# RohanVKashyap/resolution-pde

Hardware: AMD Instinct MI355X
Metric: training samples/sec, FFNO2D NS 256^2 (higher is better)
Workload: dtype f32; 1 GPU; FFNO2D(1,1,width=64,n_layers=4,n_modes=20,factor=4,ff_weight_norm,n_ff_layers=3,layer_norm,dropout=0.1) train step on [B,1,256,256] Gaussian random fields (BASELINE configs[2]); batch_per_gpu=32, global_batch=32, optimizer=AdamW lr=1e-3 (rpde.optim.FlatAdamW: torch.optim.AdamW's rule, one kernel), parallelism=single, grad_bucket_bytes=6828576, target=input advanced by a fixed spectral filter (utils/synthetic.py:advance)

## Files before the change

include/rpde.h:

```cpp
#ifndef RPDE_H
#define RPDE_H

#include <stddef.h>
#include <stdint.h>

#ifdef __cplusplus
extern "C" {
#endif

typedef enum {
  RPDE_OK = 0,
  RPDE_ERR_ARG = -1,
  RPDE_ERR_HIP = -2,
  RPDE_ERR_WORKSPACE = -3,
  RPDE_ERR_MODES = -4
} rpde_status;

enum { RPDE_NORM_BACKWARD = 0, RPDE_NORM_ORTHO = 1, RPDE_NORM_FORWARD = 2 };
enum { RPDE_MODE_FULL = 0, RPDE_MODE_LOWPASS = 1 };
enum { RPDE_ACT_IDENTITY = 0, RPDE_ACT_GELU = 1, RPDE_ACT_RELU = 2 };
enum { RPDE_EPI_MULAUX = 100 };

const char* rpde_last_error(void);
int rpde_version(void);

typedef struct rpde_plan rpde_plan;
int rpde_plan_create(rpde_plan** plan, int n, int modes, int norm, void* stream);
int rpde_plan_destroy(rpde_plan* plan);
int rpde_plan_info(const rpde_plan* plan, int* n, int* modes, int* kp, int* ldn);
int rpde_plan_cache_count(void);
int rpde_plan_tables(const rpde_plan* plan, float* analysis_host, float* synthesis_host);

typedef struct {
  const float* A; const float* B; float* C;
  int M, N, K;
  int a_kmajor;
  int b_kmajor;
  int64_t lda, ldb, ldc;
  int batch, zdiv;
  int64_t sA1, sA2, sB1, sB2, sC1, sC2;
  int ksplit;
  int64_t sCk;
  float alpha;
  int accumulate;
  const float* bias; int bias_mode;
  int act_a, act_b;
  int epi_dact;
  const float* aux; int64_t ldaux;
  float drop_p; uint64_t drop_seed; int64_t drop_ld;
  int write_act;
  int drop_where;
  float* colsum;
  float* aux_out;
  const void* b_split;
  const void* a_split;
  const float* acc_src;
  const uint64_t* drop_epoch;
} rpde_gemm_desc;
int rpde_gemm_f32(const rpde_gemm_desc* d, void* stream);

size_t rpde_split_weights_bytes(int N, int K);
int rpde_split_weights(const float* w, int kmajor, int64_t ld, int N, int K, void* out, void* stream);

size_t rpde_fspectral1d_ws_bytes(int B, int n, int C, int K);
size_t rpde_fspectral1d_spec_elems(int B, int n, int C, int K);
int rpde_fspectral1d_fwd(const float* x, const float* w, float* out, float* spec_in,
                         int B, int n, int C, int K, int mode, int norm,
                         void* ws, size_t ws_bytes, void* stream);
int rpde_fspectral1d_bwd(const float* grad_out, const float* spec_in, const float* w,
                         float* grad_x, float* grad_w, const float* grad_skip,
                         int B, int n, int C, int K, int mode, int norm,
                         void* ws, size_t ws_bytes, void* stream);

size_t rpde_fspectral2d_ws_bytes(int B, int M, int N, int C, int K);
size_t rpde_fspectral2d_spec_elems(int B, int M, int N, int C, int K, int axis );
int rpde_fspectral2d_fwd(const float* x, const float* w_y, const float* w_x, float* out,
                         float* spec_y, float* spec_x,
                         int B, int M, int N, int C, int K, int mode,
                         void* ws, size_t ws_bytes, void* stream);
int rpde_fspectral2d_bwd(const float* grad_out, const float* spec_y, const float* spec_x,
                         const float* w_y, const float* w_x,
                         float* grad_x, float* grad_wy, float* grad_wx, const float* grad_skip,
                         int B, int M, int N, int C, int K, int mode,
                         void* ws, size_t ws_bytes, void* stream);
size_t rpde_fspectral2d_prep_bytes(int M, int N, int C, int K);
size_t rpde_fspectral2d_eval_ws_bytes(int B, int M, int N, int C, int K);
int rpde_fspectral2d_prepare(const float* w_y, const float* w_x, int M, int N, int C, int K,
                             void* prep, size_t prep_bytes, void* stream);
int rpde_fspectral2d_fwd_prepared(const float* x, const void* prep, float* out, int B, int M, int N, int C, int K,
                                  void* ws, size_t ws_bytes, void* stream);

size_t rpde_spectral1d_ws_bytes(int B, int Cin, int Cout, int n, int K);
int rpde_spectral1d_fwd(const float* x, const float* w, float* out, float* spec_in,
                        int B, int Cin, int Cout, int n, int K, int act_in,
                        void* ws, size_t ws_bytes, void* stream);
int rpde_spectral1d_bwd(const float* grad_out, const float* spec_in, const float* w,
                        const float* x, float* grad_x, float* grad_w,
                        int B, int Cin, int Cout, int n, int K, int act_in,
                        void* ws, size_t ws_bytes, void* stream);

size_t rpde_spectral2d_ws_bytes(int B, int Cin, int Cout, int M, int N, int m1, int m2);
size_t rpde_spectral2d_spec_elems(int B, int Cin, int M, int N, int m1, int m2);
int rpde_spectral2d_fwd(const float* x, const float* w1, const float* w2, float* out, float* spec_in,
                        int B, int Cin, int Cout, int M, int N, int m1, int m2, int act_in,
                        void* ws, size_t ws_bytes, void* stream);
int rpde_spectral2d_bwd(const float* grad_out, const float* spec_in, const float* w1, const float* w2,
                        const float* x, float* grad_x, float* grad_w1, float* grad_w2,
                        int B, int Cin, int Cout, int M, int N, int m1, int m2, int act_in,
                        void* ws, size_t ws_bytes, void* stream);

typedef struct {
  int n_layers; int dim; int factor;
  int layer_norm; float ln_eps;
  float dropout_p; uint64_t seed;
  int post_act;
  const float* const* weights;
  const float* const* biases;
  const float* ln_gamma; const float* ln_beta;
  const uint64_t* seed_epoch;
} rpde_ff_params;
size_t rpde_feedforward_ws_bytes(int64_t P, int dim, int factor, int n_layers);
size_t rpde_feedforward_fwd_ws_bytes(int dim, int factor, int n_layers);
int rpde_feedforward_is_fused(int dim, int factor, int n_layers, int64_t P);
int rpde_feedforward_fwd(const rpde_ff_params* p, const float* x, const float* residual,
                         float* const* hs, float* const* ds, float* z_last, float* out, int64_t P,
                         void* ws, size_t ws_bytes, void* stream);
int rpde_feedforward_bwd(const rpde_ff_params* p, const float* x, const float* const* hs,
                         const float* const* ds, const float* z_last,
                         const float* grad_out, float* grad_x,
                         float* const* grad_weights, float* const* grad_biases,
                         float* grad_gamma, float* grad_beta, int64_t P,
                         void* ws, size_t ws_bytes, void* stream);
int rpde_feedforward_prepare(const rpde_ff_params* p, void* prep, size_t prep_bytes, void* stream);
int rpde_feedforward_fwd_prepared(const rpde_ff_params* p, const float* x, const float* residual, float* out, int64_t P,
                                  const void* prep, size_t prep_bytes, void* stream);

size_t rpde_linear_ws_bytes(int64_t P, int in_f, int out_f);
int rpde_linear_fwd(const float* x, const float* w, const float* b, float* out,
                    int64_t P, int in_f, int out_f, void* stream);
int rpde_linear_bwd(const float* x, const float* w, const float* grad_out,
                    float* grad_x, float* grad_w, float* grad_b,
                    int64_t P, int in_f, int out_f, void* ws, size_t ws_bytes, void* stream);

int rpde_weight_norm_fwd(const float* v, const float* g, float* w, int out_f, int in_f, void* stream);
int rpde_weight_norm_bwd(const float* v, const float* g, const float* grad_w, float* grad_v, float* grad_g,
                         int out_f, int in_f, void* stream);

size_t rpde_conv1x1_ws_bytes(int B, int Cin, int Cout, int64_t S);
int rpde_conv1x1_fwd(const float* x, const float* w, const float* b, float* out,
                     int B, int Cin, int Cout, int64_t S, int act_in, int accumulate, void* stream);
int rpde_conv1x1_act_fwd(const float* x, const float* w, const float* b, float* out,
                         int B, int Cin, int Cout, int64_t S, int act_in, int accumulate, int act_out, void* stream);
size_t rpde_fnoblock2d_eval_ws_bytes(int B, int Cin, int Cout, int M, int N, int m1, int m2);
int rpde_fnoblock2d_eval_ok(int Cin, int Cout, int M, int N, int m2);
int rpde_fnoblock2d_eval_fwd(const float* x, const float* w1, const float* w2, const float* wc, const float* bc, float* out,
                             int B, int Cin, int Cout, int M, int N, int m1, int m2, int act_out,
                             void* ws, size_t ws_bytes, void* stream);
int rpde_fnoblock2d_proj_eval_ok(int Cin, int Cout, int M, int N, int m1, int m2, int Cmid, int Cq);
int rpde_fnoblock2d_proj_eval_fwd(const float* x, const float* w1, const float* w2, const float* wc, const float* bc,
                                  const float* pw1, const float* pb1, const float* pw2, const float* pb2, float* out, int B,
                                  int Cin, int Cout, int M, int N, int m1, int m2, int act_out, int Cmid, int Cq,
                                  void* ws, size_t ws_bytes, void* stream);
size_t rpde_fno2d_lift_block_eval_ws_bytes(int B, int C, int Cout, int M, int N, int m1, int m2);
int rpde_fno2d_lift_block_eval_ok(int Cu, int C, int Cout, int M, int N, int m1, int m2);
int rpde_fno2d_lift_block_eval_fwd(const float* u, const float* gx, const float* gy, const float* wl, const float* bl,
                                   const float* w1, const float* w2, const float* wc, const float* bc, float* out, int B, int C,
                                   int Cout, int M, int N, int m1, int m2, int act_out, void* ws, size_t ws_bytes, void* stream);
int rpde_conv_mlp_ok(int Cin, int Cmid, int Cout, int64_t S);
int rpde_conv_mlp_fwd(const float* x, const float* w1, const float* b1, const float* w2, const float* b2, float* out,
                      int B, int Cin, int Cmid, int Cout, int64_t S, int act_in, void* stream);
int rpde_conv1x1_bwd(const float* x, const float* w, const float* grad_out,
                     float* grad_x, float* grad_w, float* grad_b,
                     int B, int Cin, int Cout, int64_t S, int act_in, int accumulate_gx,
                     void* ws, size_t ws_bytes, void* stream);

int rpde_concat_grid(const float* x, float* out, int B, int Cin, int M, int N ,
                     int grid_dims , double lo, double hi, int channels_last,
                     const float* gridx, const float* gridy, void* stream);
int rpde_transpose_cs(const float* in, float* out, int B, int64_t S, int C, int to_channels_first, void* stream);

size_t rpde_resize1d_ws_bytes(int64_t rows, int n_in, int n_out);
int rpde_resize1d(const float* x, float* out, int64_t rows, int n_in, int n_out,
                  void* ws, size_t ws_bytes, void* stream);
size_t rpde_resize2d_ws_bytes(int64_t rows, int M, int N, int Mo, int No);
int rpde_resize2d(const float* x, float* out, int64_t rows, int M, int N, int Mo, int No,
                  void* ws, size_t ws_bytes, void* stream);

size_t rpde_freq_energy1d_ws_bytes(int64_t rows, int n, int num_modes);
int rpde_freq_energy1d(const float* pred, const float* target, double* acc, int64_t rows, int n, int num_modes,
                       void* ws, size_t ws_bytes, void* stream);
size_t rpde_freq_energy2d_ws_bytes(int64_t images, int H, int W);
int rpde_freq_energy2d(const float* pred, const float* target, const int32_t* bins, double* acc, int64_t images,
                       int H, int W, int n_bins, void* ws, size_t ws_bytes, void* stream);

int rpde_act_fwd(const float* x, float* out, int64_t n, int act, void* stream);
int rpde_act_bwd(const float* x, const float* g, float* dx, int64_t n, int act, void* stream);

int64_t rpde_rel_l2_stats_elems(int B);
int rpde_rel_l2_fwd(const float* x, const float* y, float* rel, float* loss, float* stats,
                    int B, int64_t per, int size_average, void* stream);
int rpde_rel_l2_bwd(const float* x, const float* y, const float* stats,
                    const float* grad_loss, const float* grad_rel, float* grad_x,
                    int B, int64_t per, int size_average, void* stream);

int rpde_adamw_step(float* p, const float* g, float* m, float* v, int64_t n,
                    float one_minus_lr_wd, float one_minus_b1, float b2, float one_minus_b2,
                    float step_size, float bc2_sqrt, float eps, void* stream);
int rpde_adamw_step_dev(float* p, const float* g, float* m, float* v, int64_t n,
                        float lr, float b1, float b2, float eps, float weight_decay,
                        float* step_dev, void* stream);
int rpde_adamw_set_hyper_dev(float* step_dev, float lr, float weight_decay, void* stream);
int rpde_adamw_apply_dev(float* p, const float* g, float* m, float* v, int64_t n,
                         float lr, float b1, float b2, float eps, float weight_decay,
                         const float* step_dev, void* stream);

// ... 5 lines not shown
```

resolution-pde_amd/csrc/feedforward.hip:

```cpp
#include "rpde_internal.h"
#include "pointwise.h"
#include "gemm_kernel.h"
#include "ff_fused.h"
#include "wgrad_h2.h"
#include "thin_linear.h"
#include "conv_small.h"

#include <vector>

namespace rpde {


static inline int ff_in(const rpde_ff_params* p, int l) { return l == 0 ? p->dim : p->dim * p->factor; }
static inline int ff_out(const rpde_ff_params* p, int l) { return l == p->n_layers - 1 ? p->dim : p->dim * p->factor; }

static inline int wgrad_split(long P, int out_f, int in_f) {
  const int tiles = ((out_f + 127) / 128) * ((in_f + 127) / 128);
  long s = 768 / tiles;
  const long cap = (P + 127) / 128;
  if (s > cap) s = cap;
  if (s < 1) s = 1;
  if (s > 1024) s = 1024;
  return (int)s;
}
// ... 62 lines not shown
  if (!dstored && !colsum_slab) {
    if (out_f <= 4 && thin_linear_ok(out_f, in_f) && al16(gx)) return thin_expand(gy, w, 1, in_f, nullptr, gx, P, out_f, in_f, st);
    if (in_f <= 4 && thin_linear_ok(in_f, out_f) && al16(gy)) return thin_contract(gy, w, 1, in_f, nullptr, gx, P, in_f, out_f, st);
  }
  rpde_gemm_desc d = gemm_desc();
  d.A = gy; d.a_kmajor = 1; d.lda = out_f;
  d.B = w; d.b_kmajor = 0; d.ldb = in_f;
  if (wimg && worth_presplit(P, in_f, out_f)) {
    if (!wimg_ready) RPDE_TRY(split_weights(w, 0, in_f, in_f, out_f, wimg, st));
    d.b_split = wimg;
  }
  d.C = gx; d.ldc = in_f;
  d.M = (int)P; d.N = in_f; d.K = out_f;
  if (dstored) { d.epi_dact = RPDE_EPI_MULAUX; d.aux = dstored; d.ldaux = in_f; }
  d.colsum = colsum_slab;
  return launch_gemm(d, st);
}

static size_t ff_wimg_floats(int hid) { return (split_bytes(hid, ((hid + 31) / 32) * 32) + 3) / 4; }

static size_t wgrad_ws_floats(long P, int in_f, int out_f) {
  const int S = wgrad_split(P, out_f, in_f);
  size_t a = (S > 1 ? (size_t)S * out_f * in_f : 0);
  const size_t b = wgrad_h2_slab_floats(P, out_f, in_f);
  if (b > a) a = b;
  if (in_f <= 4 && thin_linear_ok(in_f, out_f) && thin_outer_ws_floats(P, in_f, out_f) > a) a = thin_outer_ws_floats(P, in_f, out_f);
  if (out_f <= 4 && thin_linear_ok(out_f, in_f) && thin_outer_ws_floats(P, out_f, in_f) > a) a = thin_outer_ws_floats(P, out_f, in_f);
  return a;
}

}

using namespace rpde;

extern "C" {

size_t rpde_feedforward_ws_bytes(int64_t P, int dim, int factor, int n_layers) {
  const int hid = n_layers > 1 ? dim * factor : dim;
  size_t n = 2 * arena_bytes((size_t)P * hid);
  for (int l = 0; l < n_layers; ++l) {
    const int i = l == 0 ? dim : dim * factor, o = l == n_layers - 1 ? dim : dim * factor;
    n += arena_bytes(wgrad_ws_floats(P, i, o));
    n += arena_bytes((size_t)(colsum_tiles(P) + REDUCE_CHUNKS) * hid);
    n += arena_bytes(ff_wimg_floats(hid));
  }
  n += arena_bytes(colsum_ws_floats(P, hid)) + arena_bytes(ff_tail_bwd_ws_floats(P, dim));
  rpde_ff_params q;
  memset(&q, 0, sizeof(q));
  q.dim = dim; q.factor = factor; q.n_layers = n_layers;
  if (ff3_fused_ok(&q, (long)P))
    n += arena_bytes((size_t)P * dim) + arena_bytes(ff3_fused_bwd_part_floats()) + arena_bytes(ff3_fused_ws_floats());
  return n;
}

size_t rpde_feedforward_fwd_ws_bytes(int dim, int factor, int n_layers) {
  const size_t a = (size_t)n_layers * arena_bytes(ff_wimg_floats(n_layers > 1 ? dim * factor : dim)), b = arena_bytes(ff3_fused_ws_floats());
  return a > b ? a : b;
}

int rpde_feedforward_is_fused(int dim, int factor, int n_layers, int64_t P) {
  rpde_ff_params q;
  memset(&q, 0, sizeof(q));
  q.dim = dim; q.factor = factor; q.n_layers = n_layers;
  return ff3_fused_ok(&q, (long)P) ? 1 : 0;
}

int rpde_feedforward_prepare(const rpde_ff_params* p, void* prep, size_t prep_bytes, void* stream) {
  RPDE_CHECK_ARG(p && prep, "feedforward_prepare: bad arguments");
  RPDE_CHECK_ARG(ff3_fused_ok(p, 32) && prep_bytes >= arena_bytes(ff3_fused_ws_floats()), "feedforward_prepare: shape not fused or buffer too small");
  RPDE_CHECK_ARG(p->weights && p->weights[0] && p->weights[1] && p->weights[2], "feedforward_prepare: null weights");
  return ff3_fused_prepare(p, prep, as_stream(stream));
}

int rpde_feedforward_fwd_prepared(const rpde_ff_params* p, const float* x, const float* residual, float* out, int64_t P,
                                  const void* prep, size_t prep_bytes, void* stream) {
  RPDE_CHECK_ARG(p && x && out && prep && P > 0 && P < (1L << 31), "feedforward_fwd_prepared: bad arguments");
  RPDE_CHECK_ARG(ff3_fused_ok(p, P) && prep_bytes >= arena_bytes(ff3_fused_ws_floats()), "feedforward_fwd_prepared: shape not fused");
  RPDE_CHECK_ARG(!p->layer_norm || (p->ln_gamma && p->ln_beta), "feedforward_fwd_prepared: layer_norm needs gamma/beta");
  RPDE_CHECK_ARG(p->dropout_p == 0.f, "feedforward_fwd_prepared: evaluation only");
  return ff3_fused_fwd(p, x, residual, nullptr, nullptr, out , out, P,
                       const_cast<void*>(prep), as_stream(stream), true);
}

int rpde_feedforward_fwd(const rpde_ff_params* p, const float* x, const float* residual, float* const* hs,
                         float* const* ds, float* z_last, float* out, int64_t P, void* ws, size_t ws_bytes, void* stream) {
  RPDE_CHECK_ARG(p && x && z_last && out && P > 0, "feedforward_fwd: bad arguments");
  RPDE_CHECK_ARG(p->n_layers >= 1 && p->dim > 0 && p->factor > 0, "feedforward_fwd: bad shape");
  RPDE_CHECK_ARG(P < (1L << 31), "feedforward_fwd: too many points for one call");
  RPDE_CHECK_ARG(p->dropout_p >= 0.f && p->dropout_p < 1.f, "feedforward_fwd: dropout %f", p->dropout_p);
  hipStream_t st = as_stream(stream);
  if (ff3_fused_ok(p, P) && ws && ws_bytes >= arena_bytes(ff3_fused_ws_floats())) {
    RPDE_CHECK_ARG(p->weights[0] && p->weights[1] && p->weights[2], "feedforward_fwd: null weights");
    RPDE_CHECK_ARG(!p->layer_norm || (p->ln_gamma && p->ln_beta), "feedforward_fwd: layer_norm needs gamma/beta");
    return ff3_fused_fwd(p, x, residual, hs, ds, z_last, out, P, ws, st);
  }
  RPDE_CHECK_ARG(p->n_layers == 1 || hs, "feedforward_fwd: hidden buffers missing");
  const int L = p->n_layers;
  Arena ar(ws, ws_bytes);
  const size_t img_floats = ff_wimg_floats(L > 1 ? p->dim * p->factor : p->dim);
  float* wimg[SplitJobs::MAX] = {nullptr, nullptr, nullptr, nullptr};
  bool all_imgs = ws != nullptr && L <= SplitJobs::MAX;
  for (int l = 0; l < (all_imgs ? L : 1) && ws; ++l) {
    float* t = ar.take(img_floats);
    if (!t) { all_imgs = false; break; }
    wimg[l] = t;
  }
  if (all_imgs) {
    SplitJobs sj;
    for (int l = 0; l < L; ++l) {
      RPDE_CHECK_ARG(p->weights[l], "feedforward_fwd: null layer %d weight", l);
      if (worth_presplit(P, ff_out(p, l), ff_in(p, l))) sj.add(p->weights[l], 1, ff_in(p, l), ff_out(p, l), ff_in(p, l), wimg[l]);
    }
    RPDE_TRY(split_weights_multi(sj, st));
  }
  for (int l = 0; l < L; ++l) {
    const bool last = l == L - 1;
    RPDE_CHECK_ARG(p->weights[l] && (last || hs[l]), "feedforward_fwd: null layer %d buffers", l);
    const float* in = l == 0 ? x : hs[l - 1];
    RPDE_TRY(linear_fwd_impl(in, p->weights[l], p->biases ? p->biases[l] : nullptr, last ? z_last : hs[l], P, ff_in(p, l),
                             ff_out(p, l), last ? RPDE_ACT_IDENTITY : RPDE_ACT_GELU, (last || !ds) ? nullptr : ds[l],
                             p->dropout_p, layer_seed(p->seed, l), st, all_imgs ? wimg[l] : wimg[0], p->seed_epoch, all_imgs));
  }
  return ff_tail_fwd(z_last, residual, out, P, p->dim, p->layer_norm, p->ln_eps, p->ln_gamma, p->ln_beta,
                     make_drop(p->dropout_p, layer_seed(p->seed, L - 1), p->seed_epoch), p->post_act, st);
}

int rpde_feedforward_bwd(const rpde_ff_params* p, const float* x, const float* const* hs, const float* const* ds,
                         const float* z_last, const float* grad_out, float* grad_x, float* const* grad_weights,
                         float* const* grad_biases, float* grad_gamma, float* grad_beta, int64_t P, void* ws,
                         size_t ws_bytes, void* stream) {
  RPDE_CHECK_ARG(p && x && z_last && grad_out && P > 0, "feedforward_bwd: bad arguments");
  RPDE_CHECK_ARG(p->n_layers == 1 || (hs && ds), "feedforward_bwd: saved hidden tensors missing");
  RPDE_CHECK_ARG(P < (1L << 31), "feedforward_bwd: too many points for one call");
  hipStream_t st = as_stream(stream);
  const int L = p->n_layers;
  const int hid = L > 1 ? p->dim * p->factor : p->dim;
  Arena ar(ws, ws_bytes);
  float* buf0 = ar.take((size_t)P * hid);
  float* buf1 = ar.take((size_t)P * hid);
  std::vector<float*> slabs_l(L), csum_l(L), wt_l(L);
  for (int l = 0; l < L; ++l) slabs_l[l] = ar.take(wgrad_ws_floats(P, ff_in(p, l), ff_out(p, l)));
  for (int l = 0; l < L; ++l) csum_l[l] = ar.take((size_t)(colsum_tiles(P) + REDUCE_CHUNKS) * hid);
  for (int l = 0; l < L; ++l) wt_l[l] = ar.take(ff_wimg_floats(hid));
  float* small = ar.take(colsum_ws_floats(P, hid));
  float* tailws = ar.take(ff_tail_bwd_ws_floats(P, p->dim));
  if (!ar.ok()) { set_error("feedforward_bwd: workspace too small (%zu bytes given)", ws_bytes); return RPDE_ERR_WORKSPACE; }
  void* wt = wt_l[0];

  if (ff3_fused_ok(p, P) && hs && hs[0] && hs[1]) {
    const int recompute = !(ds && ds[0] && ds[1]);
    const int act_h = recompute ? RPDE_ACT_GELU : RPDE_ACT_IDENTITY;
    float* dz3 = ar.take((size_t)P * p->dim);
    float* part = ar.take(ff3_fused_bwd_part_floats());
    void* fimg = ar.take(ff3_fused_ws_floats());
    if (!ar.ok()) { set_error("feedforward_bwd: workspace too small (%zu bytes given)", ws_bytes); return RPDE_ERR_WORKSPACE; }
    int grid = 0;
    RPDE_TRY(ff3_fused_bwd_launch(p, recompute ? hs : ds, recompute, z_last, grad_out, dz3, buf0, buf1, nullptr, part, &grid, P,
                                  fimg, st));
    const bool both = grad_x && grad_weights && wgrad_h2_dgrad_ok(P, hid, p->dim);
    if (grad_x && !both) RPDE_TRY(linear_dgrad_impl(buf1, p->weights[0], grad_x, P, p->dim, hid, nullptr, nullptr, st, wt));
    if (grad_weights) {
      FoldJobs folds;
      RPDE_TRY(linear_wgrad_impl(hs[1], dz3, grad_weights[2], nullptr, P, hid, p->dim, slabs_l[2], small, st, act_h, &folds));
      RPDE_TRY(linear_wgrad_impl(hs[0], buf0, grad_weights[1], nullptr, P, hid, hid, slabs_l[1], small, st, act_h, &folds));
      if (both) RPDE_TRY(wgrad_h2_dgrad(buf1, x, p->weights[0], grad_weights[0], grad_x, P, p->dim, hid, slabs_l[0], st, &folds));
      else RPDE_TRY(linear_wgrad_impl(x, buf1, grad_weights[0], nullptr, P, p->dim, hid, slabs_l[0], small, st, RPDE_ACT_IDENTITY, &folds));
      RPDE_TRY(fold_jobs(folds, st));
    }
    {
      ReduceSegs sg;
      memset(&sg, 0, sizeof(sg));
      sg.n = FF3_PART; sg.nseg = 5;
      const int off[5] = {0, 256, 512, 576, 640}, len[5] = {hid, hid, p->dim, p->dim, p->dim};
      float* dst[5] = {grad_biases ? grad_biases[0] : nullptr, grad_biases ? grad_biases[1] : nullptr,
                       grad_biases ? grad_biases[2] : nullptr, p->layer_norm ? grad_gamma : nullptr,
                       p->layer_norm ? grad_beta : nullptr};
      for (int k = 0; k < 5; ++k) { sg.off[k] = off[k]; sg.len[k] = len[k]; sg.dst[k] = dst[k]; }
      RPDE_TRY(reduce_slabs_seg(part, grid, FF3_PART, sg, st));
    }
    return RPDE_OK;
  }

  FoldJobs folds;
  float* dz = buf0;
  float* other = buf1;
  int bias_done = 0;
  RPDE_TRY(ff_tail_bwd(z_last, grad_out, dz, P, p->dim, p->layer_norm, p->ln_eps, p->ln_gamma, p->ln_beta,
                       make_drop(p->dropout_p, layer_seed(p->seed, L - 1), p->seed_epoch), p->post_act, grad_gamma, grad_beta,
                       grad_biases ? grad_biases[L - 1] : nullptr, &bias_done, tailws, st, &folds));
  const bool all_imgs = L <= SplitJobs::MAX;
  if (all_imgs) {
    SplitJobs sj;
    for (int l = grad_x ? 0 : 1; l < L; ++l)
      if (worth_presplit(P, ff_in(p, l), ff_out(p, l))) sj.add(p->weights[l], 0, ff_in(p, l), ff_in(p, l), ff_out(p, l), wt_l[l]);
    RPDE_TRY(split_weights_multi(sj, st));
  }
  for (int l = L - 1; l >= 0; --l) {
    const int in_f = ff_in(p, l), out_f = ff_out(p, l);
    const float* in = l == 0 ? x : hs[l - 1];
    float* gb = (grad_biases && !bias_done) ? grad_biases[l] : nullptr;
    RPDE_TRY(linear_wgrad_impl(in, dz, grad_weights ? grad_weights[l] : nullptr, gb, P, in_f, out_f, slabs_l[l], small, st,
                               RPDE_ACT_IDENTITY, &folds));
    bias_done = 0;
    void* img = all_imgs ? wt_l[l] : wt;
    if (l > 0) {
      RPDE_CHECK_ARG(ds[l - 1], "feedforward_bwd: derivative of layer %d was not saved", l - 1);
      const bool fuse = grad_biases && can_fuse_colsum(dz, p->weights[l], other, ds[l - 1], P, in_f, out_f);
      RPDE_TRY(linear_dgrad_impl(dz, p->weights[l], other, P, in_f, out_f, ds[l - 1], fuse ? csum_l[l] : nullptr, st, img, all_imgs));
      if (fuse) {
        const int S = (int)colsum_tiles(P);
        if (!(S <= 4 * REDUCE_CHUNKS && folds.add(csum_l[l], grad_biases[l - 1], in_f, S, in_f)))
          RPDE_TRY(reduce_slabs_2pass(csum_l[l], grad_biases[l - 1], in_f, S, in_f, csum_l[l] + colsum_tiles(P) * in_f, st));
        bias_done = 1;
      }
      float* t = dz; dz = other; other = t;
    } else if (grad_x) {
      RPDE_TRY(linear_dgrad_impl(dz, p->weights[0], grad_x, P, in_f, out_f, nullptr, nullptr, st, img, all_imgs));
    }
  }
  return fold_jobs(folds, st);
}

size_t rpde_linear_ws_bytes(int64_t P, int in_f, int out_f) {
  return arena_bytes(wgrad_ws_floats(P, in_f, out_f)) + arena_bytes(colsum_ws_floats(P, out_f));
}

int rpde_linear_fwd(const float* x, const float* w, const float* b, float* out, int64_t P, int in_f, int out_f, void* stream) {
  RPDE_CHECK_ARG(x && w && out && P > 0 && in_f > 0 && out_f > 0 && P < (1L << 31), "linear_fwd: bad arguments");
  return linear_fwd_impl(x, w, b, out, P, in_f, out_f, RPDE_ACT_IDENTITY, nullptr, 0.f, 0, as_stream(stream));
}

int rpde_linear_bwd(const float* x, const float* w, const float* grad_out, float* grad_x, float* grad_w, float* grad_b,
                    int64_t P, int in_f, int out_f, void* ws, size_t ws_bytes, void* stream) {
  RPDE_CHECK_ARG(x && w && grad_out && P > 0 && in_f > 0 && out_f > 0 && P < (1L << 31), "linear_bwd: bad arguments");
  hipStream_t st = as_stream(stream);
  Arena ar(ws, ws_bytes);
  float* slabs = ar.take(wgrad_ws_floats(P, in_f, out_f));
  float* small = ar.take(colsum_ws_floats(P, out_f));
  if (!ar.ok()) { set_error("linear_bwd: workspace too small"); return RPDE_ERR_WORKSPACE; }
  RPDE_TRY(linear_wgrad_impl(x, grad_out, grad_w, grad_b, P, in_f, out_f, slabs, small, st));
  if (grad_x) RPDE_TRY(linear_dgrad_impl(grad_out, w, grad_x, P, in_f, out_f, nullptr, nullptr, st));
  return RPDE_OK;
}

static int conv1x1_ksplit(int B, int64_t S) {
  int ks = 1;
  while (ks < 8 && B * ks < 64 && S / (2 * ks) >= 128) ks *= 2;
  return ks;
}
size_t rpde_conv1x1_ws_bytes(int B, int Cin, int Cout, int64_t S) {
  return arena_bytes((size_t)B * conv1x1_ksplit(B, S) * Cout * Cin) + arena_bytes((size_t)B * Cout * 64);
}

int rpde_conv1x1_fwd(const float* x, const float* w, const float* b, float* out, int B, int Cin, int Cout, int64_t S,
                     int act_in, int accumulate, void* stream) {
  return rpde_conv1x1_act_fwd(x, w, b, out, B, Cin, Cout, S, act_in, accumulate, RPDE_ACT_IDENTITY, stream);
}

int rpde_conv1x1_act_fwd(const float* x, const float* w, const float* b, float* out, int B, int Cin, int Cout, int64_t S,
                         int act_in, int accumulate, int act_out, void* stream) {
  RPDE_CHECK_ARG(x && w && out && B > 0 && Cin > 0 && Cout > 0 && S > 0 && S < (1L << 31), "conv1x1_fwd: bad arguments");
  if (conv1x1_small_ok(x, out, Cin, Cout, S) && B <= 65535 && (long)B * S >= (1L << 20))
    return conv1x1_small(x, w, b, out, B, Cin, Cout, S, act_in, accumulate, act_out, as_stream(stream));
  rpde_gemm_desc d = gemm_desc();
  d.write_act = act_out;
// ... 82 lines not shown
```

resolution-pde_amd/csrc/ff_fused.h:

```cpp
#pragma once
#include "rpde_internal.h"

namespace rpde {
bool ff3_fused_ok(const rpde_ff_params* p, long P);
size_t ff3_fused_ws_floats();
int ff3_fused_prepare(const rpde_ff_params* p, void* ws, hipStream_t st);
int ff3_fused_fwd(const rpde_ff_params* p, const float* x, const float* residual, float* const* hs, float* const* ds,
                  float* z_last, float* out, long P, void* ws, hipStream_t st, bool prepared = false);
constexpr int FF3_PART = 704;
size_t ff3_fused_bwd_part_floats();
int ff3_fused_bwd_launch(const rpde_ff_params* p, const float* const* ds, int recompute, const float* z_last,
                         const float* grad_out, float* dz3, float* du2, float* du1, float* dx, float* part, int* grid_out,
                         long P, void* ws, hipStream_t st);
}
```

resolution-pde_amd/csrc/ff_fused.hip:

```cpp
#include "ff_fused.h"
#include "cw.h"
#include "h2.h"
#include "pointwise.h"

namespace rpde {

#ifdef RPDE_STAMPS
__device__ unsigned long long g_ffstamps[3 * 64];
#define FFSTAMP(i) do { if (stamp_on && stamp_t < 8) g_ffstamps[stamp_w * 64 + stamp_t * 8 + (i)] = __builtin_amdgcn_s_memtime(); } while (0)
__device__ unsigned long long g_fbstamps[3 * 64];
#define FBSTAMP(i) do { if (stamp_on && stamp_t >= 0 && stamp_t < 8) g_fbstamps[stamp_w * 64 + stamp_t * 8 + (i)] = __builtin_amdgcn_s_memtime(); } while (0)
#else
#define FFSTAMP(i) do { } while (0)
#define FBSTAMP(i) do { } while (0)
#endif

constexpr int FF_WAVES = 8;
constexpr int FF_FRAGS = 24;
constexpr int FF_IMG_BYTES = FF_WAVES * FF_FRAGS * 2048;
constexpr int FF_NCONST = 16;
constexpr int FF_PREP_BLOCKS = FF_WAVES * FF_FRAGS * 64 / 1024;

__global__ __launch_bounds__(1024) void k_ff3_prep(const float* __restrict__ w1, const float* __restrict__ w2,
                                                   const float* __restrict__ w3, const float* __restrict__ b1,
                                                   const float* __restrict__ b2, char* __restrict__ img,
                                                   float* __restrict__ consts) {
  __shared__ float red[6][16];
  __shared__ float fin[6];
  const int tid = threadIdx.x, l = tid & 63, wv = tid >> 6;
  float m1 = 0.f, m2 = 0.f, m3 = 0.f, r1 = 0.f, r2 = 0.f, bm = 0.f;
  {
    const float4* w14 = reinterpret_cast<const float4*>(w1);
    const float4* w34 = reinterpret_cast<const float4*>(w3);
    const float4* w24 = reinterpret_cast<const float4*>(w2);
    float4 a[4], c[4], b[16];
#pragma unroll
    for (int i = 0; i < 4; ++i) { a[i] = w14[tid + 1024 * i]; c[i] = w34[tid + 1024 * i]; }
#pragma unroll
    for (int i = 0; i < 16; ++i) b[i] = w24[tid + 1024 * i];
#pragma unroll
    for (int i = 0; i < 4; ++i) {
      m1 = fmaxf(m1, fmaxf(fmaxf(fabsf(a[i].x), fabsf(a[i].y)), fmaxf(fabsf(a[i].z), fabsf(a[i].w))));
      m3 = fmaxf(m3, fmaxf(fmaxf(fabsf(c[i].x), fabsf(c[i].y)), fmaxf(fabsf(c[i].z), fabsf(c[i].w))));
    }
#pragma unroll
    for (int i = 0; i < 16; ++i) m2 = fmaxf(m2, fmaxf(fmaxf(fabsf(b[i].x), fabsf(b[i].y)), fmaxf(fabsf(b[i].z), fabsf(b[i].w))));
  }
#pragma unroll
  for (int row = wv; row < 256; row += 16) {
    float a = fabsf(w1[row * 64 + l]);
    float b = (fabsf(w2[row * 256 + l]) + fabsf(w2[row * 256 + 64 + l])) + (fabsf(w2[row * 256 + 128 + l]) + fabsf(w2[row * 256 + 192 + l]));
    r1 = fmaxf(r1, wave_sum_dpp(a));
    r2 = fmaxf(r2, wave_sum_dpp(b));
  }
  if (tid < 256) {
    bm = fabsf(b1 ? b1[tid] : 0.f);
  } else if (tid < 512) {
    bm = fabsf(b2 ? b2[tid - 256] : 0.f);
  }
  float v[6] = {m1, m2, m3, r1, r2, 0.f};
#pragma unroll
  for (int k = 0; k < 5; ++k) { v[k] = wave_max(v[k]); if (l == 0) red[k][wv] = v[k]; }
  const float bmw = wave_max(bm);
  if (l == 0) red[5][wv] = bmw;
  __syncthreads();
  if (tid < 5) { float a = 0.f; for (int i = 0; i < 16; ++i) a = fmaxf(a, red[tid][i]); fin[tid] = a; }
  if (tid == 5) { float a = 0.f; for (int i = 0; i < 4; ++i) a = fmaxf(a, red[5][i]); fin[5] = a; }
  __shared__ float fin_b2;
  if (tid == 6) { float a = 0.f; for (int i = 4; i < 8; ++i) a = fmaxf(a, red[5][i]); fin_b2 = a; }
  __syncthreads();
  float sc[3], iv[3];
#pragma unroll
  for (int k = 0; k < 3; ++k) h2_scale(fin[k], 0, sc[k], iv[k]);
  if (tid == 0 && blockIdx.x == 0) {
    consts[0] = iv[0]; consts[1] = iv[1]; consts[2] = iv[2];
    consts[3] = fin[3]; consts[4] = fin[4]; consts[5] = fin[5]; consts[6] = fin_b2;
  }
  for (int it = blockIdx.x * 1024 + tid; it < FF_WAVES * FF_FRAGS * 64; it += gridDim.x * 1024) {
    const int ln = it & 63, f = (it >> 6) % FF_FRAGS, w = it / (64 * FF_FRAGS);
    const int g = ln >> 4, li = ln & 15;
    float x[8];
    if (f < 4) {
      const int row = 16 * (2 * w + (f >> 1)) + li, k0 = 32 * (f & 1) + 8 * g;
#pragma unroll
      for (int j = 0; j < 8; ++j) x[j] = w1[row * 64 + k0 + j] * sc[0];
    } else if (f < 20) {
      const int row = 16 * (2 * w + ((f - 4) >> 3)) + li, kap = (f - 4) & 7;
#pragma unroll
      for (int j = 0; j < 8; ++j) x[j] = w2[row * 256 + 32 * kap + frag_perm(g, j)] * sc[1];
    } else {
      const int row = 16 * (f - 20) + li;
#pragma unroll
      for (int j = 0; j < 8; ++j) x[j] = w3[row * 256 + 32 * w + frag_perm(g, j)] * sc[2];
    }
    h2_put_frag(img + ((long)(w * FF_FRAGS + f)) * 2048 + ln * 16, x);
  }
}

struct FF3P {
  const float* x; const float* res; float* out; float* z3;
  float* h1; float* d1; float* h2; float* d2;
  const char* wimg; const float* consts;
  const float* b1; const float* b2; const float* b3; const float* gamma; const float* beta;
  long P; int layer_norm; float eps; int post_act;
  DropCfg drop[3];
  int ntiles;
};

constexpr int FF_SBUF = 0;
constexpr int FF_RAW = FF_SBUF + 8192;
constexpr int FF_HBUF = FF_RAW + 8192;
constexpr int FF_H2BUF = FF_HBUF + 32768;
constexpr int FF_W3 = FF_H2BUF + 32768;
constexpr int FF_VEC = FF_W3 + 65536;
constexpr int FF_STAT = FF_VEC + 2816;
constexpr int FF_INFO = FF_STAT + 1024;
constexpr int FF_LDS = FF_INFO + 256;

__device__ __forceinline__ void ff_act4(const f32x4v acc, float inv, const float4 b, const DropCfg& drop, uint64_t id,
                                        float (&h)[4], float (&d)[4], float (&u)[4]) {
  float s[4] = {1.f, 1.f, 1.f, 1.f};
  if (drop.on()) drop_scale4(drop, id, s);
  const float bb[4] = {b.x, b.y, b.z, b.w};
#pragma unroll
  for (int r = 0; r < 4; ++r) {
    u[r] = fmaf(acc[r], inv, bb[r]) * s[r];
    act_both(RPDE_ACT_GELU, u[r], h[r], d[r]);
    d[r] *= s[r];
  }
}
__device__ __forceinline__ float4 ff_dact4(const float4 u, const DropCfg& drop, uint64_t id) {
  float s[4] = {1.f, 1.f, 1.f, 1.f};
  if (drop.on()) drop_scale4(drop, id, s);
  return make_float4(dgelu_f(u.x) * s[0], dgelu_f(u.y) * s[1], dgelu_f(u.z) * s[2], dgelu_f(u.w) * s[3]);
}

template <int MODE>
__global__ __launch_bounds__(64 * FF_WAVES, 2) void k_ff3_fwd_h2(const FF3P A0) {
  constexpr bool TRAIN = MODE != 0;
  FF3P A = A0;
#pragma unroll
  for (int i = 0; i < 3; ++i) A.drop[i] = drop_resolve(A0.drop[i]);
  __shared__ __attribute__((aligned(16))) char smem[FF_LDS];
  const int tid = threadIdx.x, l = tid & 63, w = tid >> 6, g = l >> 4, li = l & 15;
  f16x8 w1h[2][2], w1l[2][2], w2h[2][8], w2l[2][8];
  {
    const char* base = A.wimg + (long)w * FF_FRAGS * 2048 + l * 16;
#pragma unroll
    for (int f = 0; f < 4; ++f) {
      w1h[f >> 1][f & 1] = *reinterpret_cast<const f16x8*>(base + f * 2048);
      w1l[f >> 1][f & 1] = *reinterpret_cast<const f16x8*>(base + f * 2048 + 1024);
    }
#pragma unroll
    for (int f = 0; f < 16; ++f) {
      w2h[f >> 3][f & 7] = *reinterpret_cast<const f16x8*>(base + (4 + f) * 2048);
      w2l[f >> 3][f & 7] = *reinterpret_cast<const f16x8*>(base + (4 + f) * 2048 + 1024);
    }
#pragma unroll
    for (int f = 0; f < 4; ++f) {
      const uint4 hi = *reinterpret_cast<const uint4*>(base + (20 + f) * 2048);
      const uint4 lo = *reinterpret_cast<const uint4*>(base + (20 + f) * 2048 + 1024);
      *reinterpret_cast<uint4*>(smem + FF_W3 + (f * 8 + w) * 2048 + l * 16) = hi;
      *reinterpret_cast<uint4*>(smem + FF_W3 + (f * 8 + w) * 2048 + 1024 + l * 16) = lo;
    }
    float* vec = reinterpret_cast<float*>(smem + FF_VEC);
    for (int i = tid; i < 704; i += 64 * FF_WAVES) {
      float v;
      if (i < 256) v = A.b1 ? A.b1[i] : 0.f;
      else if (i < 512) v = A.b2 ? A.b2[i - 256] : 0.f;
      else if (i < 576) v = A.b3 ? A.b3[i - 512] : 0.f;
      else if (i < 640) v = A.gamma ? A.gamma[i - 576] : 1.f;
      else v = A.beta ? A.beta[i - 640] : 0.f;
      vec[i] = v;
    }
  }
  const float* const vec = reinterpret_cast<const float*>(smem + FF_VEC);
  const float winv1 = A.consts[0], winv2 = A.consts[1], winv3 = A.consts[2];
  const float c1 = A.consts[3], c2 = A.consts[4], b1max = A.consts[5], b2max = A.consts[6];
  float* const info = reinterpret_cast<float*>(smem + FF_INFO);
// ... 124 lines not shown
        ff_act4(acc[t], inv2, *reinterpret_cast<const float4*>(vec + 256 + hid), A.drop[1], (uint64_t)(pt * 256 + hid), h, d, u);
        if (MODE == 2 && pt < A.P) *reinterpret_cast<float4*>(A.h2 + pt * 256 + hid) = make_float4(u[0], u[1], u[2], u[3]);
        if (MODE == 1 && pt < A.P) {
          *reinterpret_cast<float4*>(A.h2 + pt * 256 + hid) = make_float4(h[0], h[1], h[2], h[3]);
          *reinterpret_cast<float4*>(A.d2 + pt * 256 + hid) = make_float4(d[0], d[1], d[2], d[3]);
        }
#pragma unroll
        for (int r = 0; r < 4; ++r) hv[4 * t + r] = h[r] * sh2;
      }
      h2_put_frag(smem + FF_H2BUF + ((blk * 8 + w) * 2) * 1024 + l * 16, hv);
    }
    FFSTAMP(4);
    lds_barrier();
    FFSTAMP(5);

    f32x4v acc3 = {0.f, 0.f, 0.f, 0.f};
#pragma unroll
    for (int kap = 0; kap < 8; ++kap) {
      const char* wb = smem + FF_W3 + (t3 * 8 + kap) * 2048 + l * 16;
      const char* hb = smem + FF_H2BUF + ((b3 * 8 + kap) * 2) * 1024 + l * 16;
      acc3 = h2_mfma32(*reinterpret_cast<const f16x8*>(wb), *reinterpret_cast<const f16x8*>(wb + 1024),
                       *reinterpret_cast<const f16x8*>(hb), *reinterpret_cast<const f16x8*>(hb + 1024), acc3);
    }
    if (w < 2 && next_tile < A.ntiles) {
      if (MODE == 1) cw_wait<0, 8>();
      else if (MODE == 2) cw_wait<0, 4>();
      else asm volatile("s_waitcnt vmcnt(0)" ::: "memory");
      s_convert(par ^ 1);
    }
    float v[4];
    {
      const float4 bb = *reinterpret_cast<const float4*>(vec + 512 + 16 * t3 + 4 * g);
      float u0, u1, u2, u3, inv3;
      scales(b3, u0, u1, u2, u3, inv3);
      v[0] = fmaf(acc3[0], inv3, bb.x); v[1] = fmaf(acc3[1], inv3, bb.y);
      v[2] = fmaf(acc3[2], inv3, bb.z); v[3] = fmaf(acc3[3], inv3, bb.w);
      if (TRAIN && pt3 < A.P) *reinterpret_cast<float4*>(A.z3 + off3) = make_float4(v[0], v[1], v[2], v[3]);
      if (A.drop[2].on()) {
        float s4[4];
        drop_scale4(A.drop[2], (uint64_t)(pt3 * 64 + 16 * t3 + 4 * g), s4);
#pragma unroll
        for (int r = 0; r < 4; ++r) v[r] *= s4[r];
      }
    }
    if (A.layer_norm) {
      float sum = (v[0] + v[1]) + (v[2] + v[3]);
      sum += lane_xor16(sum);
      sum += lane_xor32(sum);
      const float mw = sum * (1.f / 16.f);
      float m2 = (v[0] - mw) * (v[0] - mw) + (v[1] - mw) * (v[1] - mw) + (v[2] - mw) * (v[2] - mw) + (v[3] - mw) * (v[3] - mw);
      m2 += lane_xor16(m2);
      m2 += lane_xor32(m2);
      if (g == 0) *reinterpret_cast<float2*>(stat + ((b3 * 4 + t3) * 16 + li) * 2) = make_float2(mw, m2);
    }
    lds_barrier();
    if (A.layer_norm) {
      float mws[4], m2s = 0.f, mean = 0.f;
#pragma unroll
      for (int t = 0; t < 4; ++t) {
        const float2 s2 = *reinterpret_cast<const float2*>(stat + ((b3 * 4 + t) * 16 + li) * 2);
        mws[t] = s2.x; m2s += s2.y; mean += s2.x;
      }
      mean *= 0.25f;
#pragma unroll
      for (int t = 0; t < 4; ++t) m2s += 16.f * (mws[t] - mean) * (mws[t] - mean);
      const float rstd = rsqrtf(m2s * (1.f / 64.f) + A.eps);
      const float4 gm = *reinterpret_cast<const float4*>(vec + 576 + 16 * t3 + 4 * g);
      const float4 bt = *reinterpret_cast<const float4*>(vec + 640 + 16 * t3 + 4 * g);
      v[0] = (v[0] - mean) * rstd * gm.x + bt.x; v[1] = (v[1] - mean) * rstd * gm.y + bt.y;
      v[2] = (v[2] - mean) * rstd * gm.z + bt.z; v[3] = (v[3] - mean) * rstd * gm.w + bt.w;
    }
    if (A.post_act) {
#pragma unroll
      for (int r = 0; r < 4; ++r) v[r] = act_f(A.post_act, v[r]);
    }
    if (pt3 < A.P) *reinterpret_cast<float4*>(A.out + off3) = make_float4(v[0] + resv.x, v[1] + resv.y, v[2] + resv.z, v[3] + resv.w);
    FFSTAMP(6);
#ifdef RPDE_STAMPS
    ++stamp_t;
#endif
  }
}

__global__ __launch_bounds__(1024) void k_ff3_prep_bwd(const float* __restrict__ w1, const float* __restrict__ w2,
                                                       const float* __restrict__ w3, char* __restrict__ img,
                                                       float* __restrict__ consts) {
  __shared__ float red[5][16];
  __shared__ float fin[5];
  const int tid = threadIdx.x, l = tid & 63, wv = tid >> 6;
  float m1 = 0.f, m2 = 0.f, m3 = 0.f, r3 = 0.f, r2 = 0.f;
  {
    const float4* w14 = reinterpret_cast<const float4*>(w1);
    const float4* w34 = reinterpret_cast<const float4*>(w3);
    const float4* w24 = reinterpret_cast<const float4*>(w2);
    float4 a[4], c[4], b[16];
#pragma unroll
    for (int i = 0; i < 4; ++i) { a[i] = w14[tid + 1024 * i]; c[i] = w34[tid + 1024 * i]; }
#pragma unroll
    for (int i = 0; i < 16; ++i) b[i] = w24[tid + 1024 * i];
#pragma unroll
    for (int i = 0; i < 4; ++i) {
      m1 = fmaxf(m1, fmaxf(fmaxf(fabsf(a[i].x), fabsf(a[i].y)), fmaxf(fabsf(a[i].z), fabsf(a[i].w))));
      m3 = fmaxf(m3, fmaxf(fmaxf(fabsf(c[i].x), fabsf(c[i].y)), fmaxf(fabsf(c[i].z), fabsf(c[i].w))));
    }
#pragma unroll
    for (int i = 0; i < 16; ++i) m2 = fmaxf(m2, fmaxf(fmaxf(fabsf(b[i].x), fabsf(b[i].y)), fmaxf(fabsf(b[i].z), fabsf(b[i].w))));
  }
  {
    __shared__ float colp[2][4][256];
    const int col = tid & 255, part = tid >> 8;
    float a = 0.f, b = 0.f;
#pragma unroll
    for (int f = 0; f < 16; ++f) a += fabsf(w3[(16 * part + f) * 256 + col]);
    float wv2[64];
#pragma unroll
    for (int k = 0; k < 64; ++k) wv2[k] = w2[(64 * part + k) * 256 + col];
#pragma unroll
    for (int k = 0; k < 64; ++k) b += fabsf(wv2[k]);
    colp[0][part][col] = a; colp[1][part][col] = b;
    __syncthreads();
    if (tid < 256) {
      r3 = (colp[0][0][tid] + colp[0][1][tid]) + (colp[0][2][tid] + colp[0][3][tid]);
      r2 = (colp[1][0][tid] + colp[1][1][tid]) + (colp[1][2][tid] + colp[1][3][tid]);
    }
  }
  float v[5] = {m1, m2, m3, r3, r2};
#pragma unroll
  for (int k = 0; k < 5; ++k) { v[k] = wave_max(v[k]); if (l == 0) red[k][wv] = v[k]; }
  __syncthreads();
  if (tid < 5) { float a = 0.f; for (int i = 0; i < 16; ++i) a = fmaxf(a, red[tid][i]); fin[tid] = a; }
  __syncthreads();
  float sc[3], iv[3];
#pragma unroll
  for (int k = 0; k < 3; ++k) h2_scale(fin[k], 0, sc[k], iv[k]);
  if (tid == 0 && blockIdx.x == 0) { consts[0] = iv[0]; consts[1] = iv[1]; consts[2] = iv[2]; consts[3] = fin[3]; consts[4] = fin[4]; }
  for (int it = blockIdx.x * 1024 + tid; it < FF_WAVES * FF_FRAGS * 64; it += gridDim.x * 1024) {
    const int ln = it & 63, f = (it >> 6) % FF_FRAGS, w = it / (64 * FF_FRAGS);
    const int g = ln >> 4, li = ln & 15;
    float x[8];
    if (f < 4) {
      const int hid = 16 * (2 * w + (f >> 1)) + li;
#pragma unroll
      for (int j = 0; j < 8; ++j) x[j] = w3[(32 * (f & 1) + frag_perm(g, j)) * 256 + hid] * sc[2];
    } else if (f < 20) {
      const int hid1 = 16 * (2 * w + ((f - 4) >> 3)) + li, kap = (f - 4) & 7;
#pragma unroll
      for (int j = 0; j < 8; ++j) x[j] = w2[(32 * kap + frag_perm(g, j)) * 256 + hid1] * sc[1];
    } else {
      const int feat = 16 * (f - 20) + li;
#pragma unroll
      for (int j = 0; j < 8; ++j) x[j] = w1[(32 * w + frag_perm(g, j)) * 64 + feat] * sc[0];
    }
    h2_put_frag(img + ((long)(w * FF_FRAGS + f)) * 2048 + ln * 16, x);
  }
}

constexpr int FFB_PART = 704;
struct FF3B {
  const float* g; const float* z3; const float* d1; const float* d2;
  float* dz3; float* du2; float* du1; float* dx;
  const char* wimg; const float* consts;
  const float* gamma; const float* beta;
  float* part;
  long P; int layer_norm; float eps; int post_act;
  DropCfg drop2;
  DropCfg drop0, drop1;
  float dmax;
  int ntiles;
};

constexpr int FB_DZBUF = 0;
constexpr int FB_DUBUF = FB_DZBUF + 8192;
constexpr int FB_W3L = FB_DUBUF + 32768;
constexpr int FB_D2 = FB_W3L + 32768;
constexpr int FB_D1 = FB_D2 + 32768;
constexpr int FB_VEC = FB_D1 + 32768;
constexpr int FB_ACC = FB_VEC + 512;
constexpr int FB_INFO = FB_ACC + 8192;
constexpr int FB_LDS = FB_INFO + 128;

template <bool RECOMP>
__global__ __launch_bounds__(64 * FF_WAVES, 2) void k_ff3_bwd_h2(const FF3B A0) {
  __shared__ __attribute__((aligned(16))) char smem[FB_LDS];
  FF3B A = A0;
  A.drop2 = drop_resolve(A0.drop2); A.drop0 = drop_resolve(A0.drop0); A.drop1 = drop_resolve(A0.drop1);
  const int tid = threadIdx.x, l = tid & 63, w = tid >> 6, g = l >> 4, li = l & 15;
  f16x8 w3h[2][2], w2h[2][8], w2l[2][8];
  {
    const char* base = A.wimg + (long)w * FF_FRAGS * 2048 + l * 16;
#pragma unroll
    for (int f = 0; f < 4; ++f) {
      w3h[f >> 1][f & 1] = *reinterpret_cast<const f16x8*>(base + f * 2048);
      *reinterpret_cast<uint4*>(smem + FB_W3L + (w * 4 + f) * 1024 + l * 16) = *reinterpret_cast<const uint4*>(base + f * 2048 + 1024);
    }
#pragma unroll
    for (int f = 0; f < 16; ++f) {
      w2h[f >> 3][f & 7] = *reinterpret_cast<const f16x8*>(base + (4 + f) * 2048);
      w2l[f >> 3][f & 7] = *reinterpret_cast<const f16x8*>(base + (4 + f) * 2048 + 1024);
    }
    float* vecw = reinterpret_cast<float*>(smem + FB_VEC);
    float* accw = reinterpret_cast<float*>(smem + FB_ACC);
    for (int i = tid; i < 128; i += 64 * FF_WAVES) vecw[i] = i < 64 ? (A.gamma ? A.gamma[i] : 1.f) : (A.beta ? A.beta[i - 64] : 0.f);
    for (int i = tid; i < 2048; i += 64 * FF_WAVES) accw[i] = 0.f;
  }
  const float* const vec = reinterpret_cast<const float*>(smem + FB_VEC);
  float* const acc_db1 = reinterpret_cast<float*>(smem + FB_ACC);
  float* const acc_db2 = acc_db1 + 256;
  float* const acc_db3 = acc_db1 + 512;
  float* const acc_dg = acc_db1 + 1024;
  float* const acc_dbt = acc_db1 + 1536;
  float* const info = reinterpret_cast<float*>(smem + FB_INFO);
  const float winv1 = A.consts[0], winv2 = A.consts[1], winv3 = A.consts[2], c3t = A.consts[3], c2t = A.consts[4];
  const unsigned lds0 = lds_addr(smem);
  const int q3 = l >> 4, feat = 4 * li;

  f32x4v g4n = {0.f, 0.f, 0.f, 0.f}, z4n = g4n;
  auto in_issue = [&](int tile) {
    const long p = min((long)tile * 32 + 4 * w + q3, A.P - 1);
    g4n = global_load_b128(A.g + p * 64 + feat);
    z4n = global_load_b128(A.z3 + p * 64 + feat);
  };
  typedef __attribute__((address_space(3))) void* lds_ptr;
  typedef const __attribute__((address_space(1))) void* glb_ptr;
  auto d_issue = [&](const float* d, int area, int tile) {
#pragma unroll
    for (int blk = 0; blk < 2; ++blk)
#pragma unroll
      for (int t = 0; t < 2; ++t) {
        const float* q = d + min((long)tile * 32 + 16 * blk + li, A.P - 1) * 256 + 16 * (2 * w + t) + 4 * g;
        __builtin_amdgcn_global_load_lds((glb_ptr)(q), (lds_ptr)(smem + area + (w * 4 + blk * 2 + t) * 1024), 16, 0, 0);
      }
  };
  asm volatile("s_waitcnt vmcnt(0)" ::: "memory");
  if ((int)blockIdx.x < A.ntiles) {
    in_issue(blockIdx.x);
    d_issue(A.d2, FB_D2, blockIdx.x);
    d_issue(A.d1, FB_D1, blockIdx.x);
// ... 176 lines not shown
    FBSTAMP(6);

#pragma unroll
    for (int i = 0; i < 8; ++i) bsum[i] = 0.f;
    {
      f32x4v acc[2][2];
#pragma unroll
      for (int blk = 0; blk < 2; ++blk) {
        acc[blk][0] = (f32x4v){0.f, 0.f, 0.f, 0.f}; acc[blk][1] = (f32x4v){0.f, 0.f, 0.f, 0.f};
#pragma unroll
        for (int kap = 0; kap < 8; ++kap) {
          const char* hb = smem + FB_DUBUF + ((blk * 8 + kap) * 2) * 1024 + l * 16;
          const f16x8 bh = *reinterpret_cast<const f16x8*>(hb), bl = *reinterpret_cast<const f16x8*>(hb + 1024);
          acc[blk][0] = h2_mfma32(w2h[0][kap], w2l[0][kap], bh, bl, acc[blk][0]);
          acc[blk][1] = h2_mfma32(w2h[1][kap], w2l[1][kap], bh, bl, acc[blk][1]);
        }
      }
      if (has_next) asm volatile("s_waitcnt vmcnt(10)" ::: "memory"); else asm volatile("s_waitcnt vmcnt(2)" ::: "memory");
      FBSTAMP(7);
#pragma unroll
      for (int blk = 0; blk < 2; ++blk) {
        f32x4v dq[2];
        dq[0] = lds_read_b128(lds0 + FB_D1 + (w * 4 + blk * 2) * 1024 + l * 16);
        dq[1] = lds_read_b128(lds0 + FB_D1 + (w * 4 + blk * 2 + 1) * 1024 + l * 16);
        lds_wait(dq[0], dq[1]);
        const long pt = p0 + 16 * blk + li;
        float q0, q1, inv_b, s_du1, q2;
        bscales(blk, q0, q1, inv_b, s_du1, q2);
#pragma unroll
        for (int t = 0; t < 2; ++t) {
          const int hid = 16 * (2 * w + t) + 4 * g;
          float4 d = make_float4(dq[t].x, dq[t].y, dq[t].z, dq[t].w);
          if (RECOMP) d = ff_dact4(d, A.drop0, (uint64_t)(pt * 256 + hid));
          const float u[4] = {acc[blk][t][0] * inv_b * d.x, acc[blk][t][1] * inv_b * d.y,
                              acc[blk][t][2] * inv_b * d.z, acc[blk][t][3] * inv_b * d.w};
          if (pt < A.P) {
            *reinterpret_cast<float4*>(A.du1 + pt * 256 + hid) = make_float4(u[0], u[1], u[2], u[3]);
#pragma unroll
            for (int r = 0; r < 4; ++r) bsum[4 * t + r] += u[r];
          }
        }
      }
    }
    if (has_next) {
      asm volatile("s_waitcnt lgkmcnt(0)" ::: "memory");
      d_issue(A.d1, FB_D1, next_tile);
    }
#pragma unroll
    for (int i = 0; i < 8; ++i) bsum[i] = row_sum15(bsum[i]);
    if (li == 15) {
#pragma unroll
      for (int i = 0; i < 8; ++i) acc_db1[16 * (2 * w + (i >> 2)) + 4 * g + (i & 3)] += bsum[i];
    }
    first = false;
#ifdef RPDE_STAMPS
    ++stamp_t;
#endif
  }
  lds_barrier();
  {
    float* part = A.part + (long)blockIdx.x * FFB_PART;
    for (int i = tid; i < FFB_PART; i += 64 * FF_WAVES) {
      float v;
      if (i < 512) v = acc_db1[i];
      else {
        const float* a8 = acc_db3 + ((i - 512) >> 6) * 512 + ((i - 512) & 63);
        v = 0.f;
#pragma unroll
        for (int ww = 0; ww < FF_WAVES; ++ww) v += a8[ww * 64];
      }
      part[i] = v;
    }
  }
}

bool ff3_fused_ok(const rpde_ff_params* p, long P) {
  if (switch_off("RPDE_FUSED_FF")) return false;
  for (int l = 0; l < 3 && p->weights; ++l)
    if (reinterpret_cast<uintptr_t>(p->weights[l]) & 15) return false;
  return p->n_layers == 3 && p->dim == 64 && p->factor == 4 && P >= 32;
}
size_t ff3_fused_ws_floats() { return (FF_IMG_BYTES + FF_NCONST * 4 + 3) / 4; }

int ff3_fused_prepare(const rpde_ff_params* p, void* ws, hipStream_t st) {
  char* img = static_cast<char*>(ws);
  float* consts = reinterpret_cast<float*>(img + FF_IMG_BYTES);
  const float* b1 = p->biases ? p->biases[0] : nullptr;
  const float* b2 = p->biases ? p->biases[1] : nullptr;
  hipLaunchKernelGGL(k_ff3_prep, dim3(FF_PREP_BLOCKS), dim3(1024), 0, st, p->weights[0], p->weights[1], p->weights[2], b1, b2, img, consts);
  RPDE_LAUNCH_CHECK();
  return RPDE_OK;
}

int ff3_fused_fwd(const rpde_ff_params* p, const float* x, const float* residual, float* const* hs, float* const* ds,
                  float* z_last, float* out, long P, void* ws, hipStream_t st, bool prepared) {
  char* img = static_cast<char*>(ws);
  float* consts = reinterpret_cast<float*>(img + FF_IMG_BYTES);
  const float* b1 = p->biases ? p->biases[0] : nullptr;
  const float* b2 = p->biases ? p->biases[1] : nullptr;
  const float* b3 = p->biases ? p->biases[2] : nullptr;
  if (!prepared) RPDE_TRY(ff3_fused_prepare(p, ws, st));
  FF3P A;
  memset(&A, 0, sizeof(A));
  const bool have_h = hs && hs[0] && hs[1], have_d = ds && ds[0] && ds[1];
  const int mode = have_h ? (have_d ? 1 : 2) : 0;
  A.x = x; A.res = residual; A.out = out; A.z3 = z_last;
  if (mode) { A.h1 = hs[0]; A.h2 = hs[1]; }
  if (mode == 1) { A.d1 = ds[0]; A.d2 = ds[1]; }
  A.wimg = img; A.consts = consts; A.b1 = b1; A.b2 = b2; A.b3 = b3; A.gamma = p->ln_gamma; A.beta = p->ln_beta;
  A.P = P; A.layer_norm = p->layer_norm; A.eps = p->ln_eps; A.post_act = p->post_act;
  for (int l = 0; l < 3; ++l) {
    A.drop[l] = make_drop(p->dropout_p, layer_seed(p->seed, l), p->seed_epoch);
  }
  A.ntiles = (int)((P + 31) / 32);
  int cus;
  RPDE_HIP(cu_count(&cus));
  const int grid = A.ntiles < cus ? A.ntiles : cus;
  if (mode == 1) hipLaunchKernelGGL(k_ff3_fwd_h2<1>, dim3(grid), dim3(64 * FF_WAVES), 0, st, A);
  else if (mode == 2) hipLaunchKernelGGL(k_ff3_fwd_h2<2>, dim3(grid), dim3(64 * FF_WAVES), 0, st, A);
  else hipLaunchKernelGGL(k_ff3_fwd_h2<0>, dim3(grid), dim3(64 * FF_WAVES), 0, st, A);
  RPDE_LAUNCH_CHECK();
  return RPDE_OK;
}

size_t ff3_fused_bwd_part_floats() { return (size_t)1024 * FFB_PART; }

int ff3_fused_bwd_launch(const rpde_ff_params* p, const float* const* ds, int recompute, const float* z_last,
                         const float* grad_out, float* dz3, float* du2, float* du1, float* dx, float* part, int* grid_out,
                         long P, void* ws, hipStream_t st) {
  char* img = static_cast<char*>(ws);
  float* consts = reinterpret_cast<float*>(img + FF_IMG_BYTES);
  hipLaunchKernelGGL(k_ff3_prep_bwd, dim3(FF_PREP_BLOCKS), dim3(1024), 0, st, p->weights[0], p->weights[1], p->weights[2], img, consts);
  RPDE_LAUNCH_CHECK();
  FF3B A;
  memset(&A, 0, sizeof(A));
  A.g = grad_out; A.z3 = z_last; A.d1 = ds[0]; A.d2 = ds[1];
  A.dz3 = dz3; A.du2 = du2; A.du1 = du1; A.dx = dx;
  A.wimg = img; A.consts = consts; A.gamma = p->ln_gamma; A.beta = p->ln_beta; A.part = part;
  A.P = P; A.layer_norm = p->layer_norm; A.eps = p->ln_eps; A.post_act = p->post_act;
  DropCfg dc[3];
  for (int l = 0; l < 3; ++l)
    dc[l] = make_drop(p->dropout_p, layer_seed(p->seed, l), p->seed_epoch);
  A.drop0 = dc[0]; A.drop1 = dc[1]; A.drop2 = dc[2];
  A.dmax = 1.13f * A.drop2.scale;
  A.ntiles = (int)((P + 31) / 32);
  int cus;
  RPDE_HIP(cu_count(&cus));
  if (cus > 1024) cus = 1024;
  const int grid = A.ntiles < cus ? A.ntiles : cus;
  if (recompute) hipLaunchKernelGGL(k_ff3_bwd_h2<true>, dim3(grid), dim3(64 * FF_WAVES), 0, st, A);
  else hipLaunchKernelGGL(k_ff3_bwd_h2<false>, dim3(grid), dim3(64 * FF_WAVES), 0, st, A);
  RPDE_LAUNCH_CHECK();
  *grid_out = grid;
  return RPDE_OK;
}

}

#ifdef RPDE_STAMPS
extern "C" int rpde_debug_ffb_stamps(unsigned long long* host_out) {
  RPDE_HIP(hipDeviceSynchronize());
  RPDE_HIP(hipMemcpyFromSymbol(host_out, HIP_SYMBOL(rpde::g_fbstamps), sizeof(unsigned long long) * 3 * 64));
  return RPDE_OK;
}
extern "C" int rpde_debug_ff_stamps(unsigned long long* host_out) {
  RPDE_HIP(hipDeviceSynchronize());
  RPDE_HIP(hipMemcpyFromSymbol(host_out, HIP_SYMBOL(rpde::g_ffstamps), sizeof(unsigned long long) * 3 * 64));
  return RPDE_OK;
}
#endif
```

resolution-pde_amd/csrc/fspectral.hip:

```cpp
#include "rpde_internal.h"
#include "plan.h"
#include "pointwise.h"
#include "fused_spectral.h"
#include "mix1d.h"

namespace rpde {

struct Axis {
  int n;
  int keff, kp;
  int rows;
  int zdiv;
  long s1, s2;
  long ld;
  const rpde_plan* plan;
};

static inline int split_for(long k_total, int tiles) {
  long s = 512 / (tiles > 0 ? tiles : 1);
  const long cap = (k_total + 127) / 128;
  if (s > cap) s = cap;
  if (s < 1) s = 1;
  if (s > 512) s = 512;
  return (int)s;
// ... 80 lines not shown
  RPDE_TRY(dft_analysis(ax, x, spec_in, C, false, st));
  const float* syn_in = spec_in;
  if (mode == RPDE_MODE_FULL && mix1d_ok(ax.rows, C)) {
    float* mixed = ar.take(spec_floats(ax, C));
    if (!ar.ok()) { set_error("fspectral: workspace too small"); return RPDE_ERR_WORKSPACE; }
    RPDE_TRY(mix1d(spec_in, w, mixed, ax.rows, C, K, ax.keff, ax.kp, false, st));
    syn_in = mixed;
  } else if (mode == RPDE_MODE_FULL) {
    float* wblk = ar.take((size_t)ax.keff * 4 * C * C);
    float* mixed = ar.take(spec_floats(ax, C));
    if (!ar.ok()) { set_error("fspectral: workspace too small"); return RPDE_ERR_WORKSPACE; }
    RPDE_TRY(pack_mix_weights(w, wblk, C, C, K, ax.keff, st));
    if (ax.kp != ax.keff) RPDE_HIP(hipMemsetAsync(mixed, 0, spec_floats(ax, C) * sizeof(float), st));
    RPDE_TRY(mode_mix(ax, spec_in, wblk, mixed, C, false, st));
    syn_in = mixed;
  }
  return dft_synthesis(ax, syn_in, out, C, false, accumulate, st);
}

static int axis_bwd(const Axis& ax, const float* g, const float* spec_in, const float* w, int K, float* gx, float* gw, int C,
                    int mode, int accumulate, Arena& ar, hipStream_t st, const float* skip = nullptr) {
  float* gspec = ar.take(spec_floats(ax, C));
  if (!ar.ok()) { set_error("fspectral: workspace too small"); return RPDE_ERR_WORKSPACE; }
  RPDE_TRY(dft_analysis(ax, g, gspec, C, true, st));
  const float* dspec = gspec;
  if (mode == RPDE_MODE_FULL && mix1d_ok(ax.rows, C)) {
    float* dsp = ar.take(spec_floats(ax, C));
    if (!ar.ok()) { set_error("fspectral: workspace too small"); return RPDE_ERR_WORKSPACE; }
    if (gw) RPDE_TRY(mix1d_wgrad(spec_in, gspec, gw, ax.rows, C, K, ax.keff, ax.kp, st));
    if (gx) {
      RPDE_TRY(mix1d(gspec, w, dsp, ax.rows, C, K, ax.keff, ax.kp, true, st));
      dspec = dsp;
    }
  } else if (mode == RPDE_MODE_FULL) {
    float* wblk = ar.take((size_t)ax.keff * 4 * C * C);
    float* dsp = ar.take(spec_floats(ax, C));
    const int S = split_for(ax.rows, wgrad_tiles(C) * ax.keff);
    float* slabs = ar.take((size_t)S * ax.keff * 4 * C * C);
    if (!ar.ok()) { set_error("fspectral: workspace too small"); return RPDE_ERR_WORKSPACE; }
    if (gw) {
      RPDE_TRY(mode_mix_wgrad(ax, spec_in, gspec, slabs, C, S, st));
      RPDE_TRY(unpack_mix_grad(slabs, gw, C, C, K, ax.keff, S, (long)ax.keff * 4 * C * C, st));
    }
    if (gx) {
      RPDE_TRY(pack_mix_weights(w, wblk, C, C, K, ax.keff, st));
      if (ax.kp != ax.keff) RPDE_HIP(hipMemsetAsync(dsp, 0, spec_floats(ax, C) * sizeof(float), st));
      RPDE_TRY(mode_mix(ax, gspec, wblk, dsp, C, true, st));
      dspec = dsp;
    }
  } else if (gw) {
    RPDE_HIP(hipMemsetAsync(gw, 0, sizeof(float) * 2 * (size_t)C * C * K, st));
  }
  if (gx) RPDE_TRY(dft_synthesis(ax, dspec, gx, C, true, (!accumulate && skip) ? 2 : accumulate, st, skip));
  return RPDE_OK;
}

static bool fused_mix_on() {
  return !switch_off("RPDE_FUSED_MIX");
}

static int mixw_slabs(const Axis& ay, const Axis& ax) {
  const long tiles = (ay.rows < ax.rows ? ay.rows : ax.rows) / 32;
  long S = tiles / 4;
  if (S > 12) S = 12;
  if (S < 1) S = 1;
  return (int)S;
}

static size_t fused2d_ws(const Axis& ay, const Axis& ax, int C, bool backward) {
  const size_t spy = arena_bytes(spec_floats(ay, C)), spx = arena_bytes(spec_floats(ax, C));
  const size_t wblk = arena_bytes((size_t)ay.keff * 4 * C * C);
  const size_t img = arena_bytes(fused2d_img_bytes(ay.rows, 2 * ay.kp) / 4) + arena_bytes(fused2d_img_bytes(ax.rows, 2 * ax.kp) / 4);
  const size_t inv = arena_bytes(ay.rows) + arena_bytes(ax.rows);
  const size_t mix = arena_bytes(mix_wimg_bytes(ay.kp) / 4) + arena_bytes(4 * (size_t)ay.kp) + arena_bytes(ay.rows) + arena_bytes(ax.rows);
  size_t n = wblk + (spy > spx ? spy : spx) + img + inv + mix;
  if (backward) {
    const int Sy = split_for(ay.rows, wgrad_tiles(C) * ay.keff), Sx = split_for(ax.rows, wgrad_tiles(C) * ax.keff);
    const size_t sl = arena_bytes((size_t)(Sy > Sx ? Sy : Sx) * ay.keff * 4 * C * C);
    n += spy + spx + sl + arena_bytes(mix_wgrad_slab_floats(ay.kp, mixw_slabs(ay, ax)));
  }
  return n;
}

static int fused2d_fwd(const Axis& ay, const Axis& ax, const float* x, const float* w_y, const float* w_x, float* out,
                       float* spec_y, float* spec_x, int B, int M, int N, int C, int K, int mode, Arena& ar, hipStream_t st,
                       const void* prep = nullptr) {
  float* wblk = ar.take((size_t)ay.keff * 4 * C * C);
  const size_t sy = spec_floats(ay, C), sx = spec_floats(ax, C);
  float* mixed = ar.take(sy > sx ? sy : sx);
  void* imgy = ar.take(fused2d_img_bytes(ay.rows, 2 * ay.kp) / 4);
  void* imgx = ar.take(fused2d_img_bytes(ax.rows, 2 * ax.kp) / 4);
  float* invy = ar.take(ay.rows);
  float* invx = ar.take(ax.rows);
  void* wimg = ar.take(mix_wimg_bytes(ay.kp) / 4);
  float* wc = ar.take(4 * (size_t)ay.kp);
  float* amy = spec_y + spec_floats(ay, C);
  float* amx = spec_x + spec_floats(ax, C);
  if (!ar.ok()) { set_error("fspectral2d: workspace too small"); return RPDE_ERR_WORKSPACE; }
  if (mode == RPDE_MODE_FULL && fused_mix_on()) {
    if (prep) {
      wimg = const_cast<void*>(prep);
      wc = reinterpret_cast<float*>(static_cast<char*>(wimg) + arena_bytes(mix_wimg_bytes(ay.kp) / 4));
    } else {
      RPDE_TRY(mix_prep(w_y, w_x, K, ay.keff, ay.kp, 0, wimg, wc, st));
    }
    RPDE_TRY(fused2d_analysis(x, spec_y, spec_x, amy, amx, ay.plan, ax.plan, 0, B, M, N, st));
    RPDE_TRY(mix_h2(spec_y, spec_x, amy, amx, imgy, imgx, invy, invx, ay.rows, ax.rows, ay.kp, wimg, wc, st));
    return fused2d_synthesis(imgy, imgx, invy, invx, ay.plan, ax.plan, 0, out, nullptr, B, M, N, st);
  }
  RPDE_TRY(fused2d_analysis(x, spec_y, spec_x, nullptr, nullptr, ay.plan, ax.plan, 0, B, M, N, st));
  const Axis* axes[2] = {&ay, &ax};
  const float* ws_[2] = {w_y, w_x};
  float* specs[2] = {spec_y, spec_x};
  void* imgs[2] = {imgy, imgx};
  float* invs[2] = {invy, invx};
  for (int a = 0; a < 2; ++a) {
    const Axis& A = *axes[a];
    const float* syn_in = specs[a];
    if (mode == RPDE_MODE_FULL) {
      RPDE_TRY(pack_mix_weights(ws_[a], wblk, C, C, K, A.keff, st));
      if (A.kp != A.keff) RPDE_HIP(hipMemsetAsync(mixed, 0, spec_floats(A, C) * sizeof(float), st));
      RPDE_TRY(mode_mix(A, specs[a], wblk, mixed, C, false, st));
      syn_in = mixed;
    }
    RPDE_TRY(fused2d_split(syn_in, imgs[a], invs[a], A.rows, 2 * A.kp, st));
  }
  return fused2d_synthesis(imgy, imgx, invy, invx, ay.plan, ax.plan, 0, out, nullptr, B, M, N, st);
}

static int fused2d_bwd(const Axis& ay, const Axis& ax, const float* g, const float* spec_y, const float* spec_x,
                       const float* w_y, const float* w_x, float* gx, float* gwy, float* gwx, const float* skip, int B, int M,
                       int N, int C, int K, int mode, Arena& ar, hipStream_t st) {
  float* gsy = ar.take(spec_floats(ay, C));
  float* gsx = ar.take(spec_floats(ax, C));
  float* wblk = ar.take((size_t)ay.keff * 4 * C * C);
  const size_t sy = spec_floats(ay, C), sx = spec_floats(ax, C);
  float* dsp = ar.take(sy > sx ? sy : sx);
  void* imgy = ar.take(fused2d_img_bytes(ay.rows, 2 * ay.kp) / 4);
  void* imgx = ar.take(fused2d_img_bytes(ax.rows, 2 * ax.kp) / 4);
  float* invy = ar.take(ay.rows);
  float* invx = ar.take(ax.rows);
  const int Sy = split_for(ay.rows, wgrad_tiles(C) * ay.keff), Sx = split_for(ax.rows, wgrad_tiles(C) * ax.keff);
  float* slabs = ar.take((size_t)(Sy > Sx ? Sy : Sx) * ay.keff * 4 * C * C);
  void* wimg = ar.take(mix_wimg_bytes(ay.kp) / 4);
  float* wc = ar.take(4 * (size_t)ay.kp);
  float* amy = ar.take(ay.rows);
  float* amx = ar.take(ax.rows);
  const int Sw = mixw_slabs(ay, ax);
  float* wslabs = ar.take(mix_wgrad_slab_floats(ay.kp, Sw));
  if (!ar.ok()) { set_error("fspectral2d: workspace too small"); return RPDE_ERR_WORKSPACE; }
  const bool h2mix = mode == RPDE_MODE_FULL && fused_mix_on();
  const bool hmix = h2mix && gx, hwg = h2mix && (gwy || gwx);
  if (hmix) RPDE_TRY(mix_prep(w_y, w_x, K, ay.keff, ay.kp, 1, wimg, wc, st));
  RPDE_TRY(fused2d_analysis(g, gsy, gsx, h2mix ? amy : nullptr, h2mix ? amx : nullptr, ay.plan, ax.plan, 1, B, M, N, st));
  if (hmix) {
    RPDE_TRY(mix_h2(gsy, gsx, amy, amx, imgy, imgx, invy, invx, ay.rows, ax.rows, ay.kp, wimg, wc, st));
  }
  if (hwg) {
    RPDE_TRY(mix_wgrad_h2(spec_y, spec_x, gsy, gsx, spec_y + spec_floats(ay, C), spec_x + spec_floats(ax, C), amy, amx, gwy, gwx,
                          ay.rows, ax.rows, K, ay.keff, ay.kp, wslabs, Sw, st));
  }
  const Axis* axes[2] = {&ay, &ax};
  const float* ws_[2] = {w_y, w_x};
  const float* specs[2] = {spec_y, spec_x};
  float* gspecs[2] = {gsy, gsx};
  float* gws[2] = {gwy, gwx};
  void* imgs[2] = {imgy, imgx};
  float* invs[2] = {invy, invx};
  const int Ss[2] = {Sy, Sx};
  for (int a = 0; a < 2; ++a) {
    const Axis& A = *axes[a];
    const float* dspec = gspecs[a];
    if (mode == RPDE_MODE_FULL) {
      if (gws[a] && !hwg) {
        RPDE_TRY(mode_mix_wgrad(A, specs[a], gspecs[a], slabs, C, Ss[a], st));
        RPDE_TRY(unpack_mix_grad(slabs, gws[a], C, C, K, A.keff, Ss[a], (long)A.keff * 4 * C * C, st));
      }
      if (gx && !hmix) {
        RPDE_TRY(pack_mix_weights(ws_[a], wblk, C, C, K, A.keff, st));
        if (A.kp != A.keff) RPDE_HIP(hipMemsetAsync(dsp, 0, spec_floats(A, C) * sizeof(float), st));
        RPDE_TRY(mode_mix(A, gspecs[a], wblk, dsp, C, true, st));
        dspec = dsp;
      }
    } else if (gws[a]) {
      RPDE_HIP(hipMemsetAsync(gws[a], 0, sizeof(float) * 2 * (size_t)C * C * K, st));
    }
    if (gx && !hmix) RPDE_TRY(fused2d_split(dspec, imgs[a], invs[a], A.rows, 2 * A.kp, st));
  }
  if (gx) RPDE_TRY(fused2d_synthesis(imgy, imgx, invy, invx, ay.plan, ax.plan, 1, gx, skip, B, M, N, st));
  return RPDE_OK;
}

}

using namespace rpde;

extern "C" {

size_t rpde_fspectral1d_ws_bytes(int B, int n, int C, int K) {
  Axis ax; axis_dims(ax, n, K, B);
  return axis_ws_bytes(ax, C);
}
size_t rpde_fspectral1d_spec_elems(int B, int n, int C, int K) {
  Axis ax; axis_dims(ax, n, K, B);
  return spec_floats(ax, C);
}

int rpde_fspectral1d_fwd(const float* x, const float* w, float* out, float* spec_in, int B, int n, int C, int K, int mode,
                         int norm, void* ws, size_t ws_bytes, void* stream) {
  RPDE_CHECK_ARG(x && out && spec_in && B > 0 && n > 0 && C > 0 && K > 0, "fspectral1d_fwd: bad arguments");
  RPDE_CHECK_ARG(mode == RPDE_MODE_LOWPASS || w, "fspectral1d_fwd: null weight");
  RPDE_CHECK_ARG(mode == RPDE_MODE_FULL || mode == RPDE_MODE_LOWPASS, "Mode %d not recognized", mode);
  hipStream_t st = as_stream(stream);
  Axis ax;
  RPDE_TRY(make_axis(ax, n, K, norm, B, 1, (long)n * C, 0, C, st));
  Arena ar(ws, ws_bytes);
  return axis_fwd(ax, x, w, K, out, spec_in, C, mode, 0, ar, st);
}

int rpde_fspectral1d_bwd(const float* grad_out, const float* spec_in, const float* w, float* grad_x, float* grad_w,
                         const float* grad_skip, int B, int n, int C, int K, int mode, int norm, void* ws, size_t ws_bytes,
                         void* stream) {
  RPDE_CHECK_ARG(grad_out && spec_in && B > 0 && n > 0 && C > 0 && K > 0, "fspectral1d_bwd: bad arguments");
  RPDE_CHECK_ARG(mode == RPDE_MODE_LOWPASS || w, "fspectral1d_bwd: null weight");
  hipStream_t st = as_stream(stream);
  Axis ax;
  RPDE_TRY(make_axis(ax, n, K, norm, B, 1, (long)n * C, 0, C, st));
  Arena ar(ws, ws_bytes);
  return axis_bwd(ax, grad_out, spec_in, w, K, grad_x, grad_w, C, mode, 0, ar, st, grad_skip);
}

size_t rpde_fspectral2d_ws_bytes(int B, int M, int N, int C, int K) {
  Axis ay, ax;
  axis_dims(ay, N, K, B * M);
  axis_dims(ax, M, K, B * N);
  const size_t a = axis_ws_bytes(ay, C), b = axis_ws_bytes(ax, C);
  size_t n = a > b ? a : b;
  if (fused2d_ok(M, N, C, ay.keff, ax.keff)) { const size_t f = fused2d_ws(ay, ax, C, true); if (f > n) n = f; }
  return n;
}
size_t rpde_fspectral2d_spec_elems(int B, int M, int N, int C, int K, int axis) {
  Axis a, o;
  if (axis == 0) { axis_dims(a, N, K, B * M); axis_dims(o, M, K, B * N); } else { axis_dims(a, M, K, B * N); axis_dims(o, N, K, B * M); }
  const bool fused = axis == 0 ? fused2d_ok(M, N, C, a.keff, o.keff) : fused2d_ok(M, N, C, o.keff, a.keff);
  return spec_floats(a, C) + (fused ? (size_t)a.rows : 0);
}

int rpde_fspectral2d_fwd(const float* x, const float* w_y, const float* w_x, float* out, float* spec_y, float* spec_x, int B,
                         int M, int N, int C, int K, int mode, void* ws, size_t ws_bytes, void* stream) {
  RPDE_CHECK_ARG(x && out && spec_y && spec_x && B > 0 && M > 0 && N > 0 && C > 0 && K > 0, "fspectral2d_fwd: bad arguments");
  RPDE_CHECK_ARG(mode == RPDE_MODE_LOWPASS || (w_y && w_x), "fspectral2d_fwd: null weight");
  RPDE_CHECK_ARG(mode == RPDE_MODE_FULL || mode == RPDE_MODE_LOWPASS, "fspectral2d_fwd: mode %d", mode);
  hipStream_t st = as_stream(stream);
  Axis ay, ax;
  RPDE_TRY(make_axis(ay, N, K, RPDE_NORM_ORTHO, B * M, 1, (long)N * C, 0, C, st));
  RPDE_TRY(make_axis(ax, M, K, RPDE_NORM_ORTHO, B * N, N, (long)M * N * C, C, (long)N * C, st));
  if (fused2d_ok(M, N, C, ay.keff, ax.keff)) {
    Arena ar(ws, ws_bytes);
    return fused2d_fwd(ay, ax, x, w_y, w_x, out, spec_y, spec_x, B, M, N, C, K, mode, ar, st);
  }
  {
    Arena ar(ws, ws_bytes);
    RPDE_TRY(axis_fwd(ax, x, w_x, K, out, spec_x, C, mode, 0, ar, st));
  }
  Arena ar(ws, ws_bytes);
  return axis_fwd(ay, x, w_y, K, out, spec_y, C, mode, 1, ar, st);
}

size_t rpde_fspectral2d_prep_bytes(int M, int N, int C, int K) {
  Axis ay, ax;
  axis_dims(ay, N, K, M);
  axis_dims(ax, M, K, N);
  if (!fused2d_ok(M, N, C, ay.keff, ax.keff) || !fused_mix_on()) return 0;
  return arena_bytes(mix_wimg_bytes(ay.kp) / 4) + arena_bytes(4 * (size_t)ay.kp);
}

size_t rpde_fspectral2d_eval_ws_bytes(int B, int M, int N, int C, int K) {
  return rpde_fspectral2d_ws_bytes(B, M, N, C, K) + arena_bytes(rpde_fspectral2d_spec_elems(B, M, N, C, K, 0)) +
         arena_bytes(rpde_fspectral2d_spec_elems(B, M, N, C, K, 1));
}

int rpde_fspectral2d_prepare(const float* w_y, const float* w_x, int M, int N, int C, int K, void* prep, size_t prep_bytes,
                             void* stream) {
  RPDE_CHECK_ARG(w_y && w_x && prep && M > 0 && N > 0 && K > 0, "fspectral2d_prepare: bad arguments");
  const size_t need = rpde_fspectral2d_prep_bytes(M, N, C, K);
  RPDE_CHECK_ARG(need > 0 && prep_bytes >= need, "fspectral2d_prepare: shape not on the fused path or buffer too small");
  Axis ay;
  axis_dims(ay, N, K, M);
  float* wc = reinterpret_cast<float*>(static_cast<char*>(prep) + arena_bytes(mix_wimg_bytes(ay.kp) / 4));
  return mix_prep(w_y, w_x, K, ay.keff, ay.kp, 0, prep, wc, as_stream(stream));
}

int rpde_fspectral2d_fwd_prepared(const float* x, const void* prep, float* out, int B, int M, int N, int C, int K, void* ws,
                                  size_t ws_bytes, void* stream) {
  RPDE_CHECK_ARG(x && prep && out && ws && B > 0 && M > 0 && N > 0 && C > 0 && K > 0, "fspectral2d_fwd_prepared: bad arguments");
  RPDE_CHECK_ARG(rpde_fspectral2d_prep_bytes(M, N, C, K) > 0, "fspectral2d_fwd_prepared: shape not on the fused path");
  hipStream_t st = as_stream(stream);
  Axis ay, ax;
  RPDE_TRY(make_axis(ay, N, K, RPDE_NORM_ORTHO, B * M, 1, (long)N * C, 0, C, st));
  RPDE_TRY(make_axis(ax, M, K, RPDE_NORM_ORTHO, B * N, N, (long)M * N * C, C, (long)N * C, st));
  Arena ar(ws, ws_bytes);
  float* spec_y = ar.take(rpde_fspectral2d_spec_elems(B, M, N, C, K, 0));
  float* spec_x = ar.take(rpde_fspectral2d_spec_elems(B, M, N, C, K, 1));
  if (!ar.ok()) { set_error("fspectral2d_fwd_prepared: workspace too small"); return RPDE_ERR_WORKSPACE; }
  Arena rest(static_cast<char*>(ws) + ar.used, ws_bytes - ar.used);
  return fused2d_fwd(ay, ax, x, nullptr, nullptr, out, spec_y, spec_x, B, M, N, C, K, RPDE_MODE_FULL, rest, st, prep);
}

int rpde_fspectral2d_bwd(const float* grad_out, const float* spec_y, const float* spec_x, const float* w_y, const float* w_x,
                         float* grad_x, float* grad_wy, float* grad_wx, const float* grad_skip, int B, int M, int N, int C,
                         int K, int mode, void* ws, size_t ws_bytes, void* stream) {
  RPDE_CHECK_ARG(grad_out && spec_y && spec_x && B > 0 && M > 0 && N > 0 && C > 0 && K > 0, "fspectral2d_bwd: bad arguments");
  RPDE_CHECK_ARG(mode == RPDE_MODE_LOWPASS || (w_y && w_x), "fspectral2d_bwd: null weight");
  hipStream_t st = as_stream(stream);
  Axis ay, ax;
  RPDE_TRY(make_axis(ay, N, K, RPDE_NORM_ORTHO, B * M, 1, (long)N * C, 0, C, st));
  RPDE_TRY(make_axis(ax, M, K, RPDE_NORM_ORTHO, B * N, N, (long)M * N * C, C, (long)N * C, st));
  if (fused2d_ok(M, N, C, ay.keff, ax.keff)) {
    Arena ar(ws, ws_bytes);
    return fused2d_bwd(ay, ax, grad_out, spec_y, spec_x, w_y, w_x, grad_x, grad_wy, grad_wx, grad_skip, B, M, N, C, K, mode,
                       ar, st);
  }
  {
    Arena ar(ws, ws_bytes);
    RPDE_TRY(axis_bwd(ax, grad_out, spec_x, w_x, K, grad_x, grad_wx, C, mode, 0, ar, st, grad_skip));
  }
  Arena ar(ws, ws_bytes);
  return axis_bwd(ay, grad_out, spec_y, w_y, K, grad_x, grad_wy, C, mode, 1, ar, st);
}

}
```

resolution-pde_amd/csrc/fused_mix.hip:

```cpp
#include "fused_spectral.h"
#include "h2.h"

namespace rpde {

__global__ __launch_bounds__(256) void k_mix_prep(const float* __restrict__ w_y, const float* __restrict__ w_x, int K, int keff,
                                                  int kp, int conj_t, char* __restrict__ img, float* __restrict__ wc) {
  __shared__ float ws[64 * 64 * 2];
  __shared__ float red[2][4];
  const int k = blockIdx.x, a = blockIdx.y, tid = threadIdx.x, l = tid & 63, wv = tid >> 6, g = l >> 4, li = l & 15;
  const float* __restrict__ w = a ? w_x : w_y;
  char* out = img + (size_t)(a * kp + k) * MIX_W_BYTES_PER_MODE;
  if (k >= keff) {
    for (int i = tid; i < MIX_W_BYTES_PER_MODE / 16; i += 256) reinterpret_cast<uint4*>(out)[i] = make_uint4(0, 0, 0, 0);
    if (tid == 0) { wc[(a * kp + k) * 2] = 1.f; wc[(a * kp + k) * 2 + 1] = 0.f; }
    return;
  }
  float m = 0.f;
  float2 v[16];
#pragma unroll
  for (int u = 0; u < 16; ++u) v[u] = *reinterpret_cast<const float2*>(w + ((long)(tid + 256 * u) * K + k) * 2);
#pragma unroll
  for (int u = 0; u < 16; ++u) {
    const int e = tid + 256 * u;
    ws[e * 2] = v[u].x; ws[e * 2 + 1] = v[u].y;
    m = fmaxf(m, fmaxf(fabsf(v[u].x), fabsf(v[u].y)));
  }
  __syncthreads();
  float s = 0.f;
  {
    const int c = tid & 63, part = tid >> 6;
    for (int r = 16 * part; r < 16 * part + 16; ++r) {
      const int e = conj_t ? c * 64 + ((r + c) & 63) : r * 64 + c;
      s += fabsf(ws[e * 2]) + fabsf(ws[e * 2 + 1]);
    }
  }
  __shared__ float psum[4][64];
  psum[tid >> 6][tid & 63] = s;
  __syncthreads();
  s = tid < 64 ? (psum[0][tid] + psum[1][tid]) + (psum[2][tid] + psum[3][tid]) : 0.f;
  m = wave_max(m);
  s = wave_max(s);
  if (l == 0) { red[0][wv] = m; red[1][wv] = s; }
  __syncthreads();
  m = fmaxf(fmaxf(red[0][0], red[0][1]), fmaxf(red[0][2], red[0][3]));
  s = red[1][0];
  float sc, iv;
  h2_scale(m, 0, sc, iv);
  if (tid == 0) { wc[(a * kp + k) * 2] = iv; wc[(a * kp + k) * 2 + 1] = s; }
  const int cb = wv;
#pragma unroll
  for (int part = 0; part < 2; ++part)
#pragma unroll
    for (int ks = 0; ks < 2; ++ks) {
      float v[8];
#pragma unroll
      for (int j = 0; j < 8; ++j) {
        const int kred = 32 * ks + 8 * g + j, col = 16 * cb + li;
        const int e = conj_t ? col * 64 + kred : kred * 64 + col;
        float x = ws[e * 2 + part];
        if (conj_t && part) x = -x;
        v[j] = x * sc;
      }
      uint4 hi, lo;
      h2_split8(v, hi, lo);
      char* p = out + (((cb * 2 + part) * 2 + ks) * 2) * 1024 + l * 16;
      *reinterpret_cast<uint4*>(p) = hi;
      *reinterpret_cast<uint4*>(p + 1024) = lo;
    }
}

size_t mix_wimg_bytes(int kp) { return (size_t)2 * kp * MIX_W_BYTES_PER_MODE; }

int mix_prep(const float* w_y, const float* w_x, int K, int keff, int kp, int conj_t, void* wimg, float* wc, hipStream_t st) {
  hipLaunchKernelGGL(k_mix_prep, dim3(kp, 2), dim3(256), 0, st, w_y, w_x, K, keff, kp, conj_t, (char*)wimg, wc);
  RPDE_LAUNCH_CHECK();
  return RPDE_OK;
}

struct MixP {
  const float* spec[2];
  char* img[2];
  const float* amax[2];
  float* inv[2];
  int tiles[2];
  int tps[2];
  int nblk0;
  const char* wimg; const float* wc;
  int kp, R, nq;
};

constexpr int MIX_LDS = 4 * 3 * 2 * 2 * 1024;

template <int K32, int TG>
__global__ __launch_bounds__(256, 2) void k_mix_h2(const MixP P) {
  constexpr int BB = h2_block_bytes(K32, TG);
  constexpr int NP = h2_np(TG);
  __shared__ __attribute__((aligned(16))) char smem[MIX_LDS];
  const int tid = threadIdx.x, l = tid & 63, w = tid >> 6, g = l >> 4, li = l & 15;
  int bid = blockIdx.x;
  const int a = bid >= P.nblk0 ? 1 : 0;
  if (a) bid -= P.nblk0;
  const int q = bid % P.nq, slice = bid / P.nq;
  const int t0 = slice * P.tps[a], t1 = min(t0 + P.tps[a], P.tiles[a]);
  if (t0 >= t1) return;
  const int cb = w;
  const float* __restrict__ spec = P.spec[a];
  const float* __restrict__ amax = P.amax[a];
  char* __restrict__ img = P.img[a];
  const long lstride = (long)P.R * 64;

  f16x8 wf[4][2][2][2];
  float winv[4];
  {
    const char* base = P.wimg + ((size_t)(a * P.kp + 4 * q) * 4 + cb) * (MIX_W_BYTES_PER_MODE / 4) + l * 16;
#pragma unroll
    for (int kk = 0; kk < 4; ++kk) {
#pragma unroll
      for (int f = 0; f < 8; ++f)
        wf[kk][f >> 2][(f >> 1) & 1][f & 1] = *reinterpret_cast<const f16x8*>(base + (size_t)kk * MIX_W_BYTES_PER_MODE + f * 1024);
      winv[kk] = P.wc[(a * P.kp + 4 * q + kk) * 2];
    }
  }
  float wnorm = 0.f;
  for (int k = l; k < P.kp; k += 64) wnorm = fmaxf(wnorm, P.wc[(a * P.kp + k) * 2 + 1]);
  wnorm = wave_max(wnorm);

  float4 raw[8];
  float am_next = 0.f;
  auto issue = [&](int t) {
    const float* p = spec + ((long)t * 16 + li) * lstride + (4 * q + w) * 128 + 8 * g;
#pragma unroll
    for (int n = 0; n < 8; ++n) raw[n] = *reinterpret_cast<const float4*>(p + (n >> 2) * 64 + ((n >> 1) & 1) * 32 + (n & 1) * 4);
    am_next = amax[(long)t * 16 + li];
  };
  issue(t0);
  const bool tail = q >= 4 * K32;
  for (int t = t0; t < t1; ++t) {
    const long line0 = (long)t * 16;
    const float am_li = am_next;
    {
      const float am = am_li;
      float sin_, iin;
      h2_scale(am, 0, sin_, iin);
#pragma unroll
      for (int part = 0; part < 2; ++part)
#pragma unroll
        for (int ks = 0; ks < 2; ++ks) {
          const float4 v0 = raw[part * 4 + ks * 2], v1 = raw[part * 4 + ks * 2 + 1];
          uint2 h0, l0, h1, l1;
          h2_split4(v0.x * sin_, v0.y * sin_, v0.z * sin_, v0.w * sin_, h0, l0);
          h2_split4(v1.x * sin_, v1.y * sin_, v1.z * sin_, v1.w * sin_, h1, l1);
          const uint4 hi = make_uint4(h0.x, h0.y, h1.x, h1.y), lo = make_uint4(l0.x, l0.y, l1.x, l1.y);
          char* d = smem + (((w * 3 + part) * 2 + ks) * 2) * 1024 + l * 16;
          *reinterpret_cast<uint4*>(d) = hi;
          *reinterpret_cast<uint4*>(d + 1024) = lo;
          if (part) {
            const unsigned s = 0x80008000u;
// ... 238 lines not shown
```

resolution-pde_amd/csrc/fused_spectral.h:

```cpp
#pragma once
#include "rpde_internal.h"
#include "plan.h"

namespace rpde {

bool fused2d_ok(int M, int N, int C, int keff_y, int keff_x);
int h2_build_tables(rpde_plan* p, hipStream_t st);

__host__ __device__ constexpr int h2_np(int TG) { return (3 * TG + 3) / 4; }
__host__ __device__ constexpr int h2_block_bytes(int K32, int TG) { return (2 * K32 + h2_np(TG)) * 1024; }

size_t fused2d_img_bytes(long lines, int R);
int fused2d_analysis(const float* x, float* spec_y, float* spec_x, float* amax_y, float* amax_x, const rpde_plan* py,
                     const rpde_plan* px, int adjoint, int B, int M, int N, hipStream_t st);
int fused2d_split(const float* spec, void* img, float* inv, long lines, int R, hipStream_t st);
int fused2d_synthesis(const void* imgy, const void* imgx, const float* invy, const float* invx, const rpde_plan* py,
                      const rpde_plan* px, int adjoint, float* out, const float* skip, int B, int M, int N, hipStream_t st);

constexpr int MIX_W_BYTES_PER_MODE = 4 * 2 * 2 * 2 * 1024;
size_t mix_wimg_bytes(int kp);
int mix_prep(const float* w_y, const float* w_x, int K, int keff, int kp, int conj_t, void* wimg, float* wc, hipStream_t st);
size_t mix_wgrad_slab_floats(int kp, int S);
int mix_wgrad_h2(const float* spec_y, const float* spec_x, const float* gspec_y, const float* gspec_x, const float* amax_sy,
                 const float* amax_sx, const float* amax_gy, const float* amax_gx, float* gw_y, float* gw_x, long lines_y,
                 long lines_x, int K, int keff, int kp, float* slabs, int S, hipStream_t st);
int mix_h2(const float* spec_y, const float* spec_x, const float* amax_y, const float* amax_x, void* img_y, void* img_x,
           float* inv_y, float* inv_x, long lines_y, long lines_x, int kp, const void* wimg, const float* wc, hipStream_t st);

}
```

resolution-pde_amd/csrc/wgrad_h2.hip:

```cpp
#include "h2.h"
#include "pointwise.h"
#include "wgrad_h2.h"

namespace rpde {

constexpr int WG_WAVES = 8;
constexpr int WG_PANEL = 8192;
constexpr int WG_BLOCKS = 256;

struct WgP {
  const float* a;
  const float* b;
  float* slabs;
  long npts;
  long steps;
  int M, N, nchunk;
  const float* w;
  float* gx;
  int early;
};

template <int PA, int PB, int WM, int WN, int TM, int TN, bool ACT, bool DG = false>
__global__ __launch_bounds__(64 * WG_WAVES, 2) void k_wgrad_h2(const WgP P) {
  static_assert(!DG || (PB == 1 && PA * 2 <= 8), "data gradient: N = 64, M <= 256");
  constexpr int WFRAG = DG ? PA * 2 * 4 * 2048 : 0;
  static_assert(WM * WN == WG_WAVES && PA + PB <= WG_WAVES, "eight waves, one panel per loader wave");
  static_assert(WM * TM * 16 == PA * 64 && WN * TN * 16 == PB * 64, "wave tiles cover the block");
  static_assert((TM * 16) % 64 == 0 || 64 % (TM * 16) == 0, "a wave tile stays inside one panel or covers whole panels");
  constexpr int STAGE = (PA + PB) * WG_PANEL;
  __shared__ __attribute__((aligned(16))) char smem[2 * STAGE + WFRAG];
  __shared__ int einfo[2][WG_WAVES];
  __shared__ float wmax[WG_WAVES];
  const int tid = threadIdx.x, l = tid & 63, wave = tid >> 6, g = l >> 4, li = l & 15;
  const int chunk = blockIdx.x, mblock = blockIdx.y;
  const long s0 = P.steps * chunk / P.nchunk, s1 = P.steps * (chunk + 1) / P.nchunk;

  const bool loader = wave < PA + PB, isA = wave < PA;
  const int ld = isA ? P.M : P.N;
  const float* __restrict__ src = isA ? P.a + mblock * (64 * PA) + 64 * wave : P.b + 64 * (wave - PA);
  src += (long)g * ld + 4 * li;
  float4 buf[8];
  int e_run = 15;
  auto issue = [&](long s) {
    if (!loader || s >= s1) return;
    const float* __restrict__ q0 = src + s * 32 * ld;
    if ((s + 1) * 32 <= P.npts) {
#pragma unroll
      for (int i = 0; i < 8; ++i) buf[i] = *reinterpret_cast<const float4*>(q0 + (long)(4 * i) * ld);
    } else {
#pragma unroll
      for (int i = 0; i < 8; ++i)
        buf[i] = s * 32 + 4 * i + g < P.npts ? *reinterpret_cast<const float4*>(q0 + (long)(4 * i) * ld) : make_float4(0.f, 0.f, 0.f, 0.f);
    }
  };
  auto convert = [&](int st) {
    if (!loader) return;
    if (ACT && !isA) {
#pragma unroll
      for (int i = 0; i < 8; ++i) { buf[i].x = gelu_f(buf[i].x); buf[i].y = gelu_f(buf[i].y); buf[i].z = gelu_f(buf[i].z); buf[i].w = gelu_f(buf[i].w); }
    }
    float m = 0.f;
#pragma unroll
    for (int i = 0; i < 8; ++i) m = fmaxf(fmaxf(m, fmaxf(fabsf(buf[i].x), fabsf(buf[i].y))), fmaxf(fabsf(buf[i].z), fabsf(buf[i].w)));
    m = wave_max(m);
    e_run = max(e_run, (int)(__float_as_uint(m) >> 23) & 0xff);
    e_run = min(e_run, 254);
    const float scale = __uint_as_float((unsigned)(268 - e_run) << 23);
    char* const dst = smem + st * STAGE + wave * WG_PANEL;
#pragma unroll
    for (int i = 0; i < 8; ++i) {
      uint2 hi, lo;
      h2_split4(buf[i].x * scale, buf[i].y * scale, buf[i].z * scale, buf[i].w * scale, hi, lo);
      const int off = stage_off(4 * i + g, li);
      *reinterpret_cast<uint2*>(dst + off) = hi;
      *reinterpret_cast<uint2*>(dst + 4096 + off) = lo;
    }
    if (l == 0) einfo[st][wave] = e_run;
  };

  const int wm = wave / WN, wn = wave % WN;
  const int m_off = wm * TM * 16, n_off = wn * TN * 16;
  const int pa = m_off >> 6, ta0 = (m_off & 63) >> 4, pb = PA + (n_off >> 6), tb0 = (n_off & 63) >> 4;
  const int q = li >> 2, pp = li & 3;
  const int tsw = ((q >> 1) & 1) | ((g & 1) << 1);
  const int trow = (8 * g + q) * 128 + pp * 8;
  typedef s16x4v __attribute__((address_space(3))) * lds_tr;
  auto frag = [&](const char* panel, int tile, f16x8& hi, f16x8& lo) {
    const char* t = panel + trow + ((tile ^ tsw) << 5);
    union { struct { s16x4v a, b; } h; f16x8 v; } uh, ul;
    uh.h.a = __builtin_amdgcn_ds_read_tr16_b64_v4i16((lds_tr)(t));
    uh.h.b = __builtin_amdgcn_ds_read_tr16_b64_v4i16((lds_tr)(t + 512));
    ul.h.a = __builtin_amdgcn_ds_read_tr16_b64_v4i16((lds_tr)(t + 4096));
    ul.h.b = __builtin_amdgcn_ds_read_tr16_b64_v4i16((lds_tr)(t + 4096 + 512));
    hi = uh.v; lo = ul.v;
  };
  f32x4v acc[TM][TN];
#pragma unroll
  for (int i = 0; i < TM; ++i)
#pragma unroll
    for (int j = 0; j < TN; ++j) acc[i][j] = (f32x4v){0.f, 0.f, 0.f, 0.f};
  constexpr int NPA = (TM * 16 + 63) / 64;
  static_assert(TN * 16 <= 64, "one B panel per wave tile");
  int ea_used[NPA], eb_used = 15;
#pragma unroll
  for (int k = 0; k < NPA; ++k) ea_used[k] = 15;

  char* const wfrag = smem + 2 * STAGE;
  float w_inv = 1.f;
  if (DG && s0 < s1) {
    constexpr int NF = PA * 2 * 4 * 64 / (64 * WG_WAVES);
    float wv[NF][8];
    float m = 0.f;
#pragma unroll
    for (int r = 0; r < NF; ++r) {
      const int c = tid + r * 64 * WG_WAVES, fl = c & 63, nt = (c >> 6) & 3, ks = c >> 8;
#pragma unroll
      for (int j = 0; j < 8; ++j) {
        wv[r][j] = P.w[(long)(32 * ks + 8 * (fl >> 4) + j) * P.N + 16 * nt + (fl & 15)];
        m = fmaxf(m, fabsf(wv[r][j]));
      }
    }
    m = wave_max(m);
    if (l == 0) wmax[wave] = m;
    __syncthreads();
    m = 0.f;
#pragma unroll
    for (int i = 0; i < WG_WAVES; ++i) m = fmaxf(m, wmax[i]);
    float w_scale;
    h2_scale(m, 0, w_scale, w_inv);
#pragma unroll
    for (int r = 0; r < NF; ++r) {
      const int c = tid + r * 64 * WG_WAVES, fl = c & 63, nt = (c >> 6) & 3, ks = c >> 8;
      uint2 h0, l0, h1, l1;
      h2_split4(wv[r][0] * w_scale, wv[r][1] * w_scale, wv[r][2] * w_scale, wv[r][3] * w_scale, h0, l0);
      h2_split4(wv[r][4] * w_scale, wv[r][5] * w_scale, wv[r][6] * w_scale, wv[r][7] * w_scale, h1, l1);
      char* d = wfrag + (ks * 4 + nt) * 2048 + fl * 16;
      *reinterpret_cast<uint4*>(d) = make_uint4(h0.x, h0.y, h1.x, h1.y);
      *reinterpret_cast<uint4*>(d + 1024) = make_uint4(l0.x, l0.y, l1.x, l1.y);
    }
  }
  const int dg_mt = wave & 1, dg_nt = wave >> 1;

  const bool early_convert = (P.early >> __builtin_amdgcn_readfirstlane(wave)) & 1;
  if (s0 < s1) {
    issue(s0);
    convert(0);
    issue(s0 + 1);
    lds_barrier();
    for (long s = s0; s < s1; ++s) {
      const int cur = (int)(s - s0) & 1;
      const char* const stage = smem + cur * STAGE;
      if (early_convert && s + 1 < s1) {
        convert(cur ^ 1);
        issue(s + 2);
      }
      const int eb = __builtin_amdgcn_readfirstlane(einfo[cur][pb]);
#pragma unroll
      for (int k = 0; k < NPA; ++k) {
        const int ea = __builtin_amdgcn_readfirstlane(einfo[cur][pa + k]);
        if (ea + eb != ea_used[k] + eb_used) {
          const int d = (ea_used[k] + eb_used) - (ea + eb);
          const float f = d > -126 ? __uint_as_float((unsigned)(127 + d) << 23) : 0.f;
#pragma unroll
          for (int i = 0; i < TM; ++i)
            if (((ta0 + i) >> 2) == k) {
#pragma unroll
              for (int j = 0; j < TN; ++j) acc[i][j] *= f;
            }
        }
        ea_used[k] = ea;
      }
      eb_used = eb;
      f16x8 bh[TN], bl[TN];
#pragma unroll
      for (int j = 0; j < TN; ++j) frag(stage + (pb + ((tb0 + j) >> 2)) * WG_PANEL, (tb0 + j) & 3, bh[j], bl[j]);
#pragma unroll
      for (int i = 0; i < TM; ++i) {
        f16x8 ah, al;
        frag(stage + (pa + ((ta0 + i) >> 2)) * WG_PANEL, (ta0 + i) & 3, ah, al);
#pragma unroll
        for (int j = 0; j < TN; ++j) acc[i][j] = h2_mfma32(ah, al, bh[j], bl[j], acc[i][j]);
      }
      if (DG) {
        f32x4v tot = (f32x4v){0.f, 0.f, 0.f, 0.f};
        const int row = 16 * dg_mt + li;
#pragma unroll
        for (int k = 0; k < PA; ++k) {
          f32x4v part = (f32x4v){0.f, 0.f, 0.f, 0.f};
#pragma unroll
          for (int h = 0; h < 2; ++h) {
            const char* pa_ = stage + k * WG_PANEL + stage_off(row, 2 * (4 * h + g));
            const f16x8 ah = *reinterpret_cast<const f16x8*>(pa_), al = *reinterpret_cast<const f16x8*>(pa_ + 4096);
            const char* wb = wfrag + ((2 * k + h) * 4 + dg_nt) * 2048 + l * 16;
            const f16x8 bh = *reinterpret_cast<const f16x8*>(wb), bl = *reinterpret_cast<const f16x8*>(wb + 1024);
            part = h2_mfma32(ah, al, bh, bl, part);
          }
          const int ek = __builtin_amdgcn_readfirstlane(einfo[cur][k]);
          const float fk = __uint_as_float((unsigned)(ek - 14) << 23) * w_inv;
          tot += part * fk;
        }
        float t0 = tot[0], t1 = tot[1], t2 = tot[2], t3 = tot[3];
        quad_transpose(t0, t1, t2, t3);
        const long pq = s * 32 + 16 * dg_mt + 4 * g + (li & 3);
        if (pq < P.npts) *reinterpret_cast<float4*>(P.gx + pq * P.N + 16 * dg_nt + 4 * (li >> 2)) = make_float4(t0, t1, t2, t3);
      }
      if (!early_convert && s + 1 < s1) {
        convert(cur ^ 1);
        issue(s + 2);
      }
      lds_barrier();
    }
  }

  const float fb = __uint_as_float((unsigned)(eb_used - 14) << 23);
  float* __restrict__ out = P.slabs + (long)chunk * P.M * P.N + (long)(mblock * (64 * PA) + m_off) * P.N + n_off;
#pragma unroll
  for (int i = 0; i < TM; ++i) {
    const float fa = __uint_as_float((unsigned)(ea_used[(ta0 + i) >> 2] - 14) << 23);
#pragma unroll
    for (int j = 0; j < TN; ++j)
#pragma unroll
      for (int r = 0; r < 4; ++r) out[(long)(16 * i + 4 * g + r) * P.N + 16 * j + li] = acc[i][j][r] * fa * fb;
  }
}

bool wgrad_h2_ok(long P, int out_f, int in_f) {
  if (switch_off("RPDE_WGRAD_H2") || P < 32L * WG_BLOCKS) return false;
  return (out_f == 256 && in_f == 256) || (out_f == 256 && in_f == 64) || (out_f == 64 && in_f == 256);
}

static int wg_chunks(int, int) { return WG_BLOCKS; }

static int wg_early_mask(int out_f, int in_f) {
  return out_f == 256 && in_f == 256 ? 0xF0 : (out_f == 64 ? 0x0E : 0x00);
}

size_t wgrad_h2_slab_floats(long P, int out_f, int in_f) {
  return wgrad_h2_ok(P, out_f, in_f) ? (size_t)wg_chunks(out_f, in_f) * out_f * in_f : 0;
}

template <int PA, int PB, int WM, int WN, int TM, int TN>
static void wg_launch(const WgP& p, int mblocks, bool act, hipStream_t st) {
  const dim3 grid(p.nchunk, mblocks);
  if (act) hipLaunchKernelGGL((k_wgrad_h2<PA, PB, WM, WN, TM, TN, true>), grid, dim3(64 * WG_WAVES), 0, st, p);
  else hipLaunchKernelGGL((k_wgrad_h2<PA, PB, WM, WN, TM, TN, false>), grid, dim3(64 * WG_WAVES), 0, st, p);
}

bool wgrad_h2_dgrad_ok(long P, int out_f, int in_f) { return wgrad_h2_ok(P, out_f, in_f) && out_f == 256 && in_f == 64; }

int wgrad_h2_dgrad(const float* gy, const float* h, const float* w, float* gw, float* gx, long P, int in_f, int out_f,
                   float* slabs, hipStream_t st, FoldJobs* defer) {
  RPDE_CHECK_ARG(wgrad_h2_dgrad_ok(P, out_f, in_f) && slabs && w && gx, "wgrad_h2_dgrad: unsupported shape");
  WgP p;
  p.a = gy; p.b = h; p.slabs = slabs; p.npts = P; p.steps = (P + 31) / 32; p.M = out_f; p.N = in_f; p.nchunk = WG_BLOCKS;
  p.early = wg_early_mask(out_f, in_f);
  p.w = w; p.gx = gx;
  hipLaunchKernelGGL((k_wgrad_h2<4, 1, 4, 2, 4, 2, false, true>), dim3(p.nchunk, 1), dim3(64 * WG_WAVES), 0, st, p);
  RPDE_LAUNCH_CHECK();
  if (defer && defer->add(slabs, gw, out_f * in_f, p.nchunk, (long)out_f * in_f)) return RPDE_OK;
  return reduce_slabs(slabs, gw, (long)out_f * in_f, p.nchunk, (long)out_f * in_f, 1.f, 0, st);
}

int wgrad_h2(const float* gy, const float* h, float* gw, long P, int in_f, int out_f, int act_b, float* slabs, hipStream_t st,
             FoldJobs* defer) {
  RPDE_CHECK_ARG(wgrad_h2_ok(P, out_f, in_f) && slabs, "wgrad_h2: unsupported shape");
  RPDE_CHECK_ARG(act_b == RPDE_ACT_IDENTITY || act_b == RPDE_ACT_GELU, "wgrad_h2: activation %d", act_b);
  WgP p;
  p.a = gy; p.b = h; p.slabs = slabs; p.npts = P; p.steps = (P + 31) / 32; p.M = out_f; p.N = in_f; p.nchunk = wg_chunks(out_f, in_f);
  p.early = wg_early_mask(out_f, in_f);
  p.w = nullptr; p.gx = nullptr;
  const bool act = act_b == RPDE_ACT_GELU;
  if (out_f == 256 && in_f == 256) wg_launch<4, 4, 2, 4, 8, 4>(p, 1, act, st);
  else if (out_f == 256) wg_launch<4, 1, 4, 2, 4, 2>(p, 1, act, st);
  else wg_launch<1, 4, 1, 8, 4, 2>(p, 1, act, st);
  RPDE_LAUNCH_CHECK();
  if (defer && defer->add(slabs, gw, out_f * in_f, p.nchunk, (long)out_f * in_f)) return RPDE_OK;
  return reduce_slabs(slabs, gw, (long)out_f * in_f, p.nchunk, (long)out_f * in_f, 1.f, 0, st);
}

}
```

resolution-pde_amd/rpde/_lib.py:

```python
from __future__ import annotations

import ctypes as C
import os
from typing import Optional, Sequence

import torch

_HERE = os.path.dirname(os.path.abspath(__file__))
LIB_PATH = os.environ.get("RPDE_LIB") or os.path.join(_HERE, "lib", "librpde_hip.so")

ACT = {"identity": 0, "gelu": 1, "relu": 2}
NORM = {"backward": 0, "ortho": 1, "forward": 2}
MODE = {"full": 0, "low-pass": 1}

ERR_ARG, ERR_HIP, ERR_WORKSPACE, ERR_MODES = -1, -2, -3, -4


class RpdeError(RuntimeError):
    pass


class GemmDesc(C.Structure):
    _fields_ = [
        ("A", C.c_void_p), ("B", C.c_void_p), ("C", C.c_void_p),
        ("M", C.c_int), ("N", C.c_int), ("K", C.c_int),
        ("a_kmajor", C.c_int), ("b_kmajor", C.c_int),
        ("lda", C.c_int64), ("ldb", C.c_int64), ("ldc", C.c_int64),
        ("batch", C.c_int), ("zdiv", C.c_int),
        ("sA1", C.c_int64), ("sA2", C.c_int64), ("sB1", C.c_int64), ("sB2", C.c_int64),
        ("sC1", C.c_int64), ("sC2", C.c_int64),
        ("ksplit", C.c_int), ("sCk", C.c_int64),
        ("alpha", C.c_float), ("accumulate", C.c_int),
        ("bias", C.c_void_p), ("bias_mode", C.c_int),
        ("act_a", C.c_int), ("act_b", C.c_int),
        ("epi_dact", C.c_int),
        ("aux", C.c_void_p), ("ldaux", C.c_int64),
        ("drop_p", C.c_float), ("drop_seed", C.c_uint64), ("drop_ld", C.c_int64),
        ("write_act", C.c_int), ("drop_where", C.c_int),
        ("colsum", C.c_void_p), ("aux_out", C.c_void_p), ("b_split", C.c_void_p), ("a_split", C.c_void_p), ("acc_src", C.c_void_p),
        ("drop_epoch", C.c_void_p),
    ]


class FFParams(C.Structure):
    _fields_ = [
        ("n_layers", C.c_int), ("dim", C.c_int), ("factor", C.c_int),
        ("layer_norm", C.c_int), ("ln_eps", C.c_float),
        ("dropout_p", C.c_float), ("seed", C.c_uint64),
        ("post_act", C.c_int),
        ("weights", C.POINTER(C.c_void_p)), ("biases", C.POINTER(C.c_void_p)),
        ("ln_gamma", C.c_void_p), ("ln_beta", C.c_void_p),
        ("seed_epoch", C.c_void_p),
    ]


_P, _I, _L, _Z, _F, _D = C.c_void_p, C.c_int, C.c_int64, C.c_size_t, C.c_float, C.c_double
_PP = C.POINTER(C.c_void_p)

_SIGNATURES = {
    "rpde_last_error": (C.c_char_p, []),
    "rpde_version": (_I, []),
    "rpde_plan_cache_count": (_I, []),
    "rpde_plan_create": (_I, [C.POINTER(_P), _I, _I, _I, _P]),
    "rpde_plan_destroy": (_I, [_P]),
    "rpde_plan_info": (_I, [_P, C.POINTER(_I), C.POINTER(_I), C.POINTER(_I), C.POINTER(_I)]),
    "rpde_plan_tables": (_I, [_P, _P, _P]),
    "rpde_gemm_f32": (_I, [C.POINTER(GemmDesc), _P]),
    "rpde_split_weights_bytes": (C.c_size_t, [_I, _I]),
    "rpde_split_weights": (_I, [_P, _I, C.c_int64, _I, _I, _P, _P]),
    "rpde_fspectral1d_ws_bytes": (_Z, [_I, _I, _I, _I]),
    "rpde_fspectral1d_spec_elems": (_Z, [_I, _I, _I, _I]),
    "rpde_fspectral1d_fwd": (_I, [_P, _P, _P, _P, _I, _I, _I, _I, _I, _I, _P, _Z, _P]),
    "rpde_fspectral1d_bwd": (_I, [_P, _P, _P, _P, _P, _P, _I, _I, _I, _I, _I, _I, _P, _Z, _P]),
    "rpde_fspectral2d_ws_bytes": (_Z, [_I, _I, _I, _I, _I]),
    "rpde_fspectral2d_spec_elems": (_Z, [_I, _I, _I, _I, _I, _I]),
    "rpde_fspectral2d_fwd": (_I, [_P, _P, _P, _P, _P, _P, _I, _I, _I, _I, _I, _I, _P, _Z, _P]),
    "rpde_fspectral2d_bwd": (_I, [_P, _P, _P, _P, _P, _P, _P, _P, _P, _I, _I, _I, _I, _I, _I, _P, _Z, _P]),
    "rpde_spectral1d_ws_bytes": (_Z, [_I, _I, _I, _I, _I]),
    "rpde_spectral1d_fwd": (_I, [_P, _P, _P, _P, _I, _I, _I, _I, _I, _I, _P, _Z, _P]),
    "rpde_spectral1d_bwd": (_I, [_P, _P, _P, _P, _P, _P, _I, _I, _I, _I, _I, _I, _P, _Z, _P]),
    "rpde_spectral2d_ws_bytes": (_Z, [_I, _I, _I, _I, _I, _I, _I]),
    "rpde_spectral2d_spec_elems": (_Z, [_I, _I, _I, _I, _I, _I]),
    "rpde_spectral2d_fwd": (_I, [_P, _P, _P, _P, _P, _I, _I, _I, _I, _I, _I, _I, _I, _P, _Z, _P]),
    "rpde_spectral2d_bwd": (_I, [_P, _P, _P, _P, _P, _P, _P, _P, _I, _I, _I, _I, _I, _I, _I, _I, _P, _Z, _P]),
    "rpde_feedforward_ws_bytes": (_Z, [_L, _I, _I, _I]),
    "rpde_feedforward_fwd_ws_bytes": (_Z, [_I, _I, _I]),
    "rpde_feedforward_is_fused": (_I, [_I, _I, _I, _L]),
    "rpde_feedforward_fwd": (_I, [C.POINTER(FFParams), _P, _P, _PP, _PP, _P, _P, _L, _P, _Z, _P]),
    "rpde_feedforward_bwd": (_I, [C.POINTER(FFParams), _P, _PP, _PP, _P, _P, _P, _PP, _PP, _P, _P, _L, _P, _Z, _P]),
    "rpde_feedforward_prepare": (_I, [C.POINTER(FFParams), _P, _Z, _P]),
    "rpde_feedforward_fwd_prepared": (_I, [C.POINTER(FFParams), _P, _P, _P, _L, _P, _Z, _P]),
    "rpde_fspectral2d_prep_bytes": (_Z, [_I, _I, _I, _I]),
    "rpde_fspectral2d_eval_ws_bytes": (_Z, [_I, _I, _I, _I, _I]),
    "rpde_fspectral2d_prepare": (_I, [_P, _P, _I, _I, _I, _I, _P, _Z, _P]),
    "rpde_fspectral2d_fwd_prepared": (_I, [_P, _P, _P, _I, _I, _I, _I, _I, _P, _Z, _P]),
    "rpde_fno2d_lift_block_eval_ws_bytes": (_Z, [_I] * 7),
    "rpde_fno2d_lift_block_eval_ok": (_I, [_I] * 7),
    "rpde_fno2d_lift_block_eval_fwd": (_I, [_P] * 10 + [_I] * 8 + [_P, _Z, _P]),
    "rpde_linear_ws_bytes": (_Z, [_L, _I, _I]),
    "rpde_weight_norm_fwd": (_I, [_P, _P, _P, _I, _I, _P]),
    "rpde_weight_norm_bwd": (_I, [_P, _P, _P, _P, _P, _I, _I, _P]),
    "rpde_linear_fwd": (_I, [_P, _P, _P, _P, _L, _I, _I, _P]),
    "rpde_linear_bwd": (_I, [_P, _P, _P, _P, _P, _P, _L, _I, _I, _P, _Z, _P]),
    "rpde_conv1x1_ws_bytes": (_Z, [_I, _I, _I, _L]),
    "rpde_conv1x1_fwd": (_I, [_P, _P, _P, _P, _I, _I, _I, _L, _I, _I, _P]),
    "rpde_conv1x1_act_fwd": (_I, [_P, _P, _P, _P, _I, _I, _I, _L, _I, _I, _I, _P]),
    "rpde_fnoblock2d_eval_ws_bytes": (_Z, [_I, _I, _I, _I, _I, _I, _I]),
    "rpde_fnoblock2d_eval_ok": (_I, [_I, _I, _I, _I, _I]),
    "rpde_fnoblock2d_eval_fwd": (_I, [_P, _P, _P, _P, _P, _P, _I, _I, _I, _I, _I, _I, _I, _I, _P, _Z, _P]),
    "rpde_fnoblock2d_proj_eval_ok": (_I, [_I, _I, _I, _I, _I, _I, _I, _I]),
    "rpde_fnoblock2d_proj_eval_fwd": (_I, [_P, _P, _P, _P, _P, _P, _P, _P, _P, _P, _I, _I, _I, _I, _I, _I, _I, _I, _I, _I, _P, _Z, _P]),
    "rpde_conv_mlp_ok": (_I, [_I, _I, _I, _L]),
    "rpde_conv_mlp_fwd": (_I, [_P, _P, _P, _P, _P, _P, _I, _I, _I, _I, _L, _I, _P]),
    "rpde_conv1x1_bwd": (_I, [_P, _P, _P, _P, _P, _P, _I, _I, _I, _L, _I, _I, _P, _Z, _P]),
    "rpde_resize1d_ws_bytes": (_Z, [_L, _I, _I]),
    "rpde_resize1d": (_I, [_P, _P, _L, _I, _I, _P, _Z, _P]),
    "rpde_resize2d_ws_bytes": (_Z, [_L, _I, _I, _I, _I]),
    "rpde_resize2d": (_I, [_P, _P, _L, _I, _I, _I, _I, _P, _Z, _P]),
    "rpde_freq_energy1d_ws_bytes": (_Z, [_L, _I, _I]),
    "rpde_freq_energy1d": (_I, [_P, _P, _P, _L, _I, _I, _P, _Z, _P]),
    "rpde_freq_energy2d_ws_bytes": (_Z, [_L, _I, _I]),
    "rpde_freq_energy2d": (_I, [_P, _P, _P, _P, _L, _I, _I, _I, _P, _Z, _P]),
    "rpde_concat_grid": (_I, [_P, _P, _I, _I, _I, _I, _I, _D, _D, _I, _P, _P, _P]),
    "rpde_transpose_cs": (_I, [_P, _P, _I, _L, _I, _I, _P]),
    "rpde_act_fwd": (_I, [_P, _P, _L, _I, _P]),
    "rpde_act_bwd": (_I, [_P, _P, _P, _L, _I, _P]),
    "rpde_rel_l2_stats_elems": (_L, [_I]),
    "rpde_rel_l2_fwd": (_I, [_P, _P, _P, _P, _P, _I, _L, _I, _P]),
    "rpde_rel_l2_bwd": (_I, [_P, _P, _P, _P, _P, _P, _I, _L, _I, _P]),
    "rpde_adamw_step": (_I, [_P, _P, _P, _P, _L, _F, _F, _F, _F, _F, _F, _F, _P]),
    "rpde_adamw_step_dev": (_I, [_P, _P, _P, _P, _L, _F, _F, _F, _F, _F, _P, _P]),
    "rpde_adamw_set_hyper_dev": (_I, [_P, _F, _F, _P]),
    "rpde_adamw_apply_dev": (_I, [_P, _P, _P, _P, _L, _F, _F, _F, _F, _F, _P, _P]),
}

_lib: Optional[C.CDLL] = None


def load() -> C.CDLL:
    global _lib
    if _lib is not None:
        return _lib
    if not os.path.exists(LIB_PATH):
        raise RpdeError(
            f"{LIB_PATH} is missing: build it with `python resolution-pde_amd/rpde/build.py` "
            "(hipcc, gfx950).  There is no CPU fallback for the spectral hot path.")
    lib = C.CDLL(LIB_PATH)
    for name, (res, args) in _SIGNATURES.items():
        fn = getattr(lib, name)
        fn.restype, fn.argtypes = res, args
    _lib = lib
    return lib


def check(status: int, what: str = "") -> None:
    if status == 0:
        return
    msg = (load().rpde_last_error() or b"").decode(errors="replace")
    text = f"rpde {what} failed ({status}): {msg}"
    if status == ERR_ARG and "not recognized" in msg:
        raise ValueError(msg)
    raise RpdeError(text)


def stream_ptr() -> int:
    return torch.cuda.current_stream().cuda_stream


def ptr(t: Optional[torch.Tensor]) -> Optional[int]:
    if t is None:
        return None
    if not t.is_cuda:
        raise RpdeError("the spectral hot path runs on the GPU only (got a CPU tensor); "
                        "the CPU oracle lives under oracle/ and is test infrastructure")
# ... 17 lines not shown
```

resolution-pde_amd/rpde/ops.py:

```python
from __future__ import annotations

import contextlib
import os

import ctypes as C
from typing import List, Optional, Sequence, Tuple

import torch

from . import _lib
from ._lib import ACT, MODE, NORM, check, load, ptr, ptr_array, stream_ptr, workspace


def _f32c(t: torch.Tensor) -> torch.Tensor:
    if t.dtype != torch.float32:
        t = t.float()
    return t if t.is_contiguous() else t.contiguous()


def _as_float_storage(w: torch.Tensor) -> torch.Tensor:
    w = w if w.is_contiguous() else w.contiguous()
    return torch.view_as_real(w) if w.is_complex() else w


# ... 5 lines not shown
        _FROZEN.clear()


@contextlib.contextmanager
def frozen_weights():
    global _FROZEN
    outer = _FROZEN
    if outer is None:
        _FROZEN = {}
    try:
        yield
    finally:
        if outer is None:
            _FROZEN = None


def _frozen_entry(kind, tensors, extra, nbytes, build, originals=None):
    if _FROZEN is None or torch.cuda.is_current_stream_capturing():
        return None
    if originals is not None and any(t is not o for t, o in zip(tensors, originals)):
        return None
    key = (kind, extra) + tuple(t.data_ptr() for t in tensors)
    ver = tuple(t._version for t in tensors)
    hit = _FROZEN.get(key)
    if hit is not None and hit[0] == ver:
        return hit[1]
    buf = hit[1] if hit is not None else torch.empty(nbytes, dtype=torch.uint8, device=tensors[0].device)
    build(buf)
    _FROZEN[key] = (ver, buf, tensors)
    return buf


class _FSpectral1d(torch.autograd.Function):
    @staticmethod
    def forward(ctx, x, w, modes: int, mode: int, norm: int, with_skip: bool = False):
        lib = load()
        x = _f32c(x)
        wf = _f32c(w) if w is not None else None
        B, n, Cc = x.shape
        out = torch.empty_like(x)
        spec = torch.empty(lib.rpde_fspectral1d_spec_elems(B, n, Cc, modes), dtype=torch.float32, device=x.device)
        nws = lib.rpde_fspectral1d_ws_bytes(B, n, Cc, modes)
        ws = workspace(nws, x.device)
        check(lib.rpde_fspectral1d_fwd(ptr(x), ptr(wf), ptr(out), ptr(spec), B, n, Cc, modes, mode, norm,
                                       ws.data_ptr(), nws, stream_ptr()), "fspectral1d_fwd")
        ctx.save_for_backward(spec, wf if wf is not None else x.new_empty(0))
        ctx.dims = (B, n, Cc, modes, mode, norm, wf is not None)
        return (out, x.view_as(x)) if with_skip else out

    @staticmethod
    def backward(ctx, g, g_skip=None):
        lib = load()
        spec, wf = ctx.saved_tensors
        B, n, Cc, modes, mode, norm, has_w = ctx.dims
        if g is None:
            return g_skip, None, None, None, None, None
        g = _f32c(g)
        g_skip = _f32c(g_skip) if g_skip is not None else None
        need_x, need_w = ctx.needs_input_grad[0], ctx.needs_input_grad[1] and has_w
        gx = torch.empty_like(g) if need_x else None
        gw = torch.empty_like(wf) if need_w else None
        nws = lib.rpde_fspectral1d_ws_bytes(B, n, Cc, modes)
        ws = workspace(nws, g.device)
        check(lib.rpde_fspectral1d_bwd(ptr(g), ptr(spec), ptr(wf) if has_w else None, ptr(gx), ptr(gw),
                                       ptr(g_skip) if need_x else None, B, n, Cc, modes,
                                       mode, norm, ws.data_ptr(), nws, stream_ptr()), "fspectral1d_bwd")
        return gx, gw, None, None, None, None


class _FSpectral2d(torch.autograd.Function):
    @staticmethod
    def forward(ctx, x, wy, wx, modes: int, mode: int, with_skip: bool = False):
        lib = load()
        x = _f32c(x)
        has_w = wy is not None
        wyf = _f32c(wy) if has_w else None
        wxf = _f32c(wx) if has_w else None
        B, M, N, Cc = x.shape
        out = torch.empty_like(x)
        spec_y = torch.empty(lib.rpde_fspectral2d_spec_elems(B, M, N, Cc, modes, 0), dtype=torch.float32, device=x.device)
        spec_x = torch.empty(lib.rpde_fspectral2d_spec_elems(B, M, N, Cc, modes, 1), dtype=torch.float32, device=x.device)
        nws = lib.rpde_fspectral2d_ws_bytes(B, M, N, Cc, modes)
        ws = workspace(nws, x.device)
        check(lib.rpde_fspectral2d_fwd(ptr(x), ptr(wyf), ptr(wxf), ptr(out), ptr(spec_y), ptr(spec_x), B, M, N, Cc, modes,
                                       mode, ws.data_ptr(), nws, stream_ptr()), "fspectral2d_fwd")
        if has_w:
            ctx.save_for_backward(spec_y, spec_x, wyf, wxf)
        else:
            ctx.save_for_backward(spec_y, spec_x)
        ctx.dims = (B, M, N, Cc, modes, mode, has_w)
        return (out, x.view_as(x)) if with_skip else out

    @staticmethod
    def backward(ctx, g, g_skip=None):
        lib = load()
        B, M, N, Cc, modes, mode, has_w = ctx.dims
        if g is None:
            return g_skip, None, None, None, None, None
        if has_w:
            spec_y, spec_x, wyf, wxf = ctx.saved_tensors
        else:
            (spec_y, spec_x), wyf, wxf = ctx.saved_tensors, None, None
        g = _f32c(g)
        g_skip = _f32c(g_skip) if g_skip is not None else None
        need_x = ctx.needs_input_grad[0]
        need_w = has_w and (ctx.needs_input_grad[1] or ctx.needs_input_grad[2])
        gx = torch.empty_like(g) if need_x else None
        gwy = torch.empty_like(wyf) if need_w else None
        gwx = torch.empty_like(wxf) if need_w else None
        nws = lib.rpde_fspectral2d_ws_bytes(B, M, N, Cc, modes)
        ws = workspace(nws, g.device)
        check(lib.rpde_fspectral2d_bwd(ptr(g), ptr(spec_y), ptr(spec_x), ptr(wyf), ptr(wxf), ptr(gx), ptr(gwy), ptr(gwx),
                                       ptr(g_skip) if need_x else None,
                                       B, M, N, Cc, modes, mode, ws.data_ptr(), nws, stream_ptr()), "fspectral2d_bwd")
        return gx, gwy, gwx, None, None, None


def _fspectral2d_frozen(x, wy, wx, modes: int):
    lib = load()
    x = _f32c(x)
    B, M, N, Cc = x.shape
    npre = lib.rpde_fspectral2d_prep_bytes(M, N, Cc, modes)
    if npre == 0:
        return None
    wyf, wxf = _f32c(wy), _f32c(wx)
    prep = _frozen_entry("fs2d", (wyf, wxf), (M, N, Cc, modes), npre, lambda buf: check(
        lib.rpde_fspectral2d_prepare(ptr(wyf), ptr(wxf), M, N, Cc, modes, buf.data_ptr(), npre, stream_ptr()),
        "fspectral2d_prepare"), originals=(wy, wx))
    if prep is None:
        return None
    out = torch.empty_like(x)
    nws = lib.rpde_fspectral2d_eval_ws_bytes(B, M, N, Cc, modes)
    ws = workspace(nws, x.device)
    check(lib.rpde_fspectral2d_fwd_prepared(ptr(x), prep.data_ptr(), ptr(out), B, M, N, Cc, modes, ws.data_ptr(), nws,
                                            stream_ptr()), "fspectral2d_fwd_prepared")
    return out


def fspectral1d(x, w, modes: int, mode: str = "full", norm: str = "ortho", with_skip: bool = False):
    if mode not in MODE:
        raise ValueError(f"Mode {mode} not recognized")
    return _FSpectral1d.apply(x, w if mode == "full" else None, int(modes), MODE[mode], NORM[norm], bool(with_skip))


def fspectral2d(x, wy, wx, modes: int, mode: str = "full", with_skip: bool = False):
    if mode not in MODE:
        return (torch.zeros_like(x), x) if with_skip else torch.zeros_like(x)
    full = mode == "full"
    if full and _FROZEN is not None and not torch.is_grad_enabled() and x.is_cuda:
        out = _fspectral2d_frozen(x, wy, wx, int(modes))
        if out is not None:
            return (out, x) if with_skip else out
    return _FSpectral2d.apply(x, wy if full else None, wx if full else None, int(modes), MODE[mode], bool(with_skip))


_DROP_EPOCH: dict = {}


def drop_epoch(device) -> torch.Tensor:
    dev = torch.device(device)
    key = (dev.type, dev.index if dev.index is not None else torch.cuda.current_device())
    t = _DROP_EPOCH.get(key)
    if t is None:
        t = torch.zeros(1, dtype=torch.int64, device=dev)
        _DROP_EPOCH[key] = t
    return t


class _FeedForward(torch.autograd.Function):
    @staticmethod
    def forward(ctx, x, residual, cfg, *params):
        lib = load()
        L, dim, factor, layer_norm, eps, p_drop, seed, post_act, grad_on = cfg
        shape = x.shape
        x2 = _f32c(x).reshape(-1, dim)
        P = x2.shape[0]
        res2 = _f32c(residual).reshape(-1, dim) if residual is not None else None
        ws_ = [_f32c(params[2 * l]) for l in range(L)]
        bs_ = [_f32c(params[2 * l + 1]) for l in range(L)]
        gamma = _f32c(params[2 * L]) if layer_norm else None
        beta = _f32c(params[2 * L + 1]) if layer_norm else None
        need_grad = grad_on and any(ctx.needs_input_grad)
        hid = dim * factor
        fused = bool(lib.rpde_feedforward_is_fused(dim, factor, L, P)) and all(w.data_ptr() % 16 == 0 for w in ws_)
        lean = (not need_grad) and fused
        recompute = need_grad and fused and os.environ.get("RPDE_FF_STASH", "hd") == "u"
        hs = [None if lean else torch.empty(P, hid, dtype=torch.float32, device=x.device) for _ in range(L - 1)]
        ds = [torch.empty(P, hid, dtype=torch.float32, device=x.device) if (need_grad and not recompute) else None
              for _ in range(L - 1)]
        out = torch.empty(P, dim, dtype=torch.float32, device=x.device)
        z_last = out if lean else torch.empty(P, dim, dtype=torch.float32, device=x.device)
        wa, ba, ha, da = ptr_array(ws_), ptr_array(bs_), ptr_array(hs or [None]), ptr_array(ds or [None])
        epoch = drop_epoch(x.device).data_ptr() if p_drop > 0.0 else None
        fp = _lib.FFParams(L, dim, factor, int(layer_norm), eps, p_drop, seed, post_act,
                           C.cast(wa, C.POINTER(C.c_void_p)), C.cast(ba, C.POINTER(C.c_void_p)), ptr(gamma), ptr(beta), epoch)
        nws = lib.rpde_feedforward_fwd_ws_bytes(dim, factor, L)
        if lean and p_drop == 0.0:
            held = tuple(ws_ + bs_ + ([gamma, beta] if layer_norm else []))
            orig = tuple([params[2 * l] for l in range(L)] + [params[2 * l + 1] for l in range(L)] +
                         ([params[2 * L], params[2 * L + 1]] if layer_norm else []))
            prep = _frozen_entry("ff", held, (L, dim, factor), nws, lambda buf: check(
                lib.rpde_feedforward_prepare(C.byref(fp), buf.data_ptr(), nws, stream_ptr()), "feedforward_prepare"),
                originals=orig)
            if prep is not None:
                check(lib.rpde_feedforward_fwd_prepared(C.byref(fp), ptr(x2), ptr(res2), ptr(out), P, prep.data_ptr(), nws,
                                                        stream_ptr()), "feedforward_fwd_prepared")
                return out.reshape(shape)
        ws = workspace(nws, x.device)
        check(lib.rpde_feedforward_fwd(C.byref(fp), ptr(x2), ptr(res2), C.cast(ha, C.POINTER(C.c_void_p)),
                                       C.cast(da, C.POINTER(C.c_void_p)), ptr(z_last), ptr(out), P, ws.data_ptr(), nws,
                                       stream_ptr()), "feedforward_fwd")
        ctx.cfg = cfg
        ctx.has_res = residual is not None
        if need_grad:
            ctx.save_for_backward(x2, z_last, *hs, *ds, *ws_, *bs_, *([gamma, beta] if layer_norm else []))
        return out.reshape(shape)

    @staticmethod
    def backward(ctx, g):
        lib = load()
        L, dim, factor, layer_norm, eps, p_drop, seed, post_act, _ = ctx.cfg
        saved = ctx.saved_tensors
        x2, z_last = saved[0], saved[1]
        o = 2
        hs, ds = list(saved[o:o + L - 1]), list(saved[o + L - 1:o + 2 * (L - 1)])
        o += 2 * (L - 1)
        ws_, bs_ = list(saved[o:o + L]), list(saved[o + L:o + 2 * L])
        gamma, beta = (saved[o + 2 * L], saved[o + 2 * L + 1]) if layer_norm else (None, None)
        P = x2.shape[0]
        g2 = _f32c(g).reshape(-1, dim)
        gx = torch.empty_like(x2) if ctx.needs_input_grad[0] else None
        gws = [torch.empty_like(w) for w in ws_]
        gbs = [torch.empty_like(b) for b in bs_]
        ggamma = torch.empty_like(gamma) if layer_norm else None
        gbeta = torch.empty_like(beta) if layer_norm else None
        wa, ba, ha, da = ptr_array(ws_), ptr_array(bs_), ptr_array(hs or [None]), ptr_array(ds or [None])
        gwa, gba = ptr_array(gws), ptr_array(gbs)
        epoch = drop_epoch(g.device).data_ptr() if p_drop > 0.0 else None
        fp = _lib.FFParams(L, dim, factor, int(layer_norm), eps, p_drop, seed, post_act,
                           C.cast(wa, C.POINTER(C.c_void_p)), C.cast(ba, C.POINTER(C.c_void_p)), ptr(gamma), ptr(beta), epoch)
        nws = lib.rpde_feedforward_ws_bytes(P, dim, factor, L)
        ws = workspace(nws, g.device)
        check(lib.rpde_feedforward_bwd(C.byref(fp), ptr(x2), C.cast(ha, C.POINTER(C.c_void_p)),
                                       C.cast(da, C.POINTER(C.c_void_p)), ptr(z_last), ptr(g2), ptr(gx),
                                       C.cast(gwa, C.POINTER(C.c_void_p)), C.cast(gba, C.POINTER(C.c_void_p)),
                                       ptr(ggamma), ptr(gbeta), P, ws.data_ptr(), nws, stream_ptr()), "feedforward_bwd")
        grads: List[Optional[torch.Tensor]] = []
        for l in range(L):
            grads += [gws[l], gbs[l]]
        if layer_norm:
            grads += [ggamma, gbeta]
        gres = g if ctx.has_res else None
        return (gx.reshape(g.shape) if gx is not None else None, gres, None, *grads)


def feedforward(x, residual, weights: Sequence[torch.Tensor], biases: Sequence[torch.Tensor], ln: Optional[Tuple],
                dim: int, factor: int, dropout_p: float, seed: int, post_act: str = "identity", eps: float = 1e-5):
    L = len(weights)
    params: List[torch.Tensor] = []
    for w, b in zip(weights, biases):
        params += [w, b]
    if ln is not None:
        params += [ln[0], ln[1]]
    cfg = (L, int(dim), int(factor), ln is not None, float(eps), float(dropout_p), int(seed) & (2 ** 64 - 1), ACT[post_act],
           torch.is_grad_enabled())
    return _FeedForward.apply(x, residual, cfg, *params)


class _Linear(torch.autograd.Function):
    @staticmethod
    def forward(ctx, x, w, b):
        lib = load()
        in_f, out_f = w.shape[1], w.shape[0]
        x2 = _f32c(x).reshape(-1, in_f)
        w = _f32c(w)
        b = _f32c(b) if b is not None else None
        P = x2.shape[0]
        out = torch.empty(P, out_f, dtype=torch.float32, device=x.device)
        check(lib.rpde_linear_fwd(ptr(x2), ptr(w), ptr(b), ptr(out), P, in_f, out_f, stream_ptr()), "linear_fwd")
        ctx.save_for_backward(x2, w)
        ctx.has_b = b is not None
        return out.reshape(*x.shape[:-1], out_f)

    @staticmethod
    def backward(ctx, g):
        lib = load()
        x2, w = ctx.saved_tensors
        out_f, in_f = w.shape
        P = x2.shape[0]
        g2 = _f32c(g).reshape(-1, out_f)
        gx = torch.empty_like(x2) if ctx.needs_input_grad[0] else None
        gw = torch.empty_like(w) if ctx.needs_input_grad[1] else None
        gb = torch.empty(out_f, dtype=torch.float32, device=g.device) if (ctx.has_b and ctx.needs_input_grad[2]) else None
        nws = lib.rpde_linear_ws_bytes(P, in_f, out_f)
        ws = workspace(nws, g.device)
        check(lib.rpde_linear_bwd(ptr(x2), ptr(w), ptr(g2), ptr(gx), ptr(gw), ptr(gb), P, in_f, out_f, ws.data_ptr(), nws,
                                  stream_ptr()), "linear_bwd")
        return (gx.reshape(*g.shape[:-1], in_f) if gx is not None else None), gw, gb


def linear(x, w, b=None):
    return _Linear.apply(x, w, b)


class _WeightNorm(torch.autograd.Function):
    @staticmethod
    def forward(ctx, v, g):
        lib = load()
        v = _f32c(v)
        g = _f32c(g)
        out_f, in_f = v.shape
        w = torch.empty_like(v)
        check(lib.rpde_weight_norm_fwd(ptr(v), ptr(g), ptr(w), out_f, in_f, stream_ptr()), "weight_norm_fwd")
        ctx.save_for_backward(v, g)
        return w

    @staticmethod
    def backward(ctx, gw):
        lib = load()
        v, g = ctx.saved_tensors
        out_f, in_f = v.shape
        gw = _f32c(gw)
        gv = torch.empty_like(v) if ctx.needs_input_grad[0] else None
        gg = torch.empty_like(g) if ctx.needs_input_grad[1] else None
        if gv is None and gg is None:
            return None, None
        check(lib.rpde_weight_norm_bwd(ptr(v), ptr(g), ptr(gw), ptr(gv), ptr(gg), out_f, in_f, stream_ptr()), "weight_norm_bwd")
        return gv, gg

# ... 482 lines not shown
```

Baseline: 1020 samples/s.

## Build backward weight images during forward to drop separate backward prep launches

The fused feedforward forward pass now fills both the forward and backward half-precision weight images in a single combined prep kernel, and stores the backward image so backward can skip its own prep launch. The factorized spectral 2D op gets an analogous path where forward writes a backward image consumed later. A dgrad fusion in the wgrad kernel also appears to be reworked. The aim is fewer small kernel launches and less redundant weight preprocessing per step, at the cost of extra per-call allocations held until backward.

```diff
diff --git a/include/rpde.h b/include/rpde.h
--- a/include/rpde.h
+++ b/include/rpde.h
@@ -83,6 +83,16 @@
                          float* grad_x, float* grad_wy, float* grad_wx, const float* grad_skip,
                          int B, int M, int N, int C, int K, int mode,
                          void* ws, size_t ws_bytes, void* stream);
+size_t rpde_fspectral2d_bwd_image_bytes(int M, int N, int C, int K);
+int rpde_fspectral2d_fwd_image(const float* x, const float* w_y, const float* w_x, float* out,
+                               float* spec_y, float* spec_x,
+                               int B, int M, int N, int C, int K, int mode,
+                               void* ws, size_t ws_bytes, void* bwd_image, size_t bwd_image_bytes, void* stream);
+int rpde_fspectral2d_bwd_image(const float* grad_out, const float* spec_y, const float* spec_x,
+                               const float* w_y, const float* w_x,
+                               float* grad_x, float* grad_wy, float* grad_wx, const float* grad_skip,
+                               int B, int M, int N, int C, int K, int mode,
+                               void* ws, size_t ws_bytes, const void* bwd_image, size_t bwd_image_bytes, void* stream);
 size_t rpde_fspectral2d_prep_bytes(int M, int N, int C, int K);
 size_t rpde_fspectral2d_eval_ws_bytes(int B, int M, int N, int C, int K);
 int rpde_fspectral2d_prepare(const float* w_y, const float* w_x, int M, int N, int C, int K,
@@ -131,6 +141,16 @@
                          float* const* grad_weights, float* const* grad_biases,
                          float* grad_gamma, float* grad_beta, int64_t P,
                          void* ws, size_t ws_bytes, void* stream);
+size_t rpde_feedforward_bwd_image_bytes(int dim, int factor, int n_layers);
+int rpde_feedforward_fwd_image(const rpde_ff_params* p, const float* x, const float* residual,
+                               float* const* hs, float* const* ds, float* z_last, float* out, int64_t P,
+                               void* ws, size_t ws_bytes, void* bwd_image, size_t bwd_image_bytes, void* stream);
+int rpde_feedforward_bwd_image(const rpde_ff_params* p, const float* x, const float* const* hs,
+                               const float* const* ds, const float* z_last,
+                               const float* grad_out, float* grad_x,
+                               float* const* grad_weights, float* const* grad_biases,
+                               float* grad_gamma, float* grad_beta, int64_t P,
+                               void* ws, size_t ws_bytes, const void* bwd_image, size_t bwd_image_bytes, void* stream);
 int rpde_feedforward_prepare(const rpde_ff_params* p, void* prep, size_t prep_bytes, void* stream);
 int rpde_feedforward_fwd_prepared(const rpde_ff_params* p, const float* x, const float* residual, float* out, int64_t P,
                                   const void* prep, size_t prep_bytes, void* stream);
diff --git a/resolution-pde_amd/csrc/feedforward.hip b/resolution-pde_amd/csrc/feedforward.hip
--- a/resolution-pde_amd/csrc/feedforward.hip
+++ b/resolution-pde_amd/csrc/feedforward.hip
@@ -168,8 +168,21 @@
                        const_cast<void*>(prep), as_stream(stream), true);
 }
 
+size_t rpde_feedforward_bwd_image_bytes(int dim, int factor, int n_layers) {
+  rpde_ff_params q;
+  memset(&q, 0, sizeof(q));
+  q.dim = dim; q.factor = factor; q.n_layers = n_layers;
+  return ff3_fused_ok(&q, 32) ? arena_bytes(ff3_fused_ws_floats()) : 0;
+}
+
 int rpde_feedforward_fwd(const rpde_ff_params* p, const float* x, const float* residual, float* const* hs,
                          float* const* ds, float* z_last, float* out, int64_t P, void* ws, size_t ws_bytes, void* stream) {
+  return rpde_feedforward_fwd_image(p, x, residual, hs, ds, z_last, out, P, ws, ws_bytes, nullptr, 0, stream);
+}
+
+int rpde_feedforward_fwd_image(const rpde_ff_params* p, const float* x, const float* residual, float* const* hs,
+                               float* const* ds, float* z_last, float* out, int64_t P, void* ws, size_t ws_bytes,
+                               void* bwd_image, size_t bwd_image_bytes, void* stream) {
   RPDE_CHECK_ARG(p && x && z_last && out && P > 0, "feedforward_fwd: bad arguments");
   RPDE_CHECK_ARG(p->n_layers >= 1 && p->dim > 0 && p->factor > 0, "feedforward_fwd: bad shape");
   RPDE_CHECK_ARG(P < (1L << 31), "feedforward_fwd: too many points for one call");
@@ -178,8 +191,11 @@
   if (ff3_fused_ok(p, P) && ws && ws_bytes >= arena_bytes(ff3_fused_ws_floats())) {
     RPDE_CHECK_ARG(p->weights[0] && p->weights[1] && p->weights[2], "feedforward_fwd: null weights");
     RPDE_CHECK_ARG(!p->layer_norm || (p->ln_gamma && p->ln_beta), "feedforward_fwd: layer_norm needs gamma/beta");
-    return ff3_fused_fwd(p, x, residual, hs, ds, z_last, out, P, ws, st);
-  }
+    RPDE_CHECK_ARG(!bwd_image || bwd_image_bytes >= arena_bytes(ff3_fused_ws_floats()), "feedforward_fwd: backward image of %zu bytes",
+                   bwd_image_bytes);
+    return ff3_fused_fwd(p, x, residual, hs, ds, z_last, out, P, ws, st, false, bwd_image);
+  }
+  RPDE_CHECK_ARG(!bwd_image, "feedforward_fwd: a backward image only exists on the fused path (rpde_feedforward_is_fused, scratch given)");
   RPDE_CHECK_ARG(p->n_layers == 1 || hs, "feedforward_fwd: hidden buffers missing");
   const int L = p->n_layers;
   Arena ar(ws, ws_bytes);
@@ -215,6 +231,14 @@
                          const float* z_last, const float* grad_out, float* grad_x, float* const* grad_weights,
                          float* const* grad_biases, float* grad_gamma, float* grad_beta, int64_t P, void* ws,
                          size_t ws_bytes, void* stream) {
+  return rpde_feedforward_bwd_image(p, x, hs, ds, z_last, grad_out, grad_x, grad_weights, grad_biases, grad_gamma, grad_beta, P,
+                                    ws, ws_bytes, nullptr, 0, stream);
+}
+
+int rpde_feedforward_bwd_image(const rpde_ff_params* p, const float* x, const float* const* hs, const float* const* ds,
+                               const float* z_last, const float* grad_out, float* grad_x, float* const* grad_weights,
+                               float* const* grad_biases, float* grad_gamma, float* grad_beta, int64_t P, void* ws,
+                               size_t ws_bytes, const void* bwd_image, size_t bwd_image_bytes, void* stream) {
   RPDE_CHECK_ARG(p && x && z_last && grad_out && P > 0, "feedforward_bwd: bad arguments");
   RPDE_CHECK_ARG(p->n_layers == 1 || (hs && ds), "feedforward_bwd: saved hidden tensors missing");
   RPDE_CHECK_ARG(P < (1L << 31), "feedforward_bwd: too many points for one call");
@@ -241,8 +265,10 @@
     void* fimg = ar.take(ff3_fused_ws_floats());
     if (!ar.ok()) { set_error("feedforward_bwd: workspace too small (%zu bytes given)", ws_bytes); return RPDE_ERR_WORKSPACE; }
     int grid = 0;
+    RPDE_CHECK_ARG(!bwd_image || bwd_image_bytes >= arena_bytes(ff3_fused_ws_floats()), "feedforward_bwd: backward image of %zu bytes",
+                   bwd_image_bytes);
     RPDE_TRY(ff3_fused_bwd_launch(p, recompute ? hs : ds, recompute, z_last, grad_out, dz3, buf0, buf1, nullptr, part, &grid, P,
-                                  fimg, st));
+                                  fimg, st, bwd_image));
     const bool both = grad_x && grad_weights && wgrad_h2_dgrad_ok(P, hid, p->dim);
     if (grad_x && !both) RPDE_TRY(linear_dgrad_impl(buf1, p->weights[0], grad_x, P, p->dim, hid, nullptr, nullptr, st, wt));
     if (grad_weights) {
@@ -267,6 +293,7 @@
     return RPDE_OK;
   }
 
+  RPDE_CHECK_ARG(!bwd_image, "feedforward_bwd: a backward image only exists on the fused path");
   FoldJobs folds;
   float* dz = buf0;
   float* other = buf1;
diff --git a/resolution-pde_amd/csrc/ff_fused.h b/resolution-pde_amd/csrc/ff_fused.h
--- a/resolution-pde_amd/csrc/ff_fused.h
+++ b/resolution-pde_amd/csrc/ff_fused.h
@@ -4,12 +4,13 @@
 namespace rpde {
 bool ff3_fused_ok(const rpde_ff_params* p, long P);
 size_t ff3_fused_ws_floats();
-int ff3_fused_prepare(const rpde_ff_params* p, void* ws, hipStream_t st);
+int ff3_fused_prepare(const rpde_ff_params* p, void* ws, hipStream_t st, void* bwd_image = nullptr);
 int ff3_fused_fwd(const rpde_ff_params* p, const float* x, const float* residual, float* const* hs, float* const* ds,
-                  float* z_last, float* out, long P, void* ws, hipStream_t st, bool prepared = false);
+                  float* z_last, float* out, long P, void* ws, hipStream_t st, bool prepared = false,
+                  void* bwd_image = nullptr);
 constexpr int FF3_PART = 704;
 size_t ff3_fused_bwd_part_floats();
 int ff3_fused_bwd_launch(const rpde_ff_params* p, const float* const* ds, int recompute, const float* z_last,
                          const float* grad_out, float* dz3, float* du2, float* du1, float* dx, float* part, int* grid_out,
-                         long P, void* ws, hipStream_t st);
+                         long P, void* ws, hipStream_t st, const void* bwd_image = nullptr);
 }
diff --git a/resolution-pde_amd/csrc/ff_fused.hip b/resolution-pde_amd/csrc/ff_fused.hip
--- a/resolution-pde_amd/csrc/ff_fused.hip
+++ b/resolution-pde_amd/csrc/ff_fused.hip
@@ -21,10 +21,10 @@
 constexpr int FF_NCONST = 16;
 constexpr int FF_PREP_BLOCKS = FF_WAVES * FF_FRAGS * 64 / 1024;
 
-__global__ __launch_bounds__(1024) void k_ff3_prep(const float* __restrict__ w1, const float* __restrict__ w2,
+__device__ __forceinline__ void ff3_prep_fwd_block(const float* __restrict__ w1, const float* __restrict__ w2,
                                                    const float* __restrict__ w3, const float* __restrict__ b1,
                                                    const float* __restrict__ b2, char* __restrict__ img,
-                                                   float* __restrict__ consts) {
+                                                   float* __restrict__ consts, int blk, int nblk) {
   __shared__ float red[6][16];
   __shared__ float fin[6];
   const int tid = threadIdx.x, l = tid & 63, wv = tid >> 6;
@@ -72,11 +72,11 @@
   float sc[3], iv[3];
 #pragma unroll
   for (int k = 0; k < 3; ++k) h2_scale(fin[k], 0, sc[k], iv[k]);
-  if (tid == 0 && blockIdx.x == 0) {
+  if (tid == 0 && blk == 0) {
     consts[0] = iv[0]; consts[1] = iv[1]; consts[2] = iv[2];
     consts[3] = fin[3]; consts[4] = fin[4]; consts[5] = fin[5]; consts[6] = fin_b2;
   }
-  for (int it = blockIdx.x * 1024 + tid; it < FF_WAVES * FF_FRAGS * 64; it += gridDim.x * 1024) {
+  for (int it = blk * 1024 + tid; it < FF_WAVES * FF_FRAGS * 64; it += nblk * 1024) {
     const int ln = it & 63, f = (it >> 6) % FF_FRAGS, w = it / (64 * FF_FRAGS);
     const int g = ln >> 4, li = ln & 15;
     float x[8];
@@ -95,6 +95,12 @@
     }
     h2_put_frag(img + ((long)(w * FF_FRAGS + f)) * 2048 + ln * 16, x);
   }
+}
+__global__ __launch_bounds__(1024) void k_ff3_prep(const float* __restrict__ w1, const float* __restrict__ w2,
+                                                   const float* __restrict__ w3, const float* __restrict__ b1,
+                                                   const float* __restrict__ b2, char* __restrict__ img,
+                                                   float* __restrict__ consts) {
+  ff3_prep_fwd_block(w1, w2, w3, b1, b2, img, consts, blockIdx.x, gridDim.x);
 }
 
 struct FF3P {
@@ -385,9 +391,9 @@
   }
 }
 
-__global__ __launch_bounds__(1024) void k_ff3_prep_bwd(const float* __restrict__ w1, const float* __restrict__ w2,
-                                                       const float* __restrict__ w3, char* __restrict__ img,
-                                                       float* __restrict__ consts) {
+__device__ __forceinline__ void ff3_prep_bwd_block(const float* __restrict__ w1, const float* __restrict__ w2,
+                                                   const float* __restrict__ w3, char* __restrict__ img,
+                                                   float* __restrict__ consts, int blk, int nblk) {
   __shared__ float red[5][16];
   __shared__ float fin[5];
   const int tid = threadIdx.x, l = tid & 63, wv = tid >> 6;
@@ -436,8 +442,8 @@
   float sc[3], iv[3];
 #pragma unroll
   for (int k = 0; k < 3; ++k) h2_scale(fin[k], 0, sc[k], iv[k]);
-  if (tid == 0 && blockIdx.x == 0) { consts[0] = iv[0]; consts[1] = iv[1]; consts[2] = iv[2]; consts[3] = fin[3]; consts[4] = fin[4]; }
-  for (int it = blockIdx.x * 1024 + tid; it < FF_WAVES * FF_FRAGS * 64; it += gridDim.x * 1024) {
+  if (tid == 0 && blk == 0) { consts[0] = iv[0]; consts[1] = iv[1]; consts[2] = iv[2]; consts[3] = fin[3]; consts[4] = fin[4]; }
+  for (int it = blk * 1024 + tid; it < FF_WAVES * FF_FRAGS * 64; it += nblk * 1024) {
     const int ln = it & 63, f = (it >> 6) % FF_FRAGS, w = it / (64 * FF_FRAGS);
     const int g = ln >> 4, li = ln & 15;
     float x[8];
@@ -456,6 +462,19 @@
     }
     h2_put_frag(img + ((long)(w * FF_FRAGS + f)) * 2048 + ln * 16, x);
   }
+}
+__global__ __launch_bounds__(1024) void k_ff3_prep_bwd(const float* __restrict__ w1, const float* __restrict__ w2,
+                                                       const float* __restrict__ w3, char* __restrict__ img,
+                                                       float* __restrict__ consts) {
+  ff3_prep_bwd_block(w1, w2, w3, img, consts, blockIdx.x, gridDim.x);
+}
+__global__ __launch_bounds__(1024) void k_ff3_prep_both(const float* __restrict__ w1, const float* __restrict__ w2,
+                                                        const float* __restrict__ w3, const float* __restrict__ b1,
+                                                        const float* __restrict__ b2, char* __restrict__ img,
+                                                        float* __restrict__ consts, char* __restrict__ img_bwd,
+                                                        float* __restrict__ consts_bwd) {
+  if (blockIdx.x < FF_PREP_BLOCKS) ff3_prep_fwd_block(w1, w2, w3, b1, b2, img, consts, blockIdx.x, FF_PREP_BLOCKS);
+  else ff3_prep_bwd_block(w1, w2, w3, img_bwd, consts_bwd, blockIdx.x - FF_PREP_BLOCKS, FF_PREP_BLOCKS);
 }
 
 constexpr int FFB_PART = 704;
@@ -798,24 +817,30 @@
 }
 size_t ff3_fused_ws_floats() { return (FF_IMG_BYTES + FF_NCONST * 4 + 3) / 4; }
 
-int ff3_fused_prepare(const rpde_ff_params* p, void* ws, hipStream_t st) {
+int ff3_fused_prepare(const rpde_ff_params* p, void* ws, hipStream_t st, void* bwd_image) {
   char* img = static_cast<char*>(ws);
   float* consts = reinterpret_cast<float*>(img + FF_IMG_BYTES);
   const float* b1 = p->biases ? p->biases[0] : nullptr;
   const float* b2 = p->biases ? p->biases[1] : nullptr;
-  hipLaunchKernelGGL(k_ff3_prep, dim3(FF_PREP_BLOCKS), dim3(1024), 0, st, p->weights[0], p->weights[1], p->weights[2], b1, b2, img, consts);
+  if (bwd_image) {
+    char* imgb = static_cast<char*>(bwd_image);
+    hipLaunchKernelGGL(k_ff3_prep_both, dim3(2 * FF_PREP_BLOCKS), dim3(1024), 0, st, p->weights[0], p->weights[1], p->weights[2], b1,
+                       b2, img, consts, imgb, reinterpret_cast<float*>(imgb + FF_IMG_BYTES));
+  } else {
+    hipLaunchKernelGGL(k_ff3_prep, dim3(FF_PREP_BLOCKS), dim3(1024), 0, st, p->weights[0], p->weights[1], p->weights[2], b1, b2, img, consts);
+  }
   RPDE_LAUNCH_CHECK();
   return RPDE_OK;
 }
 
 int ff3_fused_fwd(const rpde_ff_params* p, const float* x, const float* residual, float* const* hs, float* const* ds,
-                  float* z_last, float* out, long P, void* ws, hipStream_t st, bool prepared) {
+                  float* z_last, float* out, long P, void* ws, hipStream_t st, bool prepared, void* bwd_image) {
   char* img = static_cast<char*>(ws);
   float* consts = reinterpret_cast<float*>(img + FF_IMG_BYTES);
   const float* b1 = p->biases ? p->biases[0] : nullptr;
   const float* b2 = p->biases ? p->biases[1] : nullptr;
   const float* b3 = p->biases ? p->biases[2] : nullptr;
-  if (!prepared) RPDE_TRY(ff3_fused_prepare(p, ws, st));
+  if (!prepared) RPDE_TRY(ff3_fused_prepare(p, ws, st, bwd_image));
   FF3P A;
   memset(&A, 0, sizeof(A));
   const bool have_h = hs && hs[0] && hs[1], have_d = ds && ds[0] && ds[1];
@@ -843,11 +868,13 @@
 
 int ff3_fused_bwd_launch(const rpde_ff_params* p, const float* const* ds, int recompute, const float* z_last,
                          const float* grad_out, float* dz3, float* du2, float* du1, float* dx, float* part, int* grid_out,
-                         long P, void* ws, hipStream_t st) {
-  char* img = static_cast<char*>(ws);
+                         long P, void* ws, hipStream_t st, const void* bwd_image) {
+  char* img = bwd_image ? const_cast<char*>(static_cast<const char*>(bwd_image)) : static_cast<char*>(ws);
   float* consts = reinterpret_cast<float*>(img + FF_IMG_BYTES);
-  hipLaunchKernelGGL(k_ff3_prep_bwd, dim3(FF_PREP_BLOCKS), dim3(1024), 0, st, p->weights[0], p->weights[1], p->weights[2], img, consts);
-  RPDE_LAUNCH_CHECK();
+  if (!bwd_image) {
+    hipLaunchKernelGGL(k_ff3_prep_bwd, dim3(FF_PREP_BLOCKS), dim3(1024), 0, st, p->weights[0], p->weights[1], p->weights[2], img, consts);
+    RPDE_LAUNCH_CHECK();
+  }
   FF3B A;
   memset(&A, 0, sizeof(A));
   A.g = grad_out; A.z3 = z_last; A.d1 = ds[0]; A.d2 = ds[1];
diff --git a/resolution-pde_amd/csrc/fspectral.hip b/resolution-pde_amd/csrc/fspectral.hip
--- a/resolution-pde_amd/csrc/fspectral.hip
+++ b/resolution-pde_amd/csrc/fspectral.hip
@@ -186,9 +186,13 @@
   return n;
 }
 
+static float* mix_image_consts(const Axis& ay, const void* image) {
+  return reinterpret_cast<float*>(static_cast<char*>(const_cast<void*>(image)) + arena_bytes(mix_wimg_bytes(ay.kp) / 4));
+}
+
 static int fused2d_fwd(const Axis& ay, const Axis& ax, const float* x, const float* w_y, const float* w_x, float* out,
                        float* spec_y, float* spec_x, int B, int M, int N, int C, int K, int mode, Arena& ar, hipStream_t st,
-                       const void* prep = nullptr) {
+                       const void* prep = nullptr, void* bwd_image = nullptr) {
   float* wblk = ar.take((size_t)ay.keff * 4 * C * C);
   const size_t sy = spec_floats(ay, C), sx = spec_floats(ax, C);
   float* mixed = ar.take(sy > sx ? sy : sx);
@@ -204,9 +208,9 @@
   if (mode == RPDE_MODE_FULL && fused_mix_on()) {
     if (prep) {
       wimg = const_cast<void*>(prep);
-      wc = reinterpret_cast<float*>(static_cast<char*>(wimg) + arena_bytes(mix_wimg_bytes(ay.kp) / 4));
+      wc = mix_image_consts(ay, prep);
     } else {
-      RPDE_TRY(mix_prep(w_y, w_x, K, ay.keff, ay.kp, 0, wimg, wc, st));
+      RPDE_TRY(mix_prep(w_y, w_x, K, ay.keff, ay.kp, 0, wimg, wc, st, bwd_image, bwd_image ? mix_image_consts(ay, bwd_image) : nullptr));
     }
     RPDE_TRY(fused2d_analysis(x, spec_y, spec_x, amy, amx, ay.plan, ax.plan, 0, B, M, N, st));
     RPDE_TRY(mix_h2(spec_y, spec_x, amy, amx, imgy, imgx, invy, invx, ay.rows, ax.rows, ay.kp, wimg, wc, st));
@@ -234,7 +238,7 @@
 
 static int fused2d_bwd(const Axis& ay, const Axis& ax, const float* g, const float* spec_y, const float* spec_x,
                        const float* w_y, const float* w_x, float* gx, float* gwy, float* gwx, const float* skip, int B, int M,
-                       int N, int C, int K, int mode, Arena& ar, hipStream_t st) {
+                       int N, int C, int K, int mode, Arena& ar, hipStream_t st, const void* bwd_image = nullptr) {
   float* gsy = ar.take(spec_floats(ay, C));
   float* gsx = ar.take(spec_floats(ax, C));
   float* wblk = ar.take((size_t)ay.keff * 4 * C * C);
@@ -255,7 +259,12 @@
   if (!ar.ok()) { set_error("fspectral2d: workspace too small"); return RPDE_ERR_WORKSPACE; }
   const bool h2mix = mode == RPDE_MODE_FULL && fused_mix_on();
   const bool hmix = h2mix && gx, hwg = h2mix && (gwy || gwx);
-  if (hmix) RPDE_TRY(mix_prep(w_y, w_x, K, ay.keff, ay.kp, 1, wimg, wc, st));
+  if (hmix && bwd_image) {
+    wimg = const_cast<void*>(bwd_image);
+    wc = mix_image_consts(ay, bwd_image);
+  } else if (hmix) {
+    RPDE_TRY(mix_prep(w_y, w_x, K, ay.keff, ay.kp, 1, wimg, wc, st));
+  }
   RPDE_TRY(fused2d_analysis(g, gsy, gsx, h2mix ? amy : nullptr, h2mix ? amx : nullptr, ay.plan, ax.plan, 1, B, M, N, st));
   if (hmix) {
     RPDE_TRY(mix_h2(gsy, gsx, amy, amx, imgy, imgx, invy, invx, ay.rows, ax.rows, ay.kp, wimg, wc, st));
@@ -352,6 +361,14 @@
 
 int rpde_fspectral2d_fwd(const float* x, const float* w_y, const float* w_x, float* out, float* spec_y, float* spec_x, int B,
                          int M, int N, int C, int K, int mode, void* ws, size_t ws_bytes, void* stream) {
+  return rpde_fspectral2d_fwd_image(x, w_y, w_x, out, spec_y, spec_x, B, M, N, C, K, mode, ws, ws_bytes, nullptr, 0, stream);
+}
+
+size_t rpde_fspectral2d_bwd_image_bytes(int M, int N, int C, int K) { return rpde_fspectral2d_prep_bytes(M, N, C, K); }
+
+int rpde_fspectral2d_fwd_image(const float* x, const float* w_y, const float* w_x, float* out, float* spec_y, float* spec_x,
+                               int B, int M, int N, int C, int K, int mode, void* ws, size_t ws_bytes, void* bwd_image,
+                               size_t bwd_image_bytes, void* stream) {
   RPDE_CHECK_ARG(x && out && spec_y && spec_x && B > 0 && M > 0 && N > 0 && C > 0 && K > 0, "fspectral2d_fwd: bad arguments");
   RPDE_CHECK_ARG(mode == RPDE_MODE_LOWPASS || (w_y && w_x), "fspectral2d_fwd: null weight");
   RPDE_CHECK_ARG(mode == RPDE_MODE_FULL || mode == RPDE_MODE_LOWPASS, "fspectral2d_fwd: mode %d", mode);
@@ -359,9 +376,12 @@
   Axis ay, ax;
   RPDE_TRY(make_axis(ay, N, K, RPDE_NORM_ORTHO, B * M, 1, (long)N * C, 0, C, st));
   RPDE_TRY(make_axis(ax, M, K, RPDE_NORM_ORTHO, B * N, N, (long)M * N * C, C, (long)N * C, st));
+  RPDE_CHECK_ARG(!bwd_image || (mode == RPDE_MODE_FULL && rpde_fspectral2d_bwd_image_bytes(M, N, C, K) > 0 &&
+                                bwd_image_bytes >= rpde_fspectral2d_bwd_image_bytes(M, N, C, K)),
+                 "fspectral2d_fwd: this call has no backward image (rpde_fspectral2d_bwd_image_bytes) or the buffer is too small");
   if (fused2d_ok(M, N, C, ay.keff, ax.keff)) {
     Arena ar(ws, ws_bytes);
-    return fused2d_fwd(ay, ax, x, w_y, w_x, out, spec_y, spec_x, B, M, N, C, K, mode, ar, st);
+    return fused2d_fwd(ay, ax, x, w_y, w_x, out, spec_y, spec_x, B, M, N, C, K, mode, ar, st, nullptr, bwd_image);
   }
   {
     Arena ar(ws, ws_bytes);
@@ -414,16 +434,27 @@
 int rpde_fspectral2d_bwd(const float* grad_out, const float* spec_y, const float* spec_x, const float* w_y, const float* w_x,
                          float* grad_x, float* grad_wy, float* grad_wx, const float* grad_skip, int B, int M, int N, int C,
                          int K, int mode, void* ws, size_t ws_bytes, void* stream) {
+  return rpde_fspectral2d_bwd_image(grad_out, spec_y, spec_x, w_y, w_x, grad_x, grad_wy, grad_wx, grad_skip, B, M, N, C, K, mode, ws,
+                                    ws_bytes, nullptr, 0, stream);
+}
+
+int rpde_fspectral2d_bwd_image(const float* grad_out, const float* spec_y, const float* spec_x, const float* w_y,
+                               const float* w_x, float* grad_x, float* grad_wy, float* grad_wx, const float* grad_skip, int B,
+                               int M, int N, int C, int K, int mode, void* ws, size_t ws_bytes, const void* bwd_image,
+                               size_t bwd_image_bytes, void* stream) {
   RPDE_CHECK_ARG(grad_out && spec_y && spec_x && B > 0 && M > 0 && N > 0 && C > 0 && K > 0, "fspectral2d_bwd: bad arguments");
   RPDE_CHECK_ARG(mode == RPDE_MODE_LOWPASS || (w_y && w_x), "fspectral2d_bwd: null weight");
   hipStream_t st = as_stream(stream);
   Axis ay, ax;
   RPDE_TRY(make_axis(ay, N, K, RPDE_NORM_ORTHO, B * M, 1, (long)N * C, 0, C, st));
   RPDE_TRY(make_axis(ax, M, K, RPDE_NORM_ORTHO, B * N, N, (long)M * N * C, C, (long)N * C, st));
+  RPDE_CHECK_ARG(!bwd_image || (mode == RPDE_MODE_FULL && rpde_fspectral2d_bwd_image_bytes(M, N, C, K) > 0 &&
+                                bwd_image_bytes >= rpde_fspectral2d_bwd_image_bytes(M, N, C, K)),
+                 "fspectral2d_bwd: this call has no backward image (rpde_fspectral2d_bwd_image_bytes) or the buffer is too small");
   if (fused2d_ok(M, N, C, ay.keff, ax.keff)) {
     Arena ar(ws, ws_bytes);
     return fused2d_bwd(ay, ax, grad_out, spec_y, spec_x, w_y, w_x, grad_x, grad_wy, grad_wx, grad_skip, B, M, N, C, K, mode,
-                       ar, st);
+                       ar, st, bwd_image);
   }
   {
     Arena ar(ws, ws_bytes);
diff --git a/resolution-pde_amd/csrc/fused_mix.hip b/resolution-pde_amd/csrc/fused_mix.hip
--- a/resolution-pde_amd/csrc/fused_mix.hip
+++ b/resolution-pde_amd/csrc/fused_mix.hip
@@ -4,10 +4,12 @@
 namespace rpde {
 
 __global__ __launch_bounds__(256) void k_mix_prep(const float* __restrict__ w_y, const float* __restrict__ w_x, int K, int keff,
-                                                  int kp, int conj_t, char* __restrict__ img, float* __restrict__ wc) {
+                                                  int kp, int conj_t, char* __restrict__ img, float* __restrict__ wc,
+                                                  char* __restrict__ img_t, float* __restrict__ wc_t) {
   __shared__ float ws[64 * 64 * 2];
   __shared__ float red[2][4];
   const int k = blockIdx.x, a = blockIdx.y, tid = threadIdx.x, l = tid & 63, wv = tid >> 6, g = l >> 4, li = l & 15;
+  if (blockIdx.z) { conj_t = 1; img = img_t; wc = wc_t; }
   const float* __restrict__ w = a ? w_x : w_y;
   char* out = img + (size_t)(a * kp + k) * MIX_W_BYTES_PER_MODE;
   if (k >= keff) {
@@ -71,8 +73,10 @@
 
 size_t mix_wimg_bytes(int kp) { return (size_t)2 * kp * MIX_W_BYTES_PER_MODE; }
 
-int mix_prep(const float* w_y, const float* w_x, int K, int keff, int kp, int conj_t, void* wimg, float* wc, hipStream_t st) {
-  hipLaunchKernelGGL(k_mix_prep, dim3(kp, 2), dim3(256), 0, st, w_y, w_x, K, keff, kp, conj_t, (char*)wimg, wc);
+int mix_prep(const float* w_y, const float* w_x, int K, int keff, int kp, int conj_t, void* wimg, float* wc, hipStream_t st,
+             void* wimg_t, float* wc_t) {
+  hipLaunchKernelGGL(k_mix_prep, dim3(kp, 2, wimg_t ? 2 : 1), dim3(256), 0, st, w_y, w_x, K, keff, kp, conj_t, (char*)wimg, wc,
+                     (char*)wimg_t, wc_t);
   RPDE_LAUNCH_CHECK();
   return RPDE_OK;
 }
diff --git a/resolution-pde_amd/csrc/fused_spectral.h b/resolution-pde_amd/csrc/fused_spectral.h
--- a/resolution-pde_amd/csrc/fused_spectral.h
+++ b/resolution-pde_amd/csrc/fused_spectral.h
@@ -19,7 +19,8 @@
 
 constexpr int MIX_W_BYTES_PER_MODE = 4 * 2 * 2 * 2 * 1024;
 size_t mix_wimg_bytes(int kp);
-int mix_prep(const float* w_y, const float* w_x, int K, int keff, int kp, int conj_t, void* wimg, float* wc, hipStream_t st);
+int mix_prep(const float* w_y, const float* w_x, int K, int keff, int kp, int conj_t, void* wimg, float* wc, hipStream_t st,
+             void* wimg_t = nullptr, float* wc_t = nullptr);
 size_t mix_wgrad_slab_floats(int kp, int S);
 int mix_wgrad_h2(const float* spec_y, const float* spec_x, const float* gspec_y, const float* gspec_x, const float* amax_sy,
                  const float* amax_sx, const float* amax_gy, const float* amax_gx, float* gw_y, float* gw_x, long lines_y,
diff --git a/resolution-pde_amd/csrc/wgrad_h2.hip b/resolution-pde_amd/csrc/wgrad_h2.hip
--- a/resolution-pde_amd/csrc/wgrad_h2.hip
+++ b/resolution-pde_amd/csrc/wgrad_h2.hip
@@ -1,3 +1,4 @@
+#include <type_traits>
 #include "h2.h"
 #include "pointwise.h"
 #include "wgrad_h2.h"
@@ -47,10 +48,18 @@
     if ((s + 1) * 32 <= P.npts) {
 #pragma unroll
       for (int i = 0; i < 8; ++i) buf[i] = *reinterpret_cast<const float4*>(q0 + (long)(4 * i) * ld);
-    } else {
+    } else if constexpr (!DG) {
 #pragma unroll
       for (int i = 0; i < 8; ++i)
         buf[i] = s * 32 + 4 * i + g < P.npts ? *reinterpret_cast<const float4*>(q0 + (long)(4 * i) * ld) : make_float4(0.f, 0.f, 0.f, 0.f);
+    } else {
+#pragma unroll
+      for (int i = 0; i < 8; ++i) {
+        const long r = s * 32 + 4 * i + g;
+        float4 v = *reinterpret_cast<const float4*>(q0 + ((r < P.npts ? r : P.npts - 1) - (s * 32 + g)) * ld);
+        asm volatile("" : "+v"(v.x), "+v"(v.y), "+v"(v.z), "+v"(v.w));
+        buf[i] = r < P.npts ? v : make_float4(0.f, 0.f, 0.f, 0.f);
+      }
     }
   };
   auto convert = [&](int st) {
@@ -140,9 +149,13 @@
     }
   }
   const int dg_mt = wave & 1, dg_nt = wave >> 1;
+  __amdgpu_buffer_rsrc_t gx_rows;
+  if constexpr (DG)
+    gx_rows = __builtin_amdgcn_make_buffer_rsrc(P.gx + s0 * 32 * P.N, 0,
+                                                __builtin_amdgcn_readfirstlane((int)((min(s1 * 32, P.npts) - s0 * 32) * P.N * 4)), 0x00020000);
 
   const bool early_convert = (P.early >> __builtin_amdgcn_readfirstlane(wave)) & 1;
-  if (s0 < s1) {
+  if (!DG && s0 < s1) {
     issue(s0);
     convert(0);
     issue(s0 + 1);
@@ -181,29 +194,6 @@
 #pragma unroll
         for (int j = 0; j < TN; ++j) acc[i][j] = h2_mfma32(ah, al, bh[j], bl[j], acc[i][j]);
       }
-      if (DG) {
-        f32x4v tot = (f32x4v){0.f, 0.f, 0.f, 0.f};
-        const int row = 16 * dg_mt + li;
-#pragma unroll
-        for (int k = 0; k < PA; ++k) {
-          f32x4v part = (f32x4v){0.f, 0.f, 0.f, 0.f};
-#pragma unroll
-          for (int h = 0; h < 2; ++h) {
-            const char* pa_ = stage + k * WG_PANEL + stage_off(row, 2 * (4 * h + g));
-            const f16x8 ah = *reinterpret_cast<const f16x8*>(pa_), al = *reinterpret_cast<const f16x8*>(pa_ + 4096);
-            const char* wb = wfrag + ((2 * k + h) * 4 + dg_nt) * 2048 + l * 16;
-            const f16x8 bh = *reinterpret_cast<const f16x8*>(wb), bl = *reinterpret_cast<const f16x8*>(wb + 1024);
-            part = h2_mfma32(ah, al, bh, bl, part);
-          }
-          const int ek = __builtin_amdgcn_readfirstlane(einfo[cur][k]);
-          const float fk = __uint_as_float((unsigned)(ek - 14) << 23) * w_inv;
-          tot += part * fk;
-        }
-        float t0 = tot[0], t1 = tot[1], t2 = tot[2], t3 = tot[3];
-        quad_transpose(t0, t1, t2, t3);
-        const long pq = s * 32 + 16 * dg_mt + 4 * g + (li & 3);
-        if (pq < P.npts) *reinterpret_cast<float4*>(P.gx + pq * P.N + 16 * dg_nt + 4 * (li >> 2)) = make_float4(t0, t1, t2, t3);
-      }
       if (!early_convert && s + 1 < s1) {
         convert(cur ^ 1);
         issue(s + 2);
@@ -212,6 +202,82 @@
     }
   }
 
+  auto dg_steps = [&](auto early) {
+    constexpr bool EARLY = decltype(early)::value;
+    auto next_panel = [&](long s, int st) {
+      if (!loader || s >= s1) return;
+      convert(st);
+      issue(s + 1);
+    };
+    issue(s0);
+    convert(0);
+    issue(s0 + 1);
+    lds_barrier();
+    if (EARLY) next_panel(s0 + 1, 1);
+    for (long s = s0; s < s1; ++s) {
+      const int cur = (int)(s - s0) & 1;
+      const char* const stage = smem + cur * STAGE;
+      const int eb = __builtin_amdgcn_readfirstlane(einfo[cur][pb]);
+#pragma unroll
+      for (int k = 0; k < NPA; ++k) {
+        const int ea = __builtin_amdgcn_readfirstlane(einfo[cur][pa + k]);
+        if (ea + eb != ea_used[k] + eb_used) {
+          const int d = (ea_used[k] + eb_used) - (ea + eb);
+          const float f = d > -126 ? __uint_as_float((unsigned)(127 + d) << 23) : 0.f;
+#pragma unroll
+          for (int i = 0; i < TM; ++i)
+            if (((ta0 + i) >> 2) == k) {
+#pragma unroll
+              for (int j = 0; j < TN; ++j) acc[i][j] *= f;
+            }
+        }
+        ea_used[k] = ea;
+      }
+      eb_used = eb;
+      f16x8 bh[TN], bl[TN];
+#pragma unroll
+      for (int j = 0; j < TN; ++j) frag(stage + (pb + ((tb0 + j) >> 2)) * WG_PANEL, (tb0 + j) & 3, bh[j], bl[j]);
+#pragma unroll
+      for (int i = 0; i < TM; ++i) {
+        f16x8 ah, al;
+        frag(stage + (pa + ((ta0 + i) >> 2)) * WG_PANEL, (ta0 + i) & 3, ah, al);
+#pragma unroll
+        for (int j = 0; j < TN; ++j) acc[i][j] = h2_mfma32(ah, al, bh[j], bl[j], acc[i][j]);
+      }
+      f32x4v tot = (f32x4v){0.f, 0.f, 0.f, 0.f};
+      const int row = 16 * dg_mt + li;
+#pragma unroll
+      for (int k = 0; k < PA; ++k) {
+        f32x4v part = (f32x4v){0.f, 0.f, 0.f, 0.f};
+#pragma unroll
+        for (int h = 0; h < 2; ++h) {
+          const char* pa_ = stage + k * WG_PANEL + stage_off(row, 2 * (4 * h + g));
+          const f16x8 ah = *reinterpret_cast<const f16x8*>(pa_), al = *reinterpret_cast<const f16x8*>(pa_ + 4096);
+          const char* wb = wfrag + ((2 * k + h) * 4 + dg_nt) * 2048 + l * 16;
+          const f16x8 bh = *reinterpret_cast<const f16x8*>(wb), bl = *reinterpret_cast<const f16x8*>(wb + 1024);
+          part = h2_mfma32(ah, al, bh, bl, part);
+        }
+        const int ek = __builtin_amdgcn_readfirstlane(einfo[cur][k]);
+        const float fk = __uint_as_float((unsigned)(ek - 14) << 23) * w_inv;
+        tot += part * fk;
+      }
+      float t0 = tot[0], t1 = tot[1], t2 = tot[2], t3 = tot[3];
+      quad_transpose(t0, t1, t2, t3);
+      typedef unsigned u32x4v __attribute__((ext_vector_type(4)));
+      const int prow = (int)(s - s0) * 32 + 16 * dg_mt + 4 * g + (li & 3);
+      __builtin_amdgcn_raw_buffer_store_b128((u32x4v){__float_as_uint(t0), __float_as_uint(t1), __float_as_uint(t2), __float_as_uint(t3)},
+                                             gx_rows, (prow * P.N + 16 * dg_nt + 4 * (li >> 2)) * 4, 0, 0);
+      if (!EARLY) next_panel(s + 1, cur ^ 1);
+      lds_barrier();
+      if (EARLY) next_panel(s + 2, cur);
+    }
+  };
+  if constexpr (DG) {
+    if (s0 < s1) {
+      if (early_convert) dg_steps(std::true_type()); else dg_steps(std::false_type());
+    }
+  }
+
   const float fb = __uint_as_float((unsigned)(eb_used - 14) << 23);
   float* __restrict__ out = P.slabs + (long)chunk * P.M * P.N + (long)(mblock * (64 * PA) + m_off) * P.N + n_off;
 #pragma unroll
@@ -232,6 +298,9 @@
 static int wg_chunks(int, int) { return WG_BLOCKS; }
 
 static int wg_early_mask(int out_f, int in_f) {
+#ifdef RPDE_WG_DG_EARLY
+  if (out_f == 256 && in_f == 64) return RPDE_WG_DG_EARLY;
+#endif
   return out_f == 256 && in_f == 256 ? 0xF0 : (out_f == 64 ? 0x0E : 0x00);
 }
 
@@ -251,6 +320,7 @@
 int wgrad_h2_dgrad(const float* gy, const float* h, const float* w, float* gw, float* gx, long P, int in_f, int out_f,
                    float* slabs, hipStream_t st, FoldJobs* defer) {
   RPDE_CHECK_ARG(wgrad_h2_dgrad_ok(P, out_f, in_f) && slabs && w && gx, "wgrad_h2_dgrad: unsupported shape");
+  RPDE_CHECK_ARG((P / WG_BLOCKS + 64) * in_f * 4 < (1L << 31), "wgrad_h2_dgrad: %ld points per workgroup", P / WG_BLOCKS);
   WgP p;
   p.a = gy; p.b = h; p.slabs = slabs; p.npts = P; p.steps = (P + 31) / 32; p.M = out_f; p.N = in_f; p.nchunk = WG_BLOCKS;
   p.early = wg_early_mask(out_f, in_f);
diff --git a/resolution-pde_amd/rpde/_lib.py b/resolution-pde_amd/rpde/_lib.py
--- a/resolution-pde_amd/rpde/_lib.py
+++ b/resolution-pde_amd/rpde/_lib.py
@@ -88,8 +88,14 @@
     "rpde_feedforward_is_fused": (_I, [_I, _I, _I, _L]),
     "rpde_feedforward_fwd": (_I, [C.POINTER(FFParams), _P, _P, _PP, _PP, _P, _P, _L, _P, _Z, _P]),
     "rpde_feedforward_bwd": (_I, [C.POINTER(FFParams), _P, _PP, _PP, _P, _P, _P, _PP, _PP, _P, _P, _L, _P, _Z, _P]),
+    "rpde_feedforward_bwd_image_bytes": (_Z, [_I, _I, _I]),
+    "rpde_feedforward_fwd_image": (_I, [C.POINTER(FFParams), _P, _P, _PP, _PP, _P, _P, _L, _P, _Z, _P, _Z, _P]),
+    "rpde_feedforward_bwd_image": (_I, [C.POINTER(FFParams), _P, _PP, _PP, _P, _P, _P, _PP, _PP, _P, _P, _L, _P, _Z, _P, _Z, _P]),
     "rpde_feedforward_prepare": (_I, [C.POINTER(FFParams), _P, _Z, _P]),
     "rpde_feedforward_fwd_prepared": (_I, [C.POINTER(FFParams), _P, _P, _P, _L, _P, _Z, _P]),
+    "rpde_fspectral2d_bwd_image_bytes": (_Z, [_I, _I, _I, _I]),
+    "rpde_fspectral2d_fwd_image": (_I, [_P, _P, _P, _P, _P, _P, _I, _I, _I, _I, _I, _I, _P, _Z, _P, _Z, _P]),
+    "rpde_fspectral2d_bwd_image": (_I, [_P, _P, _P, _P, _P, _P, _P, _P, _P, _I, _I, _I, _I, _I, _I, _P, _Z, _P, _Z, _P]),
     "rpde_fspectral2d_prep_bytes": (_Z, [_I, _I, _I, _I]),
     "rpde_fspectral2d_eval_ws_bytes": (_Z, [_I, _I, _I, _I, _I]),
     "rpde_fspectral2d_prepare": (_I, [_P, _P, _I, _I, _I, _I, _P, _Z, _P]),
diff --git a/resolution-pde_amd/rpde/ops.py b/resolution-pde_amd/rpde/ops.py
--- a/resolution-pde_amd/rpde/ops.py
+++ b/resolution-pde_amd/rpde/ops.py
@@ -111,8 +111,13 @@
         spec_x = torch.empty(lib.rpde_fspectral2d_spec_elems(B, M, N, Cc, modes, 1), dtype=torch.float32, device=x.device)
         nws = lib.rpde_fspectral2d_ws_bytes(B, M, N, Cc, modes)
         ws = workspace(nws, x.device)
-        check(lib.rpde_fspectral2d_fwd(ptr(x), ptr(wyf), ptr(wxf), ptr(out), ptr(spec_y), ptr(spec_x), B, M, N, Cc, modes,
-                                       mode, ws.data_ptr(), nws, stream_ptr()), "fspectral2d_fwd")
+        need_x_grad = ctx.needs_input_grad[0]
+        nimg = lib.rpde_fspectral2d_bwd_image_bytes(M, N, Cc, modes) if (has_w and need_x_grad and mode == MODE["full"]) else 0
+        image = torch.empty((nimg + 3) // 4, dtype=torch.float32, device=x.device) if nimg else None
+        check(lib.rpde_fspectral2d_fwd_image(ptr(x), ptr(wyf), ptr(wxf), ptr(out), ptr(spec_y), ptr(spec_x), B, M, N, Cc, modes,
+                                             mode, ws.data_ptr(), nws, ptr(image), 4 * image.numel() if image is not None else 0,
+                                             stream_ptr()), "fspectral2d_fwd")
+        ctx.bwd_image = image
         if has_w:
             ctx.save_for_backward(spec_y, spec_x, wyf, wxf)
         else:
@@ -139,9 +144,11 @@
         gwx = torch.empty_like(wxf) if need_w else None
         nws = lib.rpde_fspectral2d_ws_bytes(B, M, N, Cc, modes)
         ws = workspace(nws, g.device)
-        check(lib.rpde_fspectral2d_bwd(ptr(g), ptr(spec_y), ptr(spec_x), ptr(wyf), ptr(wxf), ptr(gx), ptr(gwy), ptr(gwx),
-                                       ptr(g_skip) if need_x else None,
-                                       B, M, N, Cc, modes, mode, ws.data_ptr(), nws, stream_ptr()), "fspectral2d_bwd")
+        image = ctx.bwd_image
+        check(lib.rpde_fspectral2d_bwd_image(ptr(g), ptr(spec_y), ptr(spec_x), ptr(wyf), ptr(wxf), ptr(gx), ptr(gwy), ptr(gwx),
+                                             ptr(g_skip) if need_x else None,
+                                             B, M, N, Cc, modes, mode, ws.data_ptr(), nws, ptr(image),
+                                             4 * image.numel() if image is not None else 0, stream_ptr()), "fspectral2d_bwd")
         return gx, gwy, gwx, None, None, None
 
 
@@ -236,11 +243,15 @@
                                                         stream_ptr()), "feedforward_fwd_prepared")
                 return out.reshape(shape)
         ws = workspace(nws, x.device)
-        check(lib.rpde_feedforward_fwd(C.byref(fp), ptr(x2), ptr(res2), C.cast(ha, C.POINTER(C.c_void_p)),
-                                       C.cast(da, C.POINTER(C.c_void_p)), ptr(z_last), ptr(out), P, ws.data_ptr(), nws,
-                                       stream_ptr()), "feedforward_fwd")
+        nimg = lib.rpde_feedforward_bwd_image_bytes(dim, factor, L) if (need_grad and fused) else 0
+        image = torch.empty((nimg + 3) // 4, dtype=torch.float32, device=x.device) if nimg else None
+        check(lib.rpde_feedforward_fwd_image(C.byref(fp), ptr(x2), ptr(res2), C.cast(ha, C.POINTER(C.c_void_p)),
+                                             C.cast(da, C.POINTER(C.c_void_p)), ptr(z_last), ptr(out), P, ws.data_ptr(), nws,
+                                             ptr(image), 4 * image.numel() if image is not None else 0, stream_ptr()),
+              "feedforward_fwd")
         ctx.cfg = cfg
         ctx.has_res = residual is not None
+        ctx.bwd_image = image
         if need_grad:
             ctx.save_for_backward(x2, z_last, *hs, *ds, *ws_, *bs_, *([gamma, beta] if layer_norm else []))
         return out.reshape(shape)
@@ -270,10 +281,12 @@
                            C.cast(wa, C.POINTER(C.c_void_p)), C.cast(ba, C.POINTER(C.c_void_p)), ptr(gamma), ptr(beta), epoch)
         nws = lib.rpde_feedforward_ws_bytes(P, dim, factor, L)
         ws = workspace(nws, g.device)
-        check(lib.rpde_feedforward_bwd(C.byref(fp), ptr(x2), C.cast(ha, C.POINTER(C.c_void_p)),
-                                       C.cast(da, C.POINTER(C.c_void_p)), ptr(z_last), ptr(g2), ptr(gx),
-                                       C.cast(gwa, C.POINTER(C.c_void_p)), C.cast(gba, C.POINTER(C.c_void_p)),
-                                       ptr(ggamma), ptr(gbeta), P, ws.data_ptr(), nws, stream_ptr()), "feedforward_bwd")
+        image = ctx.bwd_image
+        check(lib.rpde_feedforward_bwd_image(C.byref(fp), ptr(x2), C.cast(ha, C.POINTER(C.c_void_p)),
+                                             C.cast(da, C.POINTER(C.c_void_p)), ptr(z_last), ptr(g2), ptr(gx),
+                                             C.cast(gwa, C.POINTER(C.c_void_p)), C.cast(gba, C.POINTER(C.c_void_p)),
+                                             ptr(ggamma), ptr(gbeta), P, ws.data_ptr(), nws, ptr(image),
+                                             4 * image.numel() if image is not None else 0, stream_ptr()), "feedforward_bwd")
         grads: List[Optional[torch.Tensor]] = []
         for l in range(L):
             grads += [gws[l], gbs[l]]
```

Result: no change. 1024 samples/s, median of 6 (+0.4%).
